# friendlymatthew/heif

Measured on AMD Instinct MI355X. Metric: Mpixels/s decoded (bit-exact) on 4032x3024 HEIC batch, higher is better.
Workload: dtype u8

## Files before the change

### heif_amd/csrc/api.cpp

```cpp
#include <hip/hip_runtime.h>

#include <algorithm>
#include <cmath>
#include <cstdlib>
#include <cstring>
#include <atomic>
#include <memory>
#include <mutex>
#include <string>
#include <thread>
#include <vector>

#include "../../include/heifgpu.h"
#include "common/desc.hpp"
#include "host/batch.hpp"
#include "host/heic_image.hpp"
#include "kernels/cabac.hpp"
#include "kernels/kernels.hpp"

using namespace hg;

struct heifgpu_image {
    ParsedImage img;
};

static_assert(sizeof(heifgpu_image_info) == 80, "heifgpu_image_info: 20 x uint32");
static_assert(sizeof(heifgpu_planes) == 40, "heifgpu_planes: 3 pointers + 3 int32 (+ padding)");
static_assert(sizeof(heifgpu_batch_opts) == 20, "heifgpu_batch_opts: 5 x uint32");
static_assert(sizeof(heifgpu_display_info) == 44, "heifgpu_display_info: 11 x 32 bits");
static_assert(sizeof(heifgpu_surface) == 16, "heifgpu_surface: pointer + int32 (+ padding)");
static_assert(sizeof(heifgpu_rect) == 16, "heifgpu_rect: 4 x uint32");
static_assert(HEIFGPU_PIX_RGB8 == RENDER_RGB8 && HEIFGPU_PIX_RGBA8 == RENDER_RGBA8 && HEIFGPU_PIX_RGB16 == RENDER_RGB16 &&
                  HEIFGPU_PIX_RGBA16 == RENDER_RGBA16,
              "pixel formats");
static_assert(sizeof(heifgpu_ipc_handle) == 72, "heifgpu_ipc_handle: 64-byte HIP handle + uint64 offset");
static_assert(HEIFGPU_PARSE_AUTO == PARSE_AUTO && HEIFGPU_PARSE_LANES == PARSE_LANES && HEIFGPU_PARSE_SOLO == PARSE_SOLO &&
                  HEIFGPU_PARSE_SPREAD == PARSE_SPREAD,
              "parse modes");
static_assert(sizeof(heifgpu_tile_params) == 55 * 4 + 64 * 4, "heifgpu_tile_params: 55 int32 + 64 uint32");

constexpr int kTimingSlots = 32;
struct RenderRing;
struct heifgpu_ctx {
    int device = 0;
    bool timing = false;
    hipStream_t parse = nullptr, xform = nullptr, recon = nullptr, upload = nullptr;
    hipStream_t prep = nullptr;
    hipEvent_t fork = nullptr, join = nullptr;
    StreamKnobs stream;
    hipEvent_t tev[kTimingSlots][10] = {};
    int timed_calls = 0, folded = 0;
    double acc[6] = {};
    RenderRing *render = nullptr;
};

namespace {
size_t xprog_words(const HostBatch &hb) { return size_t(hb.rows) + 1; }
size_t xntu_words(const HostBatch &hb) { return size_t(hb.rows) + hb.pics.size() + 1; }

bool prep_stream_default() {
    const char *e = std::getenv("HEIFGPU_PREP_STREAM");
    return e && std::atoi(e) != 0;
}

hipError_t fold_timing(heifgpu_ctx *ctx, int slot) {
    hipEvent_t *e = ctx->tev[slot];
    hipError_t r = hipEventSynchronize(e[8]);
    if (r != hipSuccess) return r;
    float t = 0.f;
    if ((r = hipEventElapsedTime(&t, e[0], e[1])) != hipSuccess) return r;
    ctx->acc[5] += t;
    if ((r = hipEventElapsedTime(&t, e[9], e[2])) != hipSuccess) return r;
    ctx->acc[0] += t;
    if ((r = hipEventElapsedTime(&t, e[3], e[4])) != hipSuccess) return r;
    ctx->acc[1] += t;
    for (int i = 2; i < 5; ++i) {
        if ((r = hipEventElapsedTime(&t, e[i + 3], e[i + 4])) != hipSuccess) return r;
        ctx->acc[i] += t;
    }
    return hipSuccess;
}
}

namespace {

thread_local std::string g_err;

int fail(int code, const std::string &msg) {
    g_err = msg;
    return code;
}

bool fault_injected(const char *what) {
    const char *e = std::getenv("HEIFGPU_FAULT_INJECT");
    return e && std::strcmp(e, what) == 0;
}

#define HIP_TRY(expr)                                                                             \
    do {                                                                                          \
        hipError_t e_ = (expr);                                                                   \
        if (e_ != hipSuccess) return fail(HEIFGPU_E_DEVICE, std::string(#expr) + ": " + hipGetErrorString(e_)); \
    } while (0)

template <class T>
struct DevBuf {
    T *p = nullptr;
    size_t n = 0;
    DevBuf() = default;
    DevBuf(const DevBuf &) = delete;
    DevBuf &operator=(const DevBuf &) = delete;
    ~DevBuf() {
        if (p) (void)hipFree(p);
    }
    size_t cap = 0;
    hipError_t alloc(size_t count) {
        n = count;
        if (p && count <= cap) return hipSuccess;
        if (p) {
            hipError_t e = hipFree(p);
            p = nullptr;
            cap = 0;
            if (e != hipSuccess) return e;
        }
        cap = std::max<size_t>(count, 1);
        return hipMalloc(reinterpret_cast<void **>(&p), cap * sizeof(T));
    }
};

struct PinnedBuf {
    uint8_t *p = nullptr;
    size_t cap = 0;
    PinnedBuf() = default;
    PinnedBuf(const PinnedBuf &) = delete;
    PinnedBuf &operator=(const PinnedBuf &) = delete;
    ~PinnedBuf() {
        if (p) (void)hipHostFree(p);
    }
    hipError_t reserve(size_t bytes) {
        if (p && bytes <= cap) return hipSuccess;
        if (p) {
            hipError_t e = hipHostFree(p);
            p = nullptr;
            cap = 0;
            if (e != hipSuccess) return e;
        }
        cap = std::max<size_t>(bytes, 4096);
        return hipHostMalloc(reinterpret_cast<void **>(&p), cap, hipHostMallocDefault);
    }
};

}

constexpr int kRenderSlots = 4;
struct RenderRing {
    struct Slot {
        PinnedBuf host;
        DevBuf<RenderDesc> dev;
        DevBuf<ScaleDesc> sdev;
        DevBuf<TensorDesc> tdev;
        hipEvent_t done = nullptr;
        bool pending = false;
    } slot[kRenderSlots];
    int next = 0;
    ~RenderRing() {
        for (Slot &s : slot)
            if (s.done) (void)hipEventDestroy(s.done);
    }
};

struct ParseSet {
    DevBuf<TuRec> tus;
    DevBuf<Coef> coefs;
    DevBuf<uint32_t> row_counts, status;
    DevBuf<uint8_t> maps;
    DevBuf<SaoParams> sao;
    DevBuf<int16_t> resid;
    DevBuf<uint32_t> xprog, xntu;
    DevBuf<uint8_t> rbsp;
    DevBuf<uint32_t> rsubs;
    hipEvent_t parsed = nullptr, transformed = nullptr, recon_done = nullptr, progreset = nullptr, prepped = nullptr;
    bool pending = false;
    ~ParseSet() {
        if (parsed) (void)hipEventDestroy(parsed);
        if (transformed) (void)hipEventDestroy(transformed);
        if (recon_done) (void)hipEventDestroy(recon_done);
        if (progreset) (void)hipEventDestroy(progreset);
        if (prepped) (void)hipEventDestroy(prepped);
    }
};

struct DescGen {
    DevBuf<PicDesc> pics;
    DevBuf<SeqParams> seqs;
    DevBuf<uint8_t> sf;
    DevBuf<OutImage> outs;
    DevBuf<uint32_t> sticky;
    std::vector<OutImage> out_host;
    hipEvent_t done = nullptr;
    bool pending = false;
    std::vector<uint32_t> pic_image;
    size_t n_images = 0;
    bool loaded = false;
    ~DescGen() {
        if (done) (void)hipEventDestroy(done);
    }
};

struct heifgpu_batch {
    int device = 0;
    size_t n_images = 0;
    int n_pics = 0;
    uint32_t tile_stride = 1, tile_offset = 0;
    PinnedBuf stage;
    hipEvent_t uploaded = nullptr;
    bool loaded = false;
    BatchArgs args{};
    DevBuf<uint8_t> bits;
    DevBuf<uint32_t> subs, porder;
    DevBuf<uint8_t> xctx;
    DevBuf<uint8_t> recon;
    DescGen gen[2];
    int cur = 0;
    ParseSet set[3];
    int n_sets = 1, next_set = 0, last_set = 0;
    std::vector<uint32_t> pic_image;
    std::vector<heifgpu_image_info> infos;
    ~heifgpu_batch() {
        if (uploaded) (void)hipEventDestroy(uploaded);
    }
};

extern "C" {

const char *heifgpu_last_error(void) { return g_err.c_str(); }

int heifgpu_image_parse(const uint8_t *data, size_t len, heifgpu_image **out) {
    return heifgpu_image_parse_item(data, len, 0, out);
}

int heifgpu_image_parse_item(const uint8_t *data, size_t len, uint32_t item_id, heifgpu_image **out) {
    if (!data || !out) return fail(HEIFGPU_E_INVALID, "null argument");
    *out = nullptr;
    try {
        auto im = std::make_unique<heifgpu_image>();
        im->img = parse_heic(data, len, item_id);
        *out = im.release();
        return HEIFGPU_OK;
    } catch (const UnsupportedError &e) {
        return fail(HEIFGPU_E_UNSUPPORTED, e.what());
    } catch (const std::exception &e) {
        return fail(HEIFGPU_E_PARSE, e.what());
    }
}

int heifgpu_image_parse_many(const uint8_t *const *data, const size_t *len, size_t n, int threads,
                             heifgpu_image **out, int *rc) {
    if (!data || !len || !out) return fail(HEIFGPU_E_INVALID, "null argument");
    for (size_t i = 0; i < n; ++i) out[i] = nullptr;
    std::vector<int> codes(n, HEIFGPU_OK);
    std::vector<std::string> msgs(n);
    std::atomic<size_t> next{0};
    auto worker = [&] {
        for (size_t i; (i = next.fetch_add(1)) < n;) {
            if (!data[i]) {
                codes[i] = HEIFGPU_E_INVALID;
                msgs[i] = "null data";
                continue;
            }
            try {
                auto im = std::make_unique<heifgpu_image>();
                im->img = parse_heic(data[i], len[i], 0);
                out[i] = im.release();
            } catch (const UnsupportedError &e) {
                codes[i] = HEIFGPU_E_UNSUPPORTED;
                msgs[i] = e.what();
            } catch (const std::exception &e) {
                codes[i] = HEIFGPU_E_PARSE;
                msgs[i] = e.what();
            }
        }
    };
    size_t nt = threads > 0 ? size_t(threads) : size_t(std::max(1u, std::thread::hardware_concurrency()));
    nt = std::min(nt, n);
    std::vector<std::thread> pool;
    for (size_t t = 1; t < nt; ++t) pool.emplace_back(worker);
    worker();
    for (auto &th : pool) th.join();
    int first = HEIFGPU_OK;
    for (size_t i = 0; i < n; ++i) {
        if (rc) rc[i] = codes[i];
        if (codes[i] != HEIFGPU_OK && first == HEIFGPU_OK) {
            first = codes[i];
            g_err = "image " + std::to_string(i) + ": " + msgs[i];
        }
    }
    return first;
}

int heifgpu_gather_tiles(const heifgpu_image_info *info, const heifgpu_planes *dst, const heifgpu_planes *src,
                         uint32_t tile_stride, uint32_t tile_offset, void *stream) {
    if (!info || !dst || !src) return fail(HEIFGPU_E_INVALID, "null argument");
    if (tile_stride == 0) tile_stride = 1;
    if (tile_offset >= tile_stride) return fail(HEIFGPU_E_INVALID, "tile_offset must be below tile_stride");
    if (info->chroma_format_idc > 3) return fail(HEIFGPU_E_INVALID, "chroma_format_idc");
    const int planes = info->chroma_format_idc ? 3 : 1;
    for (int c = 0; c < planes; ++c)
        if (!dst->plane[c] || !src->plane[c]) return fail(HEIFGPU_E_INVALID, "missing plane");
    hipPointerAttribute_t ad{}, as{};
    HIP_TRY(hipPointerGetAttributes(&ad, dst->plane[0]));
    HIP_TRY(hipPointerGetAttributes(&as, src->plane[0]));
    int cur = 0;
    HIP_TRY(hipGetDevice(&cur));
    HIP_TRY(hipSetDevice(ad.device));
    if (ad.device != as.device) {
        const hipError_t e = hipDeviceEnablePeerAccess(as.device, 0);
        (void)hipGetLastError();
        if (e != hipSuccess && e != hipErrorPeerAccessAlreadyEnabled) {
            (void)hipSetDevice(cur);
            HIP_TRY(e);
        }
    }
    GatherArgs g{};
    for (int c = 0; c < 3; ++c) {
        g.dst[c] = reinterpret_cast<uint64_t>(dst->plane[c]);
        g.src[c] = reinterpret_cast<uint64_t>(src->plane[c]);
        g.dpitch[c] = dst->pitch[c];
        g.spitch[c] = src->pitch[c];
    }
    g.planes = planes;
    g.sx = chroma_sx(int(info->chroma_format_idc));
    g.sy = chroma_sy(int(info->chroma_format_idc));
    g.bps = int32_t(info->bytes_per_sample);
    g.W = int32_t(info->width);
    g.H = int32_t(info->height);
    g.cols = int32_t(std::max(1u, info->grid_cols));
    g.tw = int32_t(info->tile_width ? info->tile_width : info->width);
    g.th = int32_t(info->tile_height ? info->tile_height : info->height);
    g.n_tiles = int32_t(std::max(1u, info->num_tiles));
    g.stride = int32_t(tile_stride);
    g.offset = int32_t(tile_offset);
    const hipError_t e = launch_gather_tiles(g, static_cast<hipStream_t>(stream));
    (void)hipSetDevice(cur);
    HIP_TRY(e);
    return HEIFGPU_OK;
}

namespace {
std::mutex g_ipc_mu;
std::vector<std::pair<void *, void *>> g_ipc_open;
}

int heifgpu_ipc_export(const void *dev_ptr, heifgpu_ipc_handle *out) {
    static_assert(sizeof(hipIpcMemHandle_t) == sizeof(out->handle), "hipIpcMemHandle_t is 64 bytes");
    if (!dev_ptr || !out) return fail(HEIFGPU_E_INVALID, "null argument");
    hipDeviceptr_t base = nullptr;
    size_t size = 0;
    HIP_TRY(hipMemGetAddressRange(&base, &size, const_cast<void *>(dev_ptr)));
    hipIpcMemHandle_t h;
    HIP_TRY(hipIpcGetMemHandle(&h, base));
    std::memcpy(out->handle, &h, sizeof(h));
    out->offset = uint64_t(static_cast<const uint8_t *>(dev_ptr) - static_cast<const uint8_t *>(base));
    return HEIFGPU_OK;
}

int heifgpu_ipc_open(int device, const heifgpu_ipc_handle *h, void **dev_ptr) {
    if (!h || !dev_ptr) return fail(HEIFGPU_E_INVALID, "null argument");
    *dev_ptr = nullptr;
    int cur = 0;
    HIP_TRY(hipGetDevice(&cur));
    HIP_TRY(hipSetDevice(device));
    hipIpcMemHandle_t mh;
    std::memcpy(&mh, h->handle, sizeof(mh));
    void *base = nullptr;
    const hipError_t e = hipIpcOpenMemHandle(&base, mh, hipIpcMemLazyEnablePeerAccess);
    (void)hipSetDevice(cur);
    HIP_TRY(e);
    *dev_ptr = static_cast<uint8_t *>(base) + h->offset;
    std::lock_guard<std::mutex> lk(g_ipc_mu);
    g_ipc_open.emplace_back(*dev_ptr, base);
    return HEIFGPU_OK;
}

int heifgpu_ipc_close(void *dev_ptr) {
    void *base = nullptr;
    {
        std::lock_guard<std::mutex> lk(g_ipc_mu);
        for (size_t i = 0; i < g_ipc_open.size(); ++i)
            if (g_ipc_open[i].first == dev_ptr) {
                base = g_ipc_open[i].second;
                g_ipc_open.erase(g_ipc_open.begin() + long(i));
                break;
            }
    }
    if (!base) return fail(HEIFGPU_E_INVALID, "not a pointer returned by heifgpu_ipc_open");
    HIP_TRY(hipIpcCloseMemHandle(base));
    return HEIFGPU_OK;
}

int heifgpu_image_get_info(const heifgpu_image *img, heifgpu_image_info *info) {
    if (!img || !info) return fail(HEIFGPU_E_INVALID, "null argument");
    const ParsedImage &p = img->img;
    const SequenceParameterSet &s = p.params[0].sps;
    std::memset(info, 0, sizeof(*info));
    info->width = p.out_width;
    info->height = p.out_height;
    info->chroma_format_idc = uint32_t(s.chroma_array_type());
    info->bit_depth = uint32_t(8 + s.bit_depth_luma_minus8);
    info->bytes_per_sample = info->bit_depth > 8 ? 2 : 1;
    info->grid_rows = p.rows;
    info->grid_cols = p.cols;
    info->tile_width = p.tile_width;
    info->tile_height = p.tile_height;
    info->num_tiles = uint32_t(p.tiles.size());
    info->rotation = p.rotation;
    info->ispe_width = p.ispe_width;
    info->ispe_height = p.ispe_height;
    info->coded_bytes = p.coded_bytes;
    info->primary_item_id = p.primary_item_id;
    info->num_thumbnails = p.num_thumbnails;
    info->matrix_coeffs = p.nclx ? p.nclx_matrix : uint32_t(s.matrix_coeffs);
    info->full_range = p.nclx ? p.nclx_full_range : (s.video_full_range_flag ? 1u : 0u);
    info->item_id = p.item_id;
    info->aux_item_id = p.aux_item_id;
    return HEIFGPU_OK;
}

int heifgpu_ycbcr_to_rgb(heifgpu_ctx *ctx, const heifgpu_image_info *info, const heifgpu_planes *in, void *rgb,
                         int32_t rgb_pitch, void *stream) {
    if (!ctx || !info || !in || !rgb || !in->plane[0]) return fail(HEIFGPU_E_INVALID, "invalid argument");
    if (info->chroma_format_idc > 3) return fail(HEIFGPU_E_INVALID, "chroma_format_idc");
    if (info->chroma_format_idc && (!in->plane[1] || !in->plane[2])) return fail(HEIFGPU_E_INVALID, "missing chroma plane");
    if (info->bit_depth < 8 || info->bit_depth > 16) return fail(HEIFGPU_E_INVALID, "bit depth");
    HIP_TRY(hipSetDevice(ctx->device));
    ColorArgs c{};
    for (int k = 0; k < 3; ++k) {
        c.plane[k] = reinterpret_cast<uint64_t>(in->plane[k]);
        c.pitch[k] = in->pitch[k];
    }
    c.rgb = reinterpret_cast<uint64_t>(rgb);
    c.rgb_pitch = rgb_pitch;
    c.w = int32_t(info->width);
    c.h = int32_t(info->height);
    c.rotation = int32_t(info->rotation & 3);
    c.out_w = (c.rotation & 1) ? c.h : c.w;
    c.out_h = (c.rotation & 1) ? c.w : c.h;
    if (rgb_pitch < 3 * c.out_w) return fail(HEIFGPU_E_INVALID, "rgb_pitch smaller than 3 * output width");
    c.chroma = int32_t(info->chroma_format_idc);
    c.shift = int32_t(info->bit_depth) - 8;
    color_coefs(info->matrix_coeffs, info->full_range != 0, c);
    HIP_TRY(launch_ycbcr_rgb(c, int(info->bytes_per_sample), static_cast<hipStream_t>(stream)));
    return HEIFGPU_OK;
}

int heifgpu_image_get_display(const heifgpu_image *img, heifgpu_display_info *out) {
    if (!img || !out) return fail(HEIFGPU_E_INVALID, "null argument");
    const ParsedImage &p = img->img;
    std::memset(out, 0, sizeof(*out));
    out->out_width = p.display.out_width;
    out->out_height = p.display.out_height;
    for (int k = 0; k < 4; ++k) out->m[k] = p.display.m[k];
    out->t[0] = p.display.t[0];
    out->t[1] = p.display.t[1];
    out->n_transforms = p.display.n_transforms;
    out->alpha_item_id = p.alpha_item_id;
    out->alpha_premultiplied = p.alpha_premultiplied;
    return HEIFGPU_OK;
}

static int render_desc_fill(size_t i, const heifgpu_image *const *imgs, const heifgpu_planes *in,
                            const heifgpu_image *const *alpha_imgs, const heifgpu_planes *alpha_in, uint32_t format,
                            const heifgpu_surface *out, const DisplayMap &dm, uint32_t ow, uint32_t oh, int &bps,
                            RenderDesc &d) {
    const bool wide = format >= HEIFGPU_PIX_RGB16, with_alpha = (format & 1) != 0;
    const int bpp = (with_alpha ? 4 : 3) * (wide ? 2 : 1);
    heifgpu_image_info info;
    heifgpu_image_get_info(imgs[i], &info);
// ... 187 lines not shown
    }
    if (!ctx) return fail(HEIFGPU_E_INVALID, "null context");
    hipStream_t s = static_cast<hipStream_t>(stream);
    RenderRing::Slot *slot = nullptr;
    if (int rc = render_ring_slot(ctx, &slot)) return rc;
    RenderRing::Slot &sl = *slot;
    const size_t bytes = n * sizeof(ScaleDesc);
    HIP_TRY(sl.host.reserve(bytes));
    HIP_TRY(sl.sdev.alloc(n));
    std::memcpy(sl.host.p, descs.data(), bytes);
    HIP_TRY(hipMemcpyAsync(sl.sdev.p, sl.host.p, bytes, hipMemcpyHostToDevice, s));
    HIP_TRY(launch_render_scaled(sl.sdev.p, int(n), max_tiles, int(format), bps, s));
    HIP_TRY(hipEventRecord(sl.done, s));
    sl.pending = true;
    return HEIFGPU_OK;
}

int heifgpu_render_batch_tensor(heifgpu_ctx *ctx, const heifgpu_image *const *imgs, size_t n, const heifgpu_planes *in,
                                const heifgpu_image *const *alpha_imgs, const heifgpu_planes *alpha_in,
                                const heifgpu_tensor_format *fmt, const heifgpu_scale *scale, const uint32_t *flip,
                                const heifgpu_tensor_surface *out, void *stream) {
    if (!imgs || !in || !fmt || !scale || !out || n == 0) return fail(HEIFGPU_E_INVALID, "invalid argument");
    if (fmt->src > HEIFGPU_PIX_RGBA16) return fail(HEIFGPU_E_INVALID, "source format");
    if (fmt->elem > HEIFGPU_ELEM_BF16) return fail(HEIFGPU_E_INVALID, "element type");
    if (fmt->layout > HEIFGPU_LAYOUT_HWC) return fail(HEIFGPU_E_INVALID, "layout");
    const int nch = (fmt->src & 1) ? 4 : 3;
    for (int c = 0; c < nch; ++c)
        if (!std::isfinite(fmt->a[c]) || !std::isfinite(fmt->b[c]))
            return fail(HEIFGPU_E_INVALID, "scale or bias not finite");
    if (n > 65535) return fail(HEIFGPU_E_INVALID, "more than 65535 images in one render call");
    const int64_t esz = fmt->elem == HEIFGPU_ELEM_F32 ? 4 : 2;
    std::vector<TensorDesc> descs(n);
    int bps = 0, max_tiles = 0;
    for (size_t i = 0; i < n; ++i) {
        const uint32_t fl = flip ? flip[i] : 0;
        if (fl > 3) return fail(HEIFGPU_E_INVALID, "flip above 3");
        TensorDesc &td = descs[i];
        if (int rc = scale_desc_fill(i, imgs, in, alpha_imgs, alpha_in, fmt->src, scale[i], fl, nullptr, bps, td.s))
            return rc;
        const heifgpu_tensor_surface &o = out[i];
        if (!o.data || (reinterpret_cast<uintptr_t>(o.data) & uintptr_t(esz - 1)))
            return fail(HEIFGPU_E_INVALID, "tensor data null or not aligned to its element");
        const int64_t row = int64_t(td.s.r.out_w) * esz * (fmt->layout == HEIFGPU_LAYOUT_HWC ? nch : 1);
        if (o.stride_y < row || (o.stride_y & (esz - 1)))
            return fail(HEIFGPU_E_INVALID, "stride_y below the row or not a multiple of the element size");
        if (fmt->layout == HEIFGPU_LAYOUT_CHW && (o.stride_c & (esz - 1)))
            return fail(HEIFGPU_E_INVALID, "stride_c not a multiple of the element size");
        td.s.r.out = reinterpret_cast<uint64_t>(o.data);
        td.stride_c = fmt->layout == HEIFGPU_LAYOUT_CHW ? o.stride_c : 0;
        td.stride_y = o.stride_y;
        td.elem = int32_t(fmt->elem);
        td.layout = int32_t(fmt->layout);
        for (int c = 0; c < 4; ++c) {
            td.a[c] = c < nch ? fmt->a[c] : 0.f;
            td.b[c] = c < nch ? fmt->b[c] : 0.f;
        }
        max_tiles = std::max(max_tiles, td.s.r.tiles);
    }
    if (!ctx) return fail(HEIFGPU_E_INVALID, "null context");
    hipStream_t s = static_cast<hipStream_t>(stream);
    RenderRing::Slot *slot = nullptr;
    if (int rc = render_ring_slot(ctx, &slot)) return rc;
    RenderRing::Slot &sl = *slot;
    const size_t bytes = n * sizeof(TensorDesc);
    HIP_TRY(sl.host.reserve(bytes));
    HIP_TRY(sl.tdev.alloc(n));
    std::memcpy(sl.host.p, descs.data(), bytes);
    HIP_TRY(hipMemcpyAsync(sl.tdev.p, sl.host.p, bytes, hipMemcpyHostToDevice, s));
    HIP_TRY(launch_render_tensor(sl.tdev.p, int(n), max_tiles, int(fmt->src), bps, s));
    HIP_TRY(hipEventRecord(sl.done, s));
    sl.pending = true;
    return HEIFGPU_OK;
}

void heifgpu_image_free(heifgpu_image *img) { delete img; }

int heifgpu_create(int device, heifgpu_ctx **out) {
    if (!out) return fail(HEIFGPU_E_INVALID, "null argument");
    *out = nullptr;
    int n = 0;
    HIP_TRY(hipGetDeviceCount(&n));
    if (device < 0 || device >= n) return fail(HEIFGPU_E_DEVICE, "no such HIP device");
    HIP_TRY(hipSetDevice(device));
    auto c = std::make_unique<heifgpu_ctx>();
    c->device = device;
    c->stream = stream_knobs_from_env();
    static const bool prio = [] {
        const char *e = std::getenv("HEIFGPU_PARSE_PRIORITY");
        return e && std::atoi(e) != 0;
    }();
    int least = 0, greatest = 0;
    HIP_TRY(hipDeviceGetStreamPriorityRange(&least, &greatest));
    HIP_TRY(hipStreamCreateWithPriority(&c->parse, hipStreamNonBlocking, prio ? greatest : least));
    static const bool rprio = [] {
        const char *e = std::getenv("HEIFGPU_RECON_PRIORITY");
        return e && std::atoi(e) != 0;
    }();
    HIP_TRY(hipStreamCreateWithPriority(&c->xform, hipStreamNonBlocking, rprio ? greatest : least));
    HIP_TRY(hipStreamCreateWithPriority(&c->recon, hipStreamNonBlocking, rprio ? greatest : least));
    HIP_TRY(hipStreamCreateWithFlags(&c->upload, hipStreamNonBlocking));
    if (prep_stream_default()) HIP_TRY(hipStreamCreateWithFlags(&c->prep, hipStreamNonBlocking));
    HIP_TRY(hipEventCreateWithFlags(&c->fork, hipEventDisableTiming));
    HIP_TRY(hipEventCreateWithFlags(&c->join, hipEventDisableTiming));
    for (auto &row : c->tev)
        for (auto &e : row) HIP_TRY(hipEventCreate(&e));
    *out = c.release();
    return HEIFGPU_OK;
}

void heifgpu_destroy(heifgpu_ctx *ctx) {
    if (!ctx) return;
    (void)hipSetDevice(ctx->device);
    (void)hipDeviceSynchronize();
    for (auto &row : ctx->tev)
        for (auto &e : row)
            if (e) (void)hipEventDestroy(e);
    if (ctx->fork) (void)hipEventDestroy(ctx->fork);
    if (ctx->join) (void)hipEventDestroy(ctx->join);
    if (ctx->parse) (void)hipStreamDestroy(ctx->parse);
    if (ctx->xform) (void)hipStreamDestroy(ctx->xform);
    if (ctx->recon) (void)hipStreamDestroy(ctx->recon);
    if (ctx->upload) (void)hipStreamDestroy(ctx->upload);
    if (ctx->prep) (void)hipStreamDestroy(ctx->prep);
    delete ctx->render;
    delete ctx;
}

int heifgpu_set_timing(heifgpu_ctx *ctx, int enable) {
    if (!ctx) return fail(HEIFGPU_E_INVALID, "null ctx");
    if (enable && !ctx->timing) {
        for (double &v : ctx->acc) v = 0.0;
        ctx->timed_calls = ctx->folded = 0;
    }
    ctx->timing = enable != 0;
    return HEIFGPU_OK;
}

int heifgpu_stage_times(heifgpu_ctx *ctx, float ms[6]) {
    if (!ctx || !ms) return fail(HEIFGPU_E_INVALID, "null argument");
    if (!ctx->timing) return fail(HEIFGPU_E_INVALID, "timing disabled");
    for (int i = 0; i < 6; ++i) ms[i] = 0.f;
    for (int c = ctx->folded; c < ctx->timed_calls; ++c) HIP_TRY(fold_timing(ctx, c % kTimingSlots));
    if (ctx->timed_calls)
        for (int i = 0; i < 6; ++i) ms[i] = float(ctx->acc[i] / ctx->timed_calls);
    for (double &v : ctx->acc) v = 0.0;
    ctx->timed_calls = ctx->folded = 0;
    return HEIFGPU_OK;
}

static Rect rect_of(const heifgpu_rect &r) { return Rect{r.x, r.y, r.width, r.height}; }

int heifgpu_window_source_rect(const heifgpu_image *img, const heifgpu_rect *window, heifgpu_rect *src) {
    if (!img || !src) return fail(HEIFGPU_E_INVALID, "null argument");
    Rect out;
    if (!window_source_rect(img->img, window ? rect_of(*window) : Rect{}, out))
        return fail(HEIFGPU_E_INVALID, "window empty or outside the displayed picture");
    *src = heifgpu_rect{out.x, out.y, out.w, out.h};
    return HEIFGPU_OK;
}

int heifgpu_image_tiles_for_rect(const heifgpu_image *img, const heifgpu_rect *src, uint32_t *col0, uint32_t *row0,
                                 uint32_t *cols, uint32_t *rows) {
    if (!img) return fail(HEIFGPU_E_INVALID, "null argument");
    const Rect r = src ? rect_of(*src) : Rect{};
    if (!rect_inside(r, img->img.out_width, img->img.out_height))
        return fail(HEIFGPU_E_INVALID, "source rectangle empty or outside the image");
    uint32_t v[4];
    tiles_for_rect(img->img, r, v[0], v[1], v[2], v[3]);
    if (col0) *col0 = v[0];
    if (row0) *row0 = v[1];
    if (cols) *cols = v[2];
    if (rows) *rows = v[3];
    return HEIFGPU_OK;
}

static int prepare_args(const heifgpu_image *const *imgs, size_t n, const heifgpu_batch_opts *opts,
                        const heifgpu_rect *src, uint32_t &stride, uint32_t &offset,
                        std::vector<const ParsedImage *> &parsed, std::vector<Rect> &rects) {
    stride = opts && opts->tile_stride ? opts->tile_stride : 1u;
    offset = opts ? opts->tile_offset : 0u;
    if (offset >= stride) return fail(HEIFGPU_E_INVALID, "tile_offset must be below tile_stride");
    for (size_t i = 0; i < n; ++i) {
        if (!imgs[i]) return fail(HEIFGPU_E_INVALID, "null image");
        parsed.push_back(&imgs[i]->img);
        if (!src) continue;
        rects.push_back(rect_of(src[i]));
        if (!rect_inside(rects.back(), imgs[i]->img.out_width, imgs[i]->img.out_height))
            return fail(HEIFGPU_E_INVALID, "source rectangle of image " + std::to_string(i) + " empty or outside the image");
    }
    return HEIFGPU_OK;
}

int heifgpu_batch_count_pictures(const heifgpu_image *const *imgs, size_t n, const heifgpu_batch_opts *opts,
                                 const heifgpu_rect *src, uint32_t *pictures) {
    if (!imgs || !pictures || n == 0) return fail(HEIFGPU_E_INVALID, "invalid argument");
    uint32_t stride, offset;
    std::vector<const ParsedImage *> parsed;
    std::vector<Rect> rects;
    if (int rc = prepare_args(imgs, n, opts, src, stride, offset, parsed, rects)) return rc;
    try {
        *pictures = uint32_t(build_batch(parsed.data(), n, stride, offset, true,
                                         src ? rects.data() : nullptr).pics.size());
    } catch (const UnsupportedError &e) {
        return fail(HEIFGPU_E_UNSUPPORTED, e.what());
    } catch (const std::exception &e) {
        return fail(HEIFGPU_E_PARSE, e.what());
    }
    return HEIFGPU_OK;
}

int heifgpu_batch_picture_count(const heifgpu_batch *b, uint32_t *pictures) {
    if (!b || !pictures) return fail(HEIFGPU_E_INVALID, "null argument");
    if (!b->loaded) return fail(HEIFGPU_E_INVALID, "batch not loaded (its last prepare failed)");
    *pictures = uint32_t(b->n_pics);
    return HEIFGPU_OK;
}

int heifgpu_batch_prepare_ex(heifgpu_ctx *ctx, const heifgpu_image *const *imgs, size_t n,
                             const heifgpu_batch_opts *opts, heifgpu_batch **inout) {
    return heifgpu_batch_prepare_rects(ctx, imgs, n, opts, nullptr, inout);
}

int heifgpu_batch_prepare_rects(heifgpu_ctx *ctx, const heifgpu_image *const *imgs, size_t n,
                                const heifgpu_batch_opts *opts, const heifgpu_rect *src, heifgpu_batch **inout) {
    if (!ctx || !imgs || !inout || n == 0) return fail(HEIFGPU_E_INVALID, "invalid argument");
    const uint32_t stride = opts && opts->tile_stride ? opts->tile_stride : 1u;
    const uint32_t offset = opts ? opts->tile_offset : 0u;
    if (offset >= stride) return fail(HEIFGPU_E_INVALID, "tile_offset must be below tile_stride");
    const uint32_t mode_req = opts ? opts->parse_mode : 0u;
    if (mode_req > HEIFGPU_PARSE_ROWS) return fail(HEIFGPU_E_INVALID, "parse_mode");
    if (mode_req == HEIFGPU_PARSE_ROWS)
        return fail(HEIFGPU_E_UNSUPPORTED, "HEIFGPU_PARSE_ROWS was removed in ABI 6 (DESIGN.md 5.9)");
    const int ppw_req = opts ? int(std::min<uint32_t>(opts->pics_per_wave, 64u)) : 0;
    if (*inout && (*inout)->device != ctx->device) return fail(HEIFGPU_E_INVALID, "batch belongs to another device");
    std::vector<const ParsedImage *> parsed;
    std::vector<Rect> rects;
    {
        uint32_t s_, o_;
        if (int rc = prepare_args(imgs, n, opts, src, s_, o_, parsed, rects)) return rc;
    }
    HIP_TRY(hipSetDevice(ctx->device));
    std::vector<heifgpu_image_info> infos;
    for (size_t i = 0; i < n; ++i) {
        heifgpu_image_info info;
        heifgpu_image_get_info(imgs[i], &info);
        infos.push_back(info);
    }
    HostBatch hb;
    try {
        hb = build_batch(parsed.data(), n, stride, offset, true, src ? rects.data() : nullptr);
    } catch (const UnsupportedError &e) {
        return fail(HEIFGPU_E_UNSUPPORTED, e.what());
    } catch (const std::exception &e) {
        return fail(HEIFGPU_E_PARSE, e.what());
    }
    std::unique_ptr<heifgpu_batch> fresh;
    heifgpu_batch *b = *inout;
    if (!b) {
        fresh = std::make_unique<heifgpu_batch>();
        b = fresh.get();
        b->device = ctx->device;
        HIP_TRY(hipEventCreateWithFlags(&b->uploaded, hipEventDisableTiming));
        static const int pipeline = [] {
            const char *e = std::getenv("HEIFGPU_PIPELINE");
            return e ? std::atoi(e) : 3;
        }();
        const int sets = opts && opts->pipeline_sets ? int(opts->pipeline_sets) : pipeline;
        b->n_sets = sets <= 1 ? 1 : (sets >= 3 ? 3 : 2);
        for (int k = 0; k < b->n_sets; ++k) {
            HIP_TRY(hipEventCreateWithFlags(&b->set[k].parsed, hipEventDisableTiming));
            HIP_TRY(hipEventCreateWithFlags(&b->set[k].transformed, hipEventDisableTiming));
            HIP_TRY(hipEventCreateWithFlags(&b->set[k].recon_done, hipEventDisableTiming));
            HIP_TRY(hipEventCreateWithFlags(&b->set[k].progreset, hipEventDisableTiming));
            HIP_TRY(hipEventCreateWithFlags(&b->set[k].prepped, hipEventDisableTiming));
        }
        for (DescGen &g : b->gen) HIP_TRY(hipEventCreateWithFlags(&g.done, hipEventDisableTiming));
    }
    HIP_TRY(hipEventSynchronize(b->uploaded));
    const int gi = b->gen[b->cur].loaded ? b->cur ^ 1 : b->cur;
    DescGen &G = b->gen[gi];
    for (int k = 0; k < b->n_sets; ++k)
        if (b->set[k].pending) HIP_TRY(hipStreamWaitEvent(ctx->upload, b->set[k].parsed, 0));
    if (G.pending) HIP_TRY(hipStreamWaitEvent(ctx->upload, G.done, 0));
    std::vector<uint32_t> order;
    const int mode = parse_mode_for(int(mode_req), int(hb.pics.size()), hb.pics.data());
    const int solo_waves = solo_waves_for(hb.lane_rows);
    int parse_group = 1;
    if (mode == PARSE_SPREAD) {
        if (spread_parse_order(hb.pics.data(), int(hb.pics.size()), order) < 0)
            return fail(HEIFGPU_E_UNSUPPORTED, "spread parse: over 2^20 pictures or 4096 substreams per picture");
    } else {
        parse_group = lanes_parse_order(hb.pics.data(), int(hb.pics.size()), hb.lane_rows,
                                        mode == PARSE_SOLO ? 1 : ppw_req, order);
    }
    const bool cross_rows = mode == PARSE_SPREAD;
    const bool grows = (order.size() > b->porder.cap || hb.bits_size > b->bits.cap || hb.bits_size > b->set[0].rbsp.cap || hb.pics.size() > G.pics.cap ||
                                     hb.subs.size() > b->subs.cap || hb.seqs.size() > G.seqs.cap ||
                                     hb.sf.size() > G.sf.cap || n > G.outs.cap || hb.recon_bytes > b->recon.cap ||
                                     hb.resid_elems > b->set[0].resid.cap || hb.tu_n > b->set[0].tus.cap ||
                                     hb.coef_n > b->set[0].coefs.cap || hb.map_bytes > b->set[0].maps.cap ||
                                     hb.sao_n > b->set[0].sao.cap || 2 * size_t(hb.rows) > b->set[0].row_counts.cap ||
                                     hb.pics.size() > b->set[0].status.cap || hb.pics.size() > G.sticky.cap ||
                                     (cross_rows && (xprog_words(hb) > b->set[0].xprog.cap || hb.rows * CTX_PAD > b->xctx.cap)) ||
                                     (mode == PARSE_SPREAD && xntu_words(hb) > b->set[0].xntu.cap));
    if (grows) {
        for (int k = 0; k < b->n_sets; ++k)
            if (b->set[k].pending) HIP_TRY(hipEventSynchronize(b->set[k].recon_done));
        HIP_TRY(hipStreamSynchronize(ctx->upload));
    }
    b->loaded = false;
    G.loaded = false;
    G.pic_image.clear();
    G.n_images = 0;
    if (fault_injected("prepare"))
        return fail(HEIFGPU_E_INVALID, "injected prepare failure (HEIFGPU_FAULT_INJECT=prepare)");
    HIP_TRY(b->bits.alloc(hb.bits_size));
    HIP_TRY(G.pics.alloc(hb.pics.size()));
    HIP_TRY(b->subs.alloc(hb.subs.size()));
    HIP_TRY(G.seqs.alloc(hb.seqs.size()));
    HIP_TRY(G.sf.alloc(hb.sf.size()));
    HIP_TRY(G.outs.alloc(n));
    HIP_TRY(G.sticky.alloc(hb.pics.size()));
    HIP_TRY(hipMemsetAsync(G.sticky.p, 0, hb.pics.size() * sizeof(uint32_t), ctx->upload));
    for (int k = 0; k < b->n_sets; ++k) {
        ParseSet &ps = b->set[k];
        HIP_TRY(ps.tus.alloc(hb.tu_n));
        HIP_TRY(ps.coefs.alloc(hb.coef_n));
        HIP_TRY(ps.row_counts.alloc(size_t(2) * hb.rows));
        HIP_TRY(ps.maps.alloc(hb.map_bytes));
        HIP_TRY(ps.sao.alloc(hb.sao_n));
        HIP_TRY(ps.status.alloc(hb.pics.size()));
        HIP_TRY(ps.resid.alloc(hb.resid_elems));
        HIP_TRY(ps.rbsp.alloc(hb.bits_size));
        HIP_TRY(ps.rsubs.alloc(hb.subs.size()));
    }
    HIP_TRY(b->recon.alloc(hb.recon_bytes));
    HIP_TRY(b->porder.alloc(order.size()));
    if (cross_rows) {
        for (int k = 0; k < b->n_sets; ++k) {
            HIP_TRY(b->set[k].xprog.alloc(xprog_words(hb)));
            if (mode == PARSE_SPREAD) HIP_TRY(b->set[k].xntu.alloc(xntu_words(hb)));
        }
        HIP_TRY(b->xctx.alloc(std::max<size_t>(hb.rows, 1) * CTX_PAD));
    }
    struct Seg {
        const void *src;
        size_t bytes;
        void *dst;
    };
    const Seg segs[] = {
        {nullptr, hb.bits_size, b->bits.p},
        {hb.pics.data(), hb.pics.size() * sizeof(PicDesc), G.pics.p},
        {hb.subs.data(), hb.subs.size() * sizeof(uint32_t), b->subs.p},
        {hb.seqs.data(), hb.seqs.size() * sizeof(SeqParams), G.seqs.p},
        {hb.sf.data(), hb.sf.size(), G.sf.p},
        {order.data(), order.size() * sizeof(uint32_t), b->porder.p},
    };
    size_t total = 0;
    for (const Seg &g : segs) total += (g.bytes + 255) & ~size_t(255);
    HIP_TRY(b->stage.reserve(total));
    {
        uint8_t *dst = b->stage.p;
        const size_t np = hb.pieces.size();
        const size_t nt = std::min<size_t>(std::max(1u, std::min(16u, std::thread::hardware_concurrency())),
                                           (hb.bits_size >> 22) + 1);
        std::atomic<size_t> next{0};
        auto copy = [&] {
            for (size_t i; (i = next.fetch_add(64)) < np;)
                for (size_t j = i; j < std::min(np, i + 64); ++j) {
                    const HostBatch::Piece &pc = hb.pieces[j];
                    std::memcpy(dst + pc.dst, pc.src, pc.len);
                    const size_t end = j + 1 < np ? hb.pieces[j + 1].dst : hb.bits_size;
                    std::memset(dst + pc.dst + pc.len, 0, end - pc.dst - pc.len);
                }
        };
        std::vector<std::thread> pool;
        for (size_t t = 1; t < nt; ++t) pool.emplace_back(copy);
        copy();
        for (auto &th : pool) th.join();
        if (np == 0) std::memset(dst, 0, hb.bits_size);
    }
    size_t off = 0;
    for (const Seg &g : segs) {
        if (g.bytes) {
            if (g.src) std::memcpy(b->stage.p + off, g.src, g.bytes);
            HIP_TRY(hipMemcpyAsync(g.dst, b->stage.p + off, g.bytes, hipMemcpyHostToDevice, ctx->upload));
        }
        off += (g.bytes + 255) & ~size_t(255);
    }
    for (int k = 0; k < b->n_sets; ++k) HIP_TRY(hipMemsetAsync(b->set[k].rbsp.p, 0, hb.bits_size, ctx->upload));
    HIP_TRY(hipEventRecord(b->uploaded, ctx->upload));
    b->n_images = n;
    b->tile_stride = stride;
    b->tile_offset = offset;
    b->infos = std::move(infos);
    b->pic_image = hb.pic_image;
    G.pic_image = hb.pic_image;
    G.n_images = n;
    G.loaded = true;
    b->n_pics = int(hb.pics.size());
    b->cur = gi;
    b->loaded = true;
    BatchArgs &a = b->args;
    a = BatchArgs{};
    a.bits = b->bits.p;
    a.pics = G.pics.p;
    a.subs = b->subs.p;
    a.rbsp = nullptr;
    a.rsubs = nullptr;
    a.parse_order = b->porder.p;
    a.n_slots = int(order.size());
    a.parse_group = parse_group;
    a.seqs = G.seqs.p;
    a.sf = G.sf.p;
    a.outs = G.outs.p;
    a.recon = b->recon.p;
    a.n_pics = b->n_pics;
    a.max_width = hb.max_w;
    a.max_wctb = hb.max_wctb;
    a.max_rows = hb.max_rows;
    a.max_log2ctb = hb.max_log2ctb;
    a.lane_rows = hb.lane_rows;
    a.parse_mode = mode;
    a.solo_waves = solo_waves;
    a.xprog = nullptr;
    a.xctx = cross_rows ? b->xctx.p : nullptr;
    a.intra_stream = intra_stream_for(mode, int(hb.pics.size()), hb.has_assembly, ctx->stream) ? 1 : 0;
    a.xntu = nullptr;
    a.stream_patience_us = ctx->stream.patience_us;
    a.wpp_ring = mode == PARSE_SOLO ? (hb.max_wpp_rows > solo_waves ? 1 : 0) : hb.wpp_ring;
    a.lanes_lean = mode == PARSE_LANES
                       ? lanes_variant_for(hb.seqs.data(), hb.pics.data(), int(hb.pics.size()), a.wpp_ring)
                       : LANES_GENERAL;
    a.flags_from_recs = mode == PARSE_LANES ? 1 : 0;
    a.has_assembly = hb.has_assembly ? 1 : 0;
    a.total_rows = int(hb.rows);
    a.bytes_per_sample = hb.bps;
    a.chroma_format = hb.chroma;
    G.out_host.assign(n, OutImage{});
    if (fresh) *inout = fresh.release();
    return HEIFGPU_OK;
}

int heifgpu_batch_prepare(heifgpu_ctx *ctx, const heifgpu_image *const *imgs, size_t n, heifgpu_batch **out) {
    if (!out) return fail(HEIFGPU_E_INVALID, "invalid argument");
    *out = nullptr;
    const int rc = heifgpu_batch_prepare_ex(ctx, imgs, n, nullptr, out);
    if (rc) return rc;
    HIP_TRY(hipStreamSynchronize(ctx->upload));
    return HEIFGPU_OK;
}

int heifgpu_batch_decode(heifgpu_ctx *ctx, heifgpu_batch *b, const heifgpu_planes *out, void *stream) {
    if (!ctx || !b || !out) return fail(HEIFGPU_E_INVALID, "invalid argument");
    if (b->device != ctx->device) return fail(HEIFGPU_E_INVALID, "batch belongs to another device");
    if (!b->loaded) return fail(HEIFGPU_E_INVALID, "batch not loaded (its last prepare failed)");
    hipStream_t s = static_cast<hipStream_t>(stream);
    HIP_TRY(hipSetDevice(ctx->device));
    DescGen &G = b->gen[b->cur];
    bool changed = false;
    for (size_t i = 0; i < b->n_images; ++i) {
        OutImage o{};
        for (int c = 0; c < 3; ++c) {
            o.plane[c] = reinterpret_cast<uint64_t>(out[i].plane[c]);
            o.pitch[c] = out[i].pitch[c];
        }
        if (!out[i].plane[0] || (b->infos[i].chroma_format_idc && (!out[i].plane[1] || !out[i].plane[2])))
            return fail(HEIFGPU_E_INVALID, "missing output plane");
        o.width = int32_t(b->infos[i].width);
        o.height = int32_t(b->infos[i].height);
        if (std::memcmp(&o, &G.out_host[i], sizeof(o)) != 0) {
            G.out_host[i] = o;
            changed = true;
        }
    }
    if (changed)
        HIP_TRY(hipMemcpyAsync(G.outs.p, G.out_host.data(), b->n_images * sizeof(OutImage), hipMemcpyHostToDevice, s));
    const int k = b->next_set;
    b->next_set = (k + 1) % b->n_sets;
    b->last_set = k;
    ParseSet &ps = b->set[k];
    BatchArgs a = b->args;
    a.tus = ps.tus.p;
    a.coefs = ps.coefs.p;
    a.row_counts = ps.row_counts.p;
    a.maps = ps.maps.p;
    a.sao = ps.sao.p;
    a.status = ps.status.p;
    a.resid = ps.resid.p;
    a.rbsp = ps.rbsp.p;
    a.rsubs = ps.rsubs.p;
    if (a.parse_mode == PARSE_SPREAD) {
        a.xprog = ps.xprog.p;
        a.xjob = ps.xprog.p + a.total_rows;
        a.xntu = a.intra_stream ? ps.xntu.p : nullptr;
    }
    static const int max_stages = [] {
        const char *e = std::getenv("HEIFGPU_STAGES");
        return e ? std::atoi(e) : 5;
    }();
    if (max_stages < 5) {
        a.intra_stream = 0;
        a.xntu = nullptr;
        HIP_TRY(hipStreamSynchronize(ctx->upload));
        HIP_TRY(hipStreamSynchronize(ctx->parse));
        HIP_TRY(hipStreamSynchronize(ctx->xform));
        HIP_TRY(hipStreamSynchronize(ctx->recon));
        HIP_TRY(hipMemsetAsync(ps.status.p, 0, size_t(b->n_pics) * sizeof(uint32_t), s));
        HIP_TRY(hipMemsetAsync(ps.row_counts.p, 0, size_t(2) * uint32_t(b->args.total_rows) * sizeof(uint32_t), s));
        HIP_TRY(launch_rbsp(a, s));
        hipError_t (*fns[5])(const BatchArgs &, hipStream_t) = {launch_parse, launch_transform, launch_intra,
                                                                launch_deblock, launch_sao_out};
        for (int i = 0; i < max_stages; ++i) HIP_TRY(fns[i](a, s));
        HIP_TRY(launch_status_fold(ps.status.p, G.sticky.p, b->n_pics, s));
        return HEIFGPU_OK;
    }
#if defined(HG_ABLATE)
    static const int ablate = [] {
        const char *e = std::getenv("HEIFGPU_ABLATE");
        return e ? std::atoi(e) : 0;
    }();
#else
    constexpr int ablate = 0;
#endif
    hipStream_t p = ctx->parse, r = ctx->recon;
    if (b->n_pics == 0) {
        return HEIFGPU_OK;
    }
    const bool t = ctx->timing;
    hipEvent_t *ev = nullptr;
    if (t) {
        const int slot = ctx->timed_calls % kTimingSlots;
        if (ctx->timed_calls - ctx->folded >= kTimingSlots) {
            HIP_TRY(fold_timing(ctx, slot));
            ++ctx->folded;
        }
        ev = ctx->tev[slot];
        ++ctx->timed_calls;
    }
    hipStream_t q = ctx->prep ? ctx->prep : p;
    HIP_TRY(hipStreamWaitEvent(q, b->uploaded, 0));
    if (ps.pending) HIP_TRY(hipStreamWaitEvent(q, ps.recon_done, 0));
    if (t) HIP_TRY(hipEventRecord(ev[0], q));
    HIP_TRY(launch_rbsp(a, q));
    if (a.intra_stream) HIP_TRY(hipEventRecord(ps.progreset, q));
    if (t) HIP_TRY(hipEventRecord(ev[1], q));
    if (q != p) {
        HIP_TRY(hipEventRecord(ps.prepped, q));
        HIP_TRY(hipStreamWaitEvent(p, ps.prepped, 0));
    }
    if (t) HIP_TRY(hipEventRecord(ev[9], p));
    HIP_TRY(launch_parse(a, p));
    if (t) HIP_TRY(hipEventRecord(ev[2], p));
    HIP_TRY(hipEventRecord(ps.parsed, p));
    HIP_TRY(hipEventRecord(ctx->fork, s));
    if (a.intra_stream) {
        HIP_TRY(hipStreamWaitEvent(r, ps.progreset, 0));
        if (t) {
            HIP_TRY(hipEventRecord(ev[3], r));
            HIP_TRY(hipEventRecord(ev[4], r));
        }
    } else {
        hipStream_t x = b->n_sets >= 3 ? ctx->xform : r;
        HIP_TRY(hipStreamWaitEvent(x, ps.parsed, 0));
        if (t) HIP_TRY(hipEventRecord(ev[3], x));
        if (!(ablate & 1)) HIP_TRY(launch_transform(a, x));
        if (t) HIP_TRY(hipEventRecord(ev[4], x));
        HIP_TRY(hipEventRecord(ps.transformed, x));
        HIP_TRY(hipStreamWaitEvent(r, ps.transformed, 0));
    }
    if (t) HIP_TRY(hipEventRecord(ev[5], r));
    if (!(ablate & 2)) HIP_TRY(launch_intra(a, r));
    if (a.intra_stream) {
        HIP_TRY(hipStreamWaitEvent(r, ps.parsed, 0));
        BatchArgs a2 = a;
        a2.stream_redo = 1;
        HIP_TRY(launch_intra(a2, r));
    }
    if (t) HIP_TRY(hipEventRecord(ev[6], r));
    if (!(ablate & 4)) HIP_TRY(launch_deblock(a, r));
    if (t) HIP_TRY(hipEventRecord(ev[7], r));
    HIP_TRY(hipStreamWaitEvent(r, ctx->fork, 0));
    if (!(ablate & 8)) HIP_TRY(launch_sao_out(a, r));
    if (t) HIP_TRY(hipEventRecord(ev[8], r));
    HIP_TRY(launch_status_fold(ps.status.p, G.sticky.p, b->n_pics, r));
    HIP_TRY(hipEventRecord(ps.recon_done, r));
    ps.pending = true;
    HIP_TRY(hipEventRecord(G.done, r));
    G.pending = true;
    HIP_TRY(hipEventRecord(ctx->join, r));
    HIP_TRY(hipStreamWaitEvent(s, ctx->join, 0));
    return HEIFGPU_OK;
}

int heifgpu_batch_parse_geometry(const heifgpu_batch *b, uint32_t *mode, uint32_t *workgroups,
                                 uint32_t *pics_per_wave, uint32_t *waves_per_workgroup) {
    if (!b || !b->loaded) return fail(HEIFGPU_E_INVALID, "invalid batch");
    const BatchArgs &a = b->args;
    const bool solo = a.parse_mode == PARSE_SOLO, lanes = a.parse_mode == PARSE_LANES;
    const uint32_t ppw = lanes ? uint32_t(std::max(1, a.parse_group)) : 1u;
    if (mode) *mode = uint32_t(a.parse_mode);
    if (workgroups) *workgroups = (uint32_t(a.n_slots) + ppw - 1) / ppw;
    if (pics_per_wave) *pics_per_wave = ppw;
    if (waves_per_workgroup) *waves_per_workgroup = solo ? uint32_t(a.solo_waves) : 1u;
    return HEIFGPU_OK;
}

int heifgpu_batch_lanes_variant(const heifgpu_batch *b, uint32_t *variant) {
    if (!b || !b->loaded || !variant) return fail(HEIFGPU_E_INVALID, "invalid argument");
    *variant = b->args.parse_mode == PARSE_LANES ? uint32_t(b->args.lanes_lean) : uint32_t(LANES_GENERAL);
    return HEIFGPU_OK;
}

int heifgpu_batch_status(heifgpu_ctx *ctx, heifgpu_batch *b, uint32_t *status, void *stream) {
    if (!ctx || !b) return fail(HEIFGPU_E_INVALID, "invalid argument");
    if (b->device != ctx->device) return fail(HEIFGPU_E_INVALID, "batch belongs to another device");
    if (!b->loaded) return fail(HEIFGPU_E_INVALID, "batch not loaded (its last prepare failed)");
    hipStream_t s = static_cast<hipStream_t>(stream);
    HIP_TRY(hipSetDevice(ctx->device));
    DescGen &G = b->gen[b->cur];
    std::vector<uint32_t> st(size_t(b->n_pics));
    if (!st.empty()) {
        HIP_TRY(hipMemcpyAsync(st.data(), G.sticky.p, st.size() * sizeof(uint32_t), hipMemcpyDeviceToHost, s));
        HIP_TRY(hipMemsetAsync(G.sticky.p, 0, st.size() * sizeof(uint32_t), s));
    }
    HIP_TRY(hipStreamSynchronize(s));
    std::vector<uint32_t> per(b->n_images, 0);
    for (size_t p = 0; p < st.size(); ++p) per[b->pic_image[p]] |= st[p];
    bool bad = false;
    for (size_t i = 0; i < b->n_images; ++i) {
        if (status) status[i] = per[i];
        bad |= per[i] != 0;
    }
    return bad ? fail(HEIFGPU_E_DECODE, "one or more pictures failed the kernel bitstream checks") : HEIFGPU_OK;
}

int heifgpu_batch_status_previous(heifgpu_ctx *ctx, heifgpu_batch *b, uint32_t *status, size_t cap, size_t *n_prev,
                                  void *stream) {
    if (!ctx || !b || !n_prev) return fail(HEIFGPU_E_INVALID, "invalid argument");
    if (b->device != ctx->device) return fail(HEIFGPU_E_INVALID, "batch belongs to another device");
    *n_prev = 0;
    if (!b->loaded) return fail(HEIFGPU_E_INVALID, "batch not loaded (its last prepare failed)");
    DescGen &P = b->gen[b->cur ^ 1];
    if (!P.loaded || P.pic_image.empty()) return HEIFGPU_OK;
    *n_prev = P.n_images;
    if (!status) return HEIFGPU_OK;
    if (cap < P.n_images) return fail(HEIFGPU_E_INVALID, "status array smaller than the previous load");
    hipStream_t s = static_cast<hipStream_t>(stream);
    HIP_TRY(hipSetDevice(ctx->device));
    if (P.pending) HIP_TRY(hipStreamWaitEvent(s, P.done, 0));
    std::vector<uint32_t> st(P.pic_image.size());
    HIP_TRY(hipMemcpyAsync(st.data(), P.sticky.p, st.size() * sizeof(uint32_t), hipMemcpyDeviceToHost, s));
    HIP_TRY(hipMemsetAsync(P.sticky.p, 0, st.size() * sizeof(uint32_t), s));
    HIP_TRY(hipStreamSynchronize(s));
    std::vector<uint32_t> per(P.n_images, 0);
    for (size_t p = 0; p < st.size(); ++p) per[P.pic_image[p]] |= st[p];
    bool bad = false;
    for (size_t i = 0; i < P.n_images; ++i) {
        status[i] = per[i];
        bad |= per[i] != 0;
    }
    return bad ? fail(HEIFGPU_E_DECODE, "one or more pictures of the previous load failed the kernel bitstream checks")
               : HEIFGPU_OK;
}

int heifgpu_abi_version(void) { return HEIFGPU_ABI_VERSION; }

void heifgpu_batch_free(heifgpu_batch *b) {
    if (!b) return;
    (void)hipSetDevice(b->device);
    (void)hipDeviceSynchronize();
    delete b;
}

int heifgpu_decode_batch(heifgpu_ctx *ctx, const heifgpu_image *const *imgs, size_t n, const heifgpu_planes *out,
                         void *stream, uint32_t *status) {
    heifgpu_batch *b = nullptr;
    int rc = heifgpu_batch_prepare(ctx, imgs, n, &b);
    if (rc) return rc;
    rc = heifgpu_batch_decode(ctx, b, out, stream);
    if (!rc) rc = heifgpu_batch_status(ctx, b, status, stream);
    heifgpu_batch_free(b);
    return rc;
}

size_t heifgpu_remove_emulation_prevention(const uint8_t *in, size_t n, uint8_t *out) {
    std::vector<uint8_t> v = RbspReader::remove_emulation_prevention(in, n);
    if (!v.empty()) std::memcpy(out, v.data(), v.size());
    return v.size();
}

int heifgpu_read_ue(const uint8_t *buf, size_t n, uint32_t *val) {
    try {
        RbspReader r(buf, n);
        *val = r.read_ue();
        return HEIFGPU_OK;
    } catch (const std::exception &e) {
        return fail(HEIFGPU_E_PARSE, e.what());
    }
}

int heifgpu_read_se(const uint8_t *buf, size_t n, int32_t *val) {
    try {
        RbspReader r(buf, n);
        *val = r.read_se();
        return HEIFGPU_OK;
    } catch (const std::exception &e) {
        return fail(HEIFGPU_E_PARSE, e.what());
    }
}

namespace {
struct VecBins {
    const uint8_t *b;
    int n, i = 0;
    bool under = false;
    int operator()() {
        if (i >= n) {
            under = true;
            return 0;
        }
        return b[i++] ? 1 : 0;
    }
};
}

int heifgpu_bins_truncated_rice(const uint8_t *bins, int n, int c_max, int c_rice, int *used) {
    VecBins v{bins, n};
    uint32_t r = bin_truncated_rice(v, uint32_t(c_max), c_rice);
    if (used) *used = v.i;
    return v.under ? -1 : int(r);
}

int heifgpu_bins_chroma_pred_mode(const uint8_t *bins, int n, int *used) {
    VecBins v{bins, n};
    uint32_t r = bin_intra_chroma_pred_mode(v, v);
    if (used) *used = v.i;
    return v.under ? -1 : int(r);
}

int heifgpu_bins_coeff_abs_level_remaining(const uint8_t *bins, int n, int c_rice, int *used) {
    VecBins v{bins, n};
    uint32_t r = bin_coeff_abs_level_remaining(v, c_rice);
    if (used) *used = v.i;
    return (v.under || r == 0xffffffffu) ? -1 : int(r);
}

int heifgpu_bins_exp_golomb(const uint8_t *bins, int n, int k, int *used) {
    VecBins v{bins, n};
    uint32_t r = bin_exp_golomb(v, k);
    if (used) *used = v.i;
    return (v.under || r == 0xffffffffu) ? -1 : int(r);
}

int heifgpu_image_tile_params(const heifgpu_image *img, uint32_t tile, heifgpu_tile_params *o) {
    if (!img || !o) return fail(HEIFGPU_E_INVALID, "invalid argument");
    const ParsedImage &pi = img->img;
    if (tile >= pi.tiles.size()) return fail(HEIFGPU_E_INVALID, "tile index out of range");
    const TileJob &t = pi.tiles[tile];
    const SequenceParameterSet &sps = pi.params[t.param].sps;
    const PictureParameterSet &pps = pi.params[t.param].pps;
    const SliceSegmentHeader &sh = t.segs[0].sh;
    std::memset(o, 0, sizeof(*o));
    o->nal_unit_type = t.segs[0].nal.nal_unit_type();
    o->slice_type = sh.slice_type;
    o->first_slice_segment_in_pic = sh.first_slice_segment_in_pic_flag;
    o->general_profile_idc = sps.general_profile_idc;
    o->general_level_idc = sps.general_level_idc;
    o->pic_width = sps.pic_width_in_luma_samples;
    o->pic_height = sps.pic_height_in_luma_samples;
    o->chroma_format_idc = sps.chroma_format_idc;
    o->bit_depth_luma = 8 + sps.bit_depth_luma_minus8;
    o->bit_depth_chroma = 8 + sps.bit_depth_chroma_minus8;
    o->log2_max_poc_lsb = sps.log2_max_pic_order_cnt_lsb;
    o->log2_min_cb = sps.log2_min_luma_coding_block_size;
    o->log2_ctb = sps.log2_ctb_size;
    o->log2_min_tb = sps.log2_min_tb_size;
    o->log2_max_tb = sps.log2_max_tb_size;
    o->max_th_depth_inter = sps.max_transform_hierarchy_depth_inter;
    o->max_th_depth_intra = sps.max_transform_hierarchy_depth_intra;
    o->scaling_list_enabled = sps.scaling_list_enabled_flag;
    o->amp = sps.amp_enabled_flag;
    o->sao = sps.sample_adaptive_offset_enabled_flag;
    o->pcm = sps.pcm_enabled_flag;
    o->num_short_term_ref_pic_sets = sps.num_short_term_ref_pic_sets;
    o->long_term_refs = sps.long_term_ref_pics_present_flag;
    o->temporal_mvp = sps.sps_temporal_mvp_enabled_flag;
    o->strong_intra_smoothing = sps.strong_intra_smoothing_enabled_flag;
    o->video_full_range = sps.video_full_range_flag;
    o->colour_primaries = sps.colour_primaries;
    o->transfer_characteristics = sps.transfer_characteristics;
    o->matrix_coeffs = sps.matrix_coeffs;
    o->init_qp = 26 + pps.init_qp_minus26;
    o->sign_data_hiding = pps.sign_data_hiding_enabled_flag;
    o->cabac_init_present = pps.cabac_init_present_flag;
    o->constrained_intra_pred = pps.constrained_intra_pred_flag;
    o->transform_skip = pps.transform_skip_enabled_flag;
    o->cu_qp_delta_enabled = pps.cu_qp_delta_enabled_flag;
    o->diff_cu_qp_delta_depth = pps.diff_cu_qp_delta_depth;
    o->cb_qp_offset = pps.pps_cb_qp_offset;
    o->cr_qp_offset = pps.pps_cr_qp_offset;
    o->slice_chroma_qp_offsets_present = pps.pps_slice_chroma_qp_offsets_present_flag;
    o->transquant_bypass = pps.transquant_bypass_enabled_flag;
    o->tiles_enabled = pps.tiles_enabled_flag;
    o->entropy_coding_sync = pps.entropy_coding_sync_enabled_flag;
    o->loop_filter_across_slices = pps.pps_loop_filter_across_slices_enabled_flag;
    o->deblocking_control_present = pps.deblocking_filter_control_present_flag;
    o->deblocking_override_enabled = pps.deblocking_filter_override_enabled_flag;
    o->deblocking_disabled = sh.slice_deblocking_filter_disabled_flag;
    o->beta_offset_div2 = sh.slice_beta_offset_div2;
    o->tc_offset_div2 = sh.slice_tc_offset_div2;
    o->log2_parallel_merge_level = pps.log2_parallel_merge_level;
// ... 12 lines not shown
```

### heif_amd/csrc/emu/emu_check.cpp

```cpp
#include <cstdio>
#include <cstdlib>
#include <cstring>
#include <vector>

#include "../../../oracle/oracle.h"
#include "../host/batch.hpp"
#include "../kernels/cabac.hpp"
#include "../kernels/kernels.hpp"

namespace hg {
thread_local EmuCtx g_emu;
}
using namespace hg;

int main(int argc, char **argv) {
    if (argc < 2) return 2;
    setvbuf(stdout, nullptr, _IONBF, 0);
    Rect want;
    bool have_rect = false;
    {
        int k = 1;
        for (int j = 1; j < argc; ++j) {
            if (j > 1 && !strncmp(argv[j], "rect=", 5)) {
                if (sscanf(argv[j] + 5, "%u,%u,%u,%u", &want.x, &want.y, &want.w, &want.h) != 4) return 2;
                have_rect = true;
            } else {
                argv[k++] = argv[j];
            }
        }
        argc = k;
    }
    int stages = argc > 2 ? atoi(argv[2]) : 5;
    const bool host_only = stages <= 0;
    const uint32_t tstride = !host_only && argc > 4 ? uint32_t(atoi(argv[3])) : 1u,
                   toff = !host_only && argc > 4 ? uint32_t(atoi(argv[4])) : 0u;
    auto read_file = [](const char *path, std::vector<uint8_t> &out) {
        FILE *f = fopen(path, "rb");
        if (!f) return false;
        fseek(f, 0, SEEK_END);
        long n = ftell(f);
        fseek(f, 0, SEEK_SET);
        out.assign(static_cast<size_t>(n), 0);
        const bool ok = fread(out.data(), 1, size_t(n), f) == size_t(n);
        fclose(f);
        return ok;
    };
    std::vector<uint8_t> data;
    if (!read_file(argv[1], data)) return 2;
    std::vector<std::vector<uint8_t>> more_data;
    for (int k = 3; host_only && k < argc; ++k) {
        more_data.emplace_back();
        if (!read_file(argv[k], more_data.back())) return 2;
    }
    ParsedImage im;
    std::vector<ParsedImage> more(more_data.size());
    HostBatch hb;
    try {
        im = parse_heic(data.data(), data.size());
        std::vector<const ParsedImage *> ims{&im};
        for (size_t k = 0; k < more.size(); ++k) {
            more[k] = parse_heic(more_data[k].data(), more_data[k].size());
            ims.push_back(&more[k]);
        }
        std::vector<Rect> rects(ims.size());
        rects[0] = want;
        hb = build_batch(ims.data(), ims.size(), tstride, toff, false, have_rect ? rects.data() : nullptr);
    } catch (const std::exception &e) {
        printf("host rejected: %s\n", e.what());
        return 3;
    }
    std::vector<TuRec> tus(hb.tu_n);
    std::vector<Coef> coefs(hb.coef_n);
    std::vector<uint32_t> rc(2 * hb.rows), status(hb.pics.size());
    std::vector<uint8_t> recon(hb.recon_bytes), maps(hb.map_bytes);
    if (getenv("HEIFGPU_EMU_DUMP_MAPS")) std::fill(maps.begin(), maps.end(), uint8_t(0xa5));
    std::vector<int16_t> resid(hb.resid_elems);
    std::vector<SaoParams> sao(hb.sao_n);
    const int W = int(im.out_width), H = int(im.out_height), bps = hb.bps;
    const int SX = chroma_sx(hb.chroma), SY = chroma_sy(hb.chroma);
    const int CW = (W + (1 << SX) - 1) >> SX, CH = (H + (1 << SY) - 1) >> SY;
    constexpr uint8_t kSentinel = 0xa5;
    std::vector<uint8_t> oy(size_t(W) * H * bps, kSentinel), ocb(size_t(CW) * CH * bps, kSentinel),
        ocr(size_t(CW) * CH * bps, kSentinel);
    OutImage out{};
    out.plane[0] = uint64_t(oy.data());
    out.plane[1] = uint64_t(ocb.data());
    out.plane[2] = uint64_t(ocr.data());
    out.pitch[0] = W * bps;
    out.pitch[1] = out.pitch[2] = CW * bps;
    out.width = W;
    out.height = H;
    BatchArgs a{};
    a.bits = hb.bits.data();
    a.pics = hb.pics.data();
    a.subs = hb.subs.data();
    std::vector<uint8_t> rbsp(hb.bits.size(), 0);
    std::vector<uint32_t> rsubs(hb.subs.size(), 0);
    a.rbsp = rbsp.data();
    a.rsubs = rsubs.data();
    std::vector<uint32_t> order;
    const int mode = parse_mode_for(PARSE_AUTO, int(hb.pics.size()), hb.pics.data());
    const int solo_waves = solo_waves_for(hb.lane_rows);
    int parse_group = 1;
    if (mode == PARSE_SPREAD) spread_parse_order(hb.pics.data(), int(hb.pics.size()), order);
    else
        parse_group = lanes_parse_order(hb.pics.data(), int(hb.pics.size()), hb.lane_rows, mode == PARSE_SOLO ? 1 : 0,
                                        order);
    std::vector<uint32_t> xprog(hb.rows + 1), xntu(hb.rows + hb.pics.size() + 1, 0);
    std::vector<uint8_t> xctx((hb.rows + 1) * size_t(CTX_PAD));
    a.parse_order = order.data();
    a.n_slots = int(order.size());
    a.parse_group = parse_group;
    a.seqs = hb.seqs.data();
    a.sf = hb.sf.data();
    a.outs = &out;
    a.tus = tus.data();
    a.coefs = coefs.data();
    a.row_counts = rc.data();
    a.recon = recon.data();
    a.resid = resid.data();
    a.maps = maps.data();
    a.sao = sao.data();
    a.status = status.data();
    a.n_pics = int(hb.pics.size());
    a.max_width = hb.max_w;
    a.max_wctb = hb.max_wctb;
    a.max_rows = hb.max_rows;
    a.max_log2ctb = hb.max_log2ctb;
    a.lane_rows = hb.lane_rows;
    a.parse_mode = mode;
    a.solo_waves = solo_waves;
    a.xprog = xprog.data();
    a.xctx = xctx.data();
    a.xjob = xprog.data() + hb.rows;
    const StreamKnobs knobs = stream_knobs_from_env();
    a.intra_stream = intra_stream_for(mode, int(hb.pics.size()), hb.has_assembly, knobs) ? 1 : 0;
    a.xntu = a.intra_stream ? xntu.data() : nullptr;
    a.stream_patience_us = knobs.patience_us;
    a.wpp_ring = mode == PARSE_SOLO ? (hb.max_wpp_rows > solo_waves ? 1 : 0) : hb.wpp_ring;
    a.lanes_lean = mode == PARSE_LANES
                       ? lanes_variant_for(hb.seqs.data(), hb.pics.data(), int(hb.pics.size()), a.wpp_ring)
                       : LANES_GENERAL;
    a.flags_from_recs = mode == PARSE_LANES ? 1 : 0;
    a.has_assembly = hb.has_assembly ? 1 : 0;
    a.total_rows = int(hb.rows);
    a.bytes_per_sample = bps;
    a.chroma_format = hb.chroma;
    if (stages <= 0) {
        printf("host ok: %zu pictures\n", hb.pics.size());
        printf("parse mode: %s\n", mode == PARSE_SOLO ? "solo" : mode == PARSE_SPREAD ? "spread" : "lanes");
        if (mode == PARSE_LANES) printf("lanes variant: %s\n", a.lanes_lean ? "lean" : "general");
        return 0;
    }
    std::fill(rc.begin(), rc.end(), 0xa5a5a5a5u);
    std::fill(status.begin(), status.end(), 0x5au);
    std::fill(xprog.begin(), xprog.end(), 0x7777u);
    std::fill(xntu.begin(), xntu.end(), 0x3333u);
    printf("pictures: %zu\n", hb.pics.size());
    emu_rbsp(a);
    emu_parse(a);
    uint32_t st = 0;
    for (uint32_t s : status) st |= s;
    uint64_t ntu = 0, ncoef = 0;
    for (uint32_t r = 0; r < hb.rows; ++r) {
        ntu += rc[2 * r];
        ncoef += rc[2 * r + 1];
    }
    if (getenv("HG_EMU_DEBUG_MODES")) {
        int shown = 0;
        for (const PicDesc &pd : hb.pics)
            for (uint32_t r = 0; r < (uint32_t)((hb.seqs[pd.seq].height + (1 << hb.seqs[pd.seq].log2_ctb) - 1) >> hb.seqs[pd.seq].log2_ctb); ++r) {
                const uint32_t nt = rc[2 * (pd.row_off + r)];
                for (uint32_t t = 0; t < nt && shown < 10; ++t) {
                    const TuRec &tu = tus[pd.tu_off + (uint64_t)r * pd.tu_cap_row + t];
                    if (tu.mode > 34) {
                        printf("bad mode %d pic %u row %u t %u x %d y %d log2 %d flags 0x%x ctu %d\n", tu.mode, (unsigned)(&pd - hb.pics.data()), r, t, tu.x, tu.y, tu.log2, tu.flags, tu.ctu);
                        ++shown;
                    }
                }
            }
    }
    printf("parse mode: %s\n", mode == PARSE_SOLO     ? "solo"
                               : mode == PARSE_SPREAD ? "spread"
                                                      : "lanes");
    if (mode == PARSE_LANES) printf("lanes variant: %s\n", a.lanes_lean ? "lean" : "general");
    printf("parse: status 0x%x, %llu TBs, %llu coefficients\n", st, (unsigned long long)ntu, (unsigned long long)ncoef);
    if (stages >= 2 && !a.intra_stream) emu_transform(a);
    if (stages >= 3) {
        emu_intra(a);
        if (a.intra_stream) {
            BatchArgs a2 = a;
            a2.stream_redo = 1;
            emu_intra(a2);
        }
    }
    if (stages >= 4) emu_deblock(a);
    if (const char *path = getenv("HEIFGPU_EMU_DUMP_MAPS")) {
        FILE *f = fopen(path, "wb");
        if (!f) return 2;
        for (const PicDesc &pd : hb.pics) {
            const SeqParams &sp = hb.seqs[pd.seq];
            const size_t n = size_t((sp.width + 3) >> 2) * size_t((sp.height + 3) >> 2);
            fwrite(maps.data() + pd.map_off, 1, 2 * n, f);
        }
        fclose(f);
    }
    if (stages >= 5) {
        emu_sao_out(a);
    } else {
        int dbk = stages >= 4 ? 0 : 1;
        oracle_set_debug_flags(dbk | 2);
        for (const PicDesc &pd : hb.pics) {
            const SeqParams &sp = hb.seqs[pd.seq];
            for (int c = 0; c < 3; ++c) {
                if (c && !sp.chroma_format) break;
                const int sx = c ? SX : 0, sy = c ? SY : 0, PW = sp.width >> sx, PH = sp.height >> sy;
                size_t off = c == 0 ? 0 : size_t(sp.width) * sp.height + size_t(c - 1) * PW * PH;
                int vw = std::min(sp.out_w, W - pd.out_x) >> sx, vh = std::min(sp.out_h, H - pd.out_y) >> sy;
                for (int y = 0; y < vh; ++y)
                    for (int x = 0; x < vw; ++x) {
                        size_t src = (off + size_t(y + (sp.conf_t >> sy)) * PW + x + (sp.conf_l >> sx)) * bps;
                        uint8_t *dst = reinterpret_cast<uint8_t *>(out.plane[c]) +
                                       size_t((pd.out_y >> sy) + y) * out.pitch[c] + size_t((pd.out_x >> sx) + x) * bps;
                        memcpy(dst, recon.data() + pd.recon_off + src, size_t(bps));
                    }
            }
        }
    }
    if (stages < 3) return st ? 1 : 0;
    oracle_image ref;
    if (oracle_decode_heic(data.data(), data.size(), &ref, nullptr, 0, nullptr)) {
        printf("oracle failed: %s\n", oracle_last_error());
        return 1;
    }
    long bad_total = 0;
    std::vector<uint8_t> shown;
    if (have_rect) {
        shown.assign(size_t(W) * H, 0);
        for (const PicDesc &pd : hb.pics) {
            if (pd.flags & PD_CHILD) continue;
            const SeqParams &sp = hb.seqs[pd.seq];
            for (int y = std::max(pd.out_y, 0); y < std::min(pd.out_y + sp.out_h, H); ++y)
                for (int x = std::max(pd.out_x, 0); x < std::min(pd.out_x + sp.out_w, W); ++x) shown[size_t(y) * W + x] = 1;
        }
        long uncovered = 0;
        for (uint32_t y = want.y; y < want.y + want.h; ++y)
            for (uint32_t x = want.x; x < want.x + want.w; ++x) uncovered += !shown[size_t(y) * W + x];
        printf("rect %u,%u %ux%u: %ld samples not covered by the selected pictures\n", want.x, want.y, want.w, want.h,
               uncovered);
        bad_total += uncovered;
    }
    const char *names[3] = {"Y", "Cb", "Cr"};
    for (int c = 0; c < 3; ++c) {
        const uint8_t *g = c == 0 ? oy.data() : (c == 1 ? ocb.data() : ocr.data());
        int pw = int(ref.pw[c]), ph = int(ref.ph[c]);
        long bad = 0;
        int fx = -1, fy = -1;
        const int sx = c ? SX : 0, sy = c ? SY : 0;
        for (int y = 0; y < ph; ++y)
            for (int x = 0; x < pw; ++x) {
                int gv = bps == 1 ? g[size_t(y) * pw + x] : reinterpret_cast<const uint16_t *>(g)[size_t(y) * pw + x];
                const uint32_t tile = uint32_t((y << sy) / int(im.tile_height)) * im.cols + uint32_t((x << sx) / int(im.tile_width));
                const bool sel = have_rect ? shown[size_t(y << sy) * W + (x << sx)] != 0 : tile % tstride == toff;
                const int exp = sel ? int(ref.plane[c][size_t(y) * pw + x]) : (bps == 1 ? kSentinel : kSentinel * 0x101);
                if (gv != exp) {
                    if (!bad) fx = x, fy = y;
                    ++bad;
                }
            }
        printf("%s: %ld mismatches", names[c], bad);
        if (bad) {
            printf(" first at (%d,%d) tile (%d,%d) emu %d ref %d", fx, fy, (fy << sy) / int(im.tile_height),
                   (fx << sx) / int(im.tile_width),
                   bps == 1 ? g[size_t(fy) * pw + fx] : 0, ref.plane[c][size_t(fy) * pw + fx]);
        }
        printf("\n");
        bad_total += bad;
    }
    oracle_image_free(&ref);
    printf("%s\n", bad_total || st ? "EMU PARITY FAIL" : "EMU PARITY OK");
    return bad_total || st ? 1 : 0;
}
```

### heif_amd/csrc/emu/emu_parse.cpp

```cpp
#include "../kernels/parse_units.hpp"

#include <cstdio>
#include <string>
#include <vector>

namespace hg {

template <class EG>
void emu_parse_lanes(const BatchArgs &a) {
    const int ppw = a.parse_order && a.parse_group > 0 ? a.parse_group : lanes_pics_per_wave(a.lane_rows, a.n_pics);
    const int n_slots = a.parse_order ? a.n_slots : a.n_pics;
    const int waves = (n_slots + ppw - 1) / ppw;
    uint64_t tab[kTabRows], seq[15];
    uint8_t scan8[128];
    for (int i = 0; i < 64; ++i) scan8_tables(scan8, i);
    for (int i = 0; i < kTabRows; ++i) tab[i] = state_row_ctx(i);
    for (int i = 0; i < 15; ++i) seq[i] = sig_seq(i);
    std::vector<LaneLds> lds(64);
    std::vector<LanePic> pics(64);
    std::vector<Lane> lanes(64);
    std::vector<uint8_t> wctx(a.wpp_ring ? 64 * CTX_PAD : 0);
    uint32_t prog[64];
    static const bool stats = std::getenv("HEIFGPU_LANES_STATS") != nullptr;
    static const std::string order = [] {
        const char *e = std::getenv("HEIFGPU_EMU_PASS_ORDER");
        std::string o;
        if (e && *e) {
            for (const char *c = e; *c; ++c)
                if (*c >= '0' + U_CTU && *c <= '0' + U_TBD) o += *c;
        } else {
            for (int i = 0; i < kPassKinds; ++i) o += (char)('0' + pass_kind(i));
        }
        return o;
    }();
    for (int w = 0; w < waves; ++w) {
        for (int l = 0; l < 64; ++l) {
            prog[l] = 0;
            const int pl = l / a.lane_rows, row = l % a.lane_rows;
            const int slot = w * ppw + pl;
            const bool in = pl < ppw && slot < n_slots && (!a.parse_order || a.parse_order[slot] != ~0u);
            const int pic = a.pic0 + (in && a.parse_order ? (int)a.parse_order[slot] : slot);
            const bool live = in && lane_init(lanes[l], pics[pl], lds[l], a, pic, row, pl * a.lane_rows, a.lane_rows);
            if (!live) lanes[l].st = U_DONE;
        }
        Env E{&a, lds.data(), prog, a.wpp_ring ? wctx.data() : nullptr, 0};
        long passes = 0, units = 0, kruns = 0, kr[U_TBD + 1] = {}, ku[U_TBD + 1] = {};
        for (;; ++passes) {
            bool any = false, progressed = false;
            for (int l = 0; l < 64; ++l) any |= lanes[l].st != U_DONE;
            if (!any) break;
            for (int l = 0; l < 64; ++l)
                if (lanes[l].st != U_DONE) {
                    const LanePic &P = pics[l / a.lane_rows];
                    const EG G{lds[l].ctx, tab, seq, a.rbsp, (P.bits_end + 64u) & ~3u, scan8, scan8 + 64};
                    q_refill(lanes[l], G);
                }
            for (const char ch : order) {
                const int kind = ch - '0';
                bool mine[64], anym = false;
                int cnt = 0;
                for (int l = 0; l < 64; ++l) {
                    E.lane = l;
                    mine[l] = lanes[l].st == kind && (kind != U_CTU || ctu_ready<EG>(lanes[l], pics[l / a.lane_rows], E));
                    anym |= mine[l];
                    cnt += mine[l] ? 1 : 0;
                }
                if (!anym) continue;
                ++kruns;
                ++kr[kind];
                ku[kind] += cnt;
                if (kind == U_SB) {
                    bool any4 = false;
                    for (int l = 0; l < 64; ++l) any4 |= mine[l] && lanes[l].tb_log2 == 2;
                    HG_COV(any4 ? COV_SB_RUN_ANY4 : COV_SB_RUN_NO4);
                }
                for (int l = 0; l < 64; ++l) {
                    Lane &L = lanes[l];
                    E.lane = l;
                    LanePic &P = pics[l / a.lane_rows];
                    if (!mine[l]) continue;
                    progressed = true;
                    ++units;
                    const EG G{lds[l].ctx, tab, seq, a.rbsp, (P.bits_end + 64u) & ~3u, scan8, scan8 + 64};
                    run_unit(kind, L, lds[l], P, E, G);
                }
            }
            if (!progressed) {
                for (int l = 0; l < 64; ++l)
                    if (lanes[l].st != U_DONE) {
                        lanes[l].status |= ST_SUBSTREAM_END;
                        atomicOr(&a.status[pics[l / a.lane_rows].pic], lanes[l].status & ~ST_SEGSW);
                        lanes[l].st = U_DONE;
                    }
                break;
            }
        }
        if (stats) {
            printf("wave %d: %ld passes, %.1f units per pass, %ld kind runs, %.2f units per kind run\n", w, passes,
                   (double)units / passes, kruns, (double)units / kruns);
            printf("  runs");
            for (int k = U_CTU; k <= U_TBD; ++k) printf(" %ld", kr[k]);
            printf("\n  units");
            for (int k = U_CTU; k <= U_TBD; ++k) printf(" %ld", ku[k]);
            printf("\n  paths");
            for (int k = 0; k < COV_N; ++k) printf(" %ld", g_cov[k]), g_cov[k] = 0;
            printf("\n  sb_paths");
            for (int k = COV_N; k < COV_SB_END; ++k) printf(" %ld", g_cov[k]), g_cov[k] = 0;
            printf("\n  tb_paths");
            for (int k = COV_SB_END; k < COV_ALL; ++k) printf(" %ld", g_cov[k]), g_cov[k] = 0;
            printf("\n");
        }
    }
}

template <bool Spread>
void emu_parse_solo(const BatchArgs &a) {
    using EG = EngSoloT<Spread>;
    const int NW = Spread ? a.max_rows : a.solo_waves;
    const int n_slots = a.parse_order ? a.n_slots : a.n_pics;
    uint64_t seq[15];
    for (int i = 0; i < 15; ++i) seq[i] = sig_seq(i);
    std::vector<LaneLds> lds((size_t)NW);
    std::vector<Lane> lanes((size_t)NW);
    std::vector<uint8_t> wctx((size_t)NW * CTX_PAD);
    std::vector<uint32_t> wbuf((size_t)NW * 192);
    std::vector<SoloWin> wins((size_t)NW);
    LanePic P;
    uint32_t prog[64];
    for (int slot = 0; slot < n_slots; ++slot) {
        const bool in = !a.parse_order || a.parse_order[slot] != ~0u;
        if (!in) continue;
        const uint32_t ent = a.parse_order ? a.parse_order[slot] : (uint32_t)slot;
        if (Spread && (ent >> 20) != 0) continue;
        const int pic = a.pic0 + (int)(Spread ? (ent & 0xfffffu) : ent);
        for (int w = 0; w < NW; ++w) {
            prog[w] = 0;
            if (!lane_init<false>(lanes[(size_t)w], P, lds[(size_t)w], a, pic, w, 0, Spread ? (1 << 20) : NW))
                lanes[(size_t)w].st = U_DONE;
            wins[(size_t)w].w = &wbuf[(size_t)w * 192];
            wins[(size_t)w].f = &wbuf[(size_t)w * 192 + 128];
        }
        const uint32_t lim = (P.bits_end + 64u) & ~3u;
        if (Spread)
            for (int w = 0; w < P.R; ++w) a.xprog[P.row_off + (uint32_t)w] = 0;
        Env E = Spread ? Env{&a, lds.data(), a.xprog + P.row_off, a.xctx + (size_t)P.row_off * CTX_PAD, 0}
                       : Env{&a, lds.data(), prog, wctx.data(), 0};
        for (;;) {
            bool any = false, progressed = false;
            for (int w = 0; w < NW; ++w) {
                Lane &L = lanes[(size_t)w];
                if (L.st == U_DONE) continue;
                any = true;
                E.lane = w;
                if (L.st == U_CTU && !ctu_ready<EG>(L, P, E)) continue;
                progressed = true;
                SoloWin &sw = wins[(size_t)w];
                const uint32_t start = L.st == U_CTU ? substream_start<EG>(L, P, a) : ~0u;
                if (start != ~0u) sw.restart(a.rbsp, start, lim, 0);
                else sw.advance(a.rbsp, L.lb, lim, 0);
                const EG G{lds[(size_t)w].ctx, 0u, 0u, seq, a.rbsp, lim, sw.view(), 0u, 0u, 0u};
                run_unit(L.st, L, lds[(size_t)w], P, E, G);
            }
            if (!any) break;
            if (!progressed) {
                for (int w = 0; w < NW; ++w)
                    if (lanes[(size_t)w].st != U_DONE) {
                        lanes[(size_t)w].status |= ST_SUBSTREAM_END;
                        atomicOr(&a.status[P.pic], lanes[(size_t)w].status);
                        lanes[(size_t)w].st = U_DONE;
                    }
                break;
            }
        }
    }
}

void emu_parse(const BatchArgs &a) {
    if (a.parse_mode == PARSE_SOLO) emu_parse_solo<false>(a);
    else if (a.parse_mode == PARSE_SPREAD) emu_parse_solo<true>(a);
    else if (a.lanes_lean) emu_parse_lanes<EngLean>(a);
    else emu_parse_lanes<Eng>(a);
}

}
```

### heif_amd/csrc/kernels/kernels.hpp

```cpp
#pragma once
#include "../common/desc.hpp"
#include "wave.hpp"
#include <cstdlib>
#include <vector>

#if defined(HG_HOST_EMU)
#include <atomic>
#include <thread>
#endif

namespace hg {

struct BatchArgs {
    const uint8_t *bits;
    const PicDesc *pics;
    const uint32_t *subs;
    uint8_t *rbsp;
    uint32_t *rsubs;
    const uint32_t *parse_order;
    int n_slots;
    const SeqParams *seqs;
    const uint8_t *sf;
    const OutImage *outs;
    TuRec *tus;
    Coef *coefs;
    uint32_t *row_counts;
    uint8_t *recon;
    int16_t *resid;
    uint8_t *maps;
    SaoParams *sao;
    uint32_t *status;
    int n_pics;
    int pic0;
    int max_width;
    int max_wctb;
    int max_rows;
    int total_rows;
    int bytes_per_sample;
    int chroma_format;
    int parse_group;
    int max_log2ctb;
    int lane_rows;
    int wpp_ring;
    int parse_mode;
    int solo_waves;
    uint32_t *xprog;
    uint8_t *xctx;
    uint32_t *xntu;
    uint32_t *xjob;
    int intra_stream;
    int stream_redo;
    uint32_t stream_patience_us;
    int has_assembly;
    int intra_split;
    int lanes_lean;
    int flags_from_recs;
};

struct ColorArgs {
    uint64_t plane[3];
    int32_t pitch[3];
    uint64_t rgb;
    int32_t rgb_pitch;
    int32_t w, h;
    int32_t out_w, out_h;
    int32_t rotation;
    int32_t chroma, shift;
    int32_t yoff, ys;
    int32_t cr_r, cb_g, cr_g, cb_b;
};
struct GatherArgs {
    uint64_t dst[3], src[3];
    int32_t dpitch[3], spitch[3];
    int32_t planes, bps;
    int32_t sx, sy;
    int32_t W, H;
    int32_t tw, th, cols, n_tiles, stride, offset;
};
inline void color_coefs(uint32_t matrix, bool full, ColorArgs &c) {
    double kr = 0.299, kb = 0.114;
    if (matrix == 1) kr = 0.2126, kb = 0.0722;
    else if (matrix == 9) kr = 0.2627, kb = 0.0593;
    const double kg = 1.0 - kr - kb;
    const double ys = full ? 1.0 : 255.0 / 219.0, cs = full ? 1.0 : 255.0 / 224.0;
    auto fx = [](double v) { return (int32_t)(v * 65536.0 + 0.5); };
    c.yoff = full ? 0 : 16;
    c.ys = fx(ys);
    c.cr_r = fx(2.0 * (1.0 - kr) * cs);
    c.cb_b = fx(2.0 * (1.0 - kb) * cs);
    c.cb_g = fx(2.0 * kb * (1.0 - kb) / kg * cs);
    c.cr_g = fx(2.0 * kr * (1.0 - kr) / kg * cs);
}

enum : int { RENDER_RGB8 = 0, RENDER_RGBA8 = 1, RENDER_RGB16 = 2, RENDER_RGBA16 = 3 };
constexpr int kRenderTile = 64;
constexpr int kRenderRowW = 256, kRenderRowH = 16;
struct RenderDesc {
    uint64_t plane[3];
    uint64_t alpha;
    uint64_t out;
    int32_t pitch[3], alpha_pitch, out_pitch;
    int32_t out_w, out_h;
    int32_t m[4], t[2];
    int32_t tiles_x, tiles;
    int32_t swap;
    int32_t chroma, shift;
    int32_t alpha_bps, alpha_shift;
    int32_t yoff, cmid, maxv;
    int32_t ys, cr_r, cb_g, cr_g, cb_b;
};
inline void render_coefs(uint32_t matrix, bool full, int depth, RenderDesc &d) {
    ColorArgs c{};
    color_coefs(matrix, full, c);
    if (depth > 8) {
        double kr = 0.299, kb = 0.114;
        if (matrix == 1) kr = 0.2126, kb = 0.0722;
        else if (matrix == 9) kr = 0.2627, kb = 0.0593;
        const double kg = 1.0 - kr - kb, top = double((1 << depth) - 1);
        const double ys = full ? 1.0 : top / double(219 << (depth - 8)), cs = full ? 1.0 : top / double(224 << (depth - 8));
        auto fx = [](double v) { return (int32_t)(v * 65536.0 + 0.5); };
        c.yoff = full ? 0 : 16 << (depth - 8);
        c.ys = fx(ys);
        c.cr_r = fx(2.0 * (1.0 - kr) * cs);
        c.cb_b = fx(2.0 * (1.0 - kb) * cs);
        c.cb_g = fx(2.0 * kb * (1.0 - kb) / kg * cs);
        c.cr_g = fx(2.0 * kr * (1.0 - kr) / kg * cs);
    }
    d.yoff = c.yoff;
    d.ys = c.ys;
    d.cr_r = c.cr_r;
    d.cb_g = c.cb_g;
    d.cr_g = c.cr_g;
    d.cb_b = c.cb_b;
    d.cmid = 1 << (depth - 1);
    d.maxv = (1 << depth) - 1;
}

constexpr int kScaleCols = 512;
constexpr int kScaleRowsA = 8, kScaleTile = 64;
struct ScaleDesc {
    RenderDesc r;
    int32_t ca, cb;
    int32_t oa, ob;
    int32_t ma, ta, mb, tb;
    int32_t na, nb, nb_log2;
    int32_t pad;
    uint64_t den;
    double inv_den;
};

enum : int { TENSOR_F32 = 0, TENSOR_F16 = 1, TENSOR_BF16 = 2 };
enum : int { TENSOR_CHW = 0, TENSOR_HWC = 1 };
struct TensorDesc {
    ScaleDesc s;
    int64_t stride_c, stride_y;
    int32_t elem, layout;
    float a[4], b[4];
};

enum : int { PARSE_AUTO = 0, PARSE_LANES = 1, PARSE_SOLO = 2, PARSE_SPREAD = 3 };
constexpr int kSoloMaxWaves = 16;
int lanes_parse_order(const PicDesc *pics, int n, int lane_rows, int ppw_force, std::vector<uint32_t> &order);
int lanes_pics_per_wave(int lane_rows, int n_pics);
constexpr int kStreamMaxPics = 192;
struct StreamKnobs {
    bool enabled = true;
    int max_pics = kStreamMaxPics;
    uint32_t patience_us = 200000;
};
StreamKnobs stream_knobs_from_env();
bool intra_stream_for(int parse_mode, int n_pics, bool has_assembly, const StreamKnobs &k);
int parse_mode_for(int requested, int n_pics, const PicDesc *pics = nullptr);
enum : int { LANES_GENERAL = 0, LANES_LEAN = 1 };
bool lanes_lean_eligible(const SeqParams *seqs, const PicDesc *pics, int n_pics, int wpp_ring);
int lanes_variant_for(const SeqParams *seqs, const PicDesc *pics, int n_pics, int wpp_ring);
int spread_parse_order(const PicDesc *pics, int n, std::vector<uint32_t> &order);
int solo_waves_for(int lane_rows);

#if defined(HG_HOST_EMU)
template <class K>
void emu_launch(K kernel, int gx, int gy, int waves, const BatchArgs &a, bool grid_stride = false,
                size_t dyn_lds = 0) {
    for (int by = 0; by < gy; ++by)
        for (int bx = 0; bx < (grid_stride ? 1 : gx); ++bx) {
            std::atomic<int> cnt{0}, gen{0};
            std::vector<std::thread> th;
            unsigned char *lds = dyn_lds ? static_cast<unsigned char *>(std::malloc(dyn_lds)) : nullptr;
            for (int w = 0; w < waves; ++w)
                th.emplace_back([&, w] {
                    g_emu.bidx = {unsigned(bx), unsigned(by), 0};
                    g_emu.tidx = {unsigned(grid_stride ? 0 : 64 * w), 0, 0};
                    g_emu.bdim = {unsigned(grid_stride ? 1 : 64 * waves), 1, 1};
                    g_emu.gdim = {unsigned(grid_stride ? 1 : gx), unsigned(gy), 1};
                    g_emu.bar_count = &cnt;
                    g_emu.bar_gen = &gen;
                    g_emu.bar_n = waves;
                    g_emu.smem = lds;
                    kernel(a);
                });
            for (auto &t : th) t.join();
            std::free(lds);
        }
}
void emu_rbsp(const BatchArgs &a);
void emu_parse(const BatchArgs &a);
void emu_transform(const BatchArgs &a);
void emu_intra(const BatchArgs &a);
void emu_deblock(const BatchArgs &a);
void emu_sao_out(const BatchArgs &a);
#else
hipError_t launch_rbsp(const BatchArgs &a, hipStream_t s);
hipError_t launch_ycbcr_rgb(const ColorArgs &c, int bytes_per_sample, hipStream_t s);
hipError_t launch_gather_tiles(const GatherArgs &g, hipStream_t s);
hipError_t launch_render(const RenderDesc *descs, int n_images, int max_tiles, int format, int bytes_per_sample,
                         hipStream_t s);
hipError_t launch_render_scaled(const ScaleDesc *descs, int n_images, int max_tiles, int format, int bytes_per_sample,
                                hipStream_t s);
hipError_t launch_render_tensor(const TensorDesc *descs, int n_images, int max_tiles, int format, int bytes_per_sample,
                                hipStream_t s);
hipError_t launch_parse(const BatchArgs &a, hipStream_t s);
hipError_t launch_parse_solo(const BatchArgs &a, hipStream_t s);
hipError_t launch_parse_lean(const BatchArgs &a, int waves, size_t lds_bytes, hipStream_t s);
hipError_t launch_transform(const BatchArgs &a, hipStream_t s);
hipError_t launch_intra(const BatchArgs &a, hipStream_t s);
hipError_t launch_deblock(const BatchArgs &a, hipStream_t s);
hipError_t launch_sao_out(const BatchArgs &a, hipStream_t s);
hipError_t launch_status_fold(const uint32_t *status, uint32_t *sticky, int n, hipStream_t s);
#endif

}
```

### heif_amd/csrc/kernels/parse_state.hpp

```cpp
#pragma once
#include "cabac.hpp"
#include "kernels.hpp"
#include "tables.hpp"

#include <algorithm>
#include <cstdint>
#include <vector>

#if defined(HG_HOST_EMU)
#include <cstdio>
#endif

#if !defined(HG_HOST_EMU)
extern "C" __device__ int hg_writelane(int src, int lane, int old) __asm("llvm.amdgcn.writelane.i32");
#endif
#if !defined(HG_NO_COLD_HINTS)
#define HG_UNLIKELY(x) __builtin_expect(!!(x), 0)
#define HG_LIKELY(x) __builtin_expect(!!(x), 1)
#else
#define HG_UNLIKELY(x) (x)
#define HG_LIKELY(x) (x)
#endif

namespace hg {

namespace {
__constant__ uint8_t c_lps_l[256] = {HG_LPS_TABLE};
__constant__ uint8_t c_trans_l[64] = {HG_TRANS_LPS};
__constant__ uint8_t c_ctx_init_l[CTX_NUM] = {HG_CTX_INIT_VALUES};
}
#if defined(HG_PARSE_PROF) && !defined(HG_HOST_EMU)
__device__ uint64_t g_prof_lanes[16];
constexpr int kCtuTimeCap = 1 << 17;
__device__ uint64_t g_ctu_t[kCtuTimeCap][3];
constexpr int kWaveRec = 4096, kWaveRecCap = 4096;
#endif

namespace {

HG_HD inline uint64_t state_row(int st) {
    uint64_t r = 0;
    for (int q = 0; q < 4; ++q) r |= (uint64_t)c_lps_l[(st << 2) | q] << (8 * q);
    const uint64_t lps_next = ((uint64_t)c_trans_l[st] << 1) | (st == 0 ? 1u : 0u);
    const uint64_t mps_next = (uint64_t)(st < 62 ? st + 1 : st) << 1;
    return r | (lps_next << 32) | (mps_next << 40);
}

constexpr int kTabRows = 128;
HG_HD inline uint64_t state_row_ctx(int s) {
    const uint64_t r = state_row(s >> 1);
    const uint64_t mps = (uint64_t)(s & 1);
    return (r & 0xffffffffull) | (((((r >> 32) & 0xffu) ^ mps) | ((mps ^ 1u) << 7)) << 32) |
           (((((r >> 40) & 0xffu) ^ mps) | (mps << 7)) << 40);
}

constexpr uint32_t kProgDone = 0x7fffffffu;
constexpr uint32_t PF_COHERENT = 1u << 31;

struct alignas(16) LaneLds {
    uint8_t ctx[CTX_PAD];
    uint8_t ipmL[16], ipmA[16];
    uint8_t dL[8], dA[8];
    int8_t qL[8], qA[8];
};

struct LanePic {
    int W, H, log2ctb, wctb, hctb, minCb, minTb, maxTb, maxDepthIntra, chroma;
    int log2qg, bdY, bdC, qpbdY, qpbdC, pcmMin, pcmMax, pcmBdY, pcmBdC, cbOff, crOff, sliceQp;
    int subx, suby;
    int w4, h4, w8, saoL, saoC;
    int R, lane0, ring;
    uint32_t flags, bits_off, bits_end, sub_first, row_off, tu_cap, coef_cap, pic;
    int8_t HG_GAS *gqpy;
    uint8_t HG_GAS *gflags;
    uint8_t HG_GAS *gdepth;
    SaoParams HG_GAS *gsao;
    TuRec HG_GAS *tu_base;
    Coef HG_GAS *coef_base;
};

enum Unit : int {
    U_DONE = 0,
    U_CTU,
    U_CQT,
    U_CU,
    U_TT,
    U_TB,
    U_SB,
    U_CTU_END,
    U_TBD,
};
constexpr int kPassKinds = 8;
HG_HD constexpr int pass_kind(int i) { return i < U_SB ? i + 1 : (i == U_SB ? (int)U_TBD : (int)U_CTU_END); }

enum : uint32_t {
    F_WPP = 1u << 0,
    F_FIRST_QG = 1u << 1,
    F_QG_NEW = 1u << 2,
    F_DQP_CODED = 1u << 3,
    F_BYPASS = 1u << 4,
    F_NXN = 1u << 5,
    F_CBF_L = 1u << 6,
    F_CBF_CB = 1u << 7,
    F_CBF_CR = 1u << 8,
    F_TS = 1u << 9,
    F_TB_CBF = 1u << 10,
    F_ANY_SB = 1u << 11,
    F_STOP = 1u << 12,
    F_PCM = 1u << 13,
    F_REINIT = 1u << 14,
};
constexpr uint32_t kMsegShift = 16, kMsegOne = 1u << kMsegShift;
constexpr uint32_t ST_SEGSW = 1u << 30;

struct Lane {
    uint32_t range, value;
    int k;
    uint64_t cur;
    int cn;
    uint32_t a0, a1, a2, a3, b0, b1, b2, b3, f0, f1, f2, f3;
    int ai, bv, fp;
    uint32_t lb;
    int32_t budget;
    uint32_t status;
    int st;
    uint32_t fl;
    int row, c, ctbx, ctby;
    int qx, qy, ql, qd;
    int tx, ty, tl, td;
    uint32_t tcbf;
    int qp_prev_last, qp_pred, cu_qp_delta_val, qpy_cur, qg_x, qg_y;
    int cu_modes, cu_chroma;
    int tb_t, tb_n, tb_cidx, tb_x, tb_y, tb_log2, tb_mode;
    uint32_t tb_coef0;
    int rc_scan, rc_last_sub, rc_last_pos, rc_i, rc_prev_c1;
    uint64_t rc_csbf;
    uint32_t ntu, ncoef;
    uint32_t nesc;
    uint32_t tu_row, coef_row;
    uint32_t cx;
    uint32_t reinit;
#if defined(HG_PARSE_PROF_SB)
    uint64_t psb[6];
#endif
};
#if defined(HG_PARSE_PROF_SB) && !defined(HG_HOST_EMU)
#define HG_PHASE_T(L, i, t0)                                                         \
    do {                                                                             \
        const uint64_t t_ = __builtin_amdgcn_s_memtime();                            \
        if ((int)__lane_id() == __builtin_ctzll(__ballot(1))) (L).psb[i] += t_ - (t0); \
        (t0) = t_;                                                                   \
    } while (0)
#endif
#if defined(HG_PARSE_PROF_SB) && !defined(HG_HOST_EMU) && !defined(HG_PARSE_PROF_TB)
#define HG_SB_T(L, i, t0) HG_PHASE_T(L, i, t0)
#elif defined(HG_PARSE_PROF_TB) && !defined(HG_HOST_EMU)
#define HG_SB_T(L, i, t0) ((void)(t0))
#else
#define HG_SB_T(L, i, t0) ((void)0)
#endif
#if defined(HG_PARSE_PROF_TB) && !defined(HG_HOST_EMU)
#define HG_TB_T0(t0) uint64_t t0 = __builtin_amdgcn_s_memtime()
#define HG_TB_T(L, i, t0) HG_PHASE_T(L, i, t0)
#else
#define HG_TB_T0(t0) ((void)0)
#define HG_TB_T(L, i, t0) ((void)0)
#endif

enum Cov : int {
    COV_TB_LUMA,
    COV_TB_CHROMA = COV_TB_LUMA + 4,
    COV_NXN = COV_TB_CHROMA + 4,
    COV_NXN_MPM,
    COV_NXN_REM = COV_NXN_MPM + 3,
    COV_DQP,
    COV_DQP_EG0,
    COV_LAST_SUFFIX,
    COV_CODED_AFTER_EMPTY,
    COV_CU_ENDS_IN_SB,
    COV_TSKIP,
    COV_LAST_CTX5,
    COV_N,
    COV_SB_SIG4 = COV_N,
    COV_SB_SIG,
    COV_SB_BEYOND8,
    COV_SB_RICE4,
    COV_SB_ESCAPE,
    COV_SB_EGK,
    COV_SB_HIDE,
    COV_SB_NO_HIDE,
    COV_SB_CTXSET_INC,
    COV_SB_INFER_DC,
    COV_SB_LAST_POS0,
    COV_SB_GT2,
    COV_SB_RUN_ANY4,
    COV_SB_RUN_NO4,
    COV_SB_END,
    COV_LAST_00 = COV_SB_END,
    COV_LAST_0M,
    COV_LAST_M0,
    COV_LAST_MM,
    COV_LAST_SUFFIX_X_ONLY,
    COV_LAST_SUFFIX_Y_ONLY,
    COV_LAST_SWAP,
    COV_ALL
};
#if defined(HG_HOST_EMU)
long g_cov[COV_ALL];
#define HG_COV(i) (++g_cov[i])
#else
#define HG_COV(i) ((void)0)
#endif

HG_HD inline size_t lane_blocks_bytes(int n) { return (sizeof(LaneLds) * (size_t)n + 15) & ~(size_t)15; }

#if !defined(HG_HOST_EMU) && defined(HG_PARSE_PROF)
int prof_read(uint64_t *out, int n) {
    uint64_t tmp[16] = {};
    if (hipMemcpyFromSymbol(tmp, HIP_SYMBOL(hg::g_prof_lanes), sizeof(tmp)) != hipSuccess) return -1;
    const uint64_t zero[16] = {};
    if (hipMemcpyToSymbol(HIP_SYMBOL(hg::g_prof_lanes), zero, sizeof(zero)) != hipSuccess) return -1;
#if defined(HG_PARSE_PROF_SB)
    const int head = 16;
#else
    const int head = 8;
#endif
    for (int k = 0; k < n && k < head; ++k) out[k] = tmp[k];
    if (n <= head) return n < head ? n : head;
    const size_t m = std::min((size_t)(n - head), (size_t)hg::kCtuTimeCap * 3);
    if (hipMemcpyFromSymbol(out + head, HIP_SYMBOL(hg::g_ctu_t), m * sizeof(uint64_t)) != hipSuccess) return -1;
    std::vector<uint64_t> z((size_t)hg::kCtuTimeCap * 3, 0);
    if (hipMemcpyToSymbol(HIP_SYMBOL(hg::g_ctu_t), z.data(), z.size() * sizeof(uint64_t)) != hipSuccess) return -1;
    return (int)(head + m);
}
#endif

}
}
```

### heif_amd/csrc/kernels/parse_units.hpp

```cpp
#pragma once
#include "parse_engine.hpp"

namespace hg {
namespace {

HG_HD inline int mode422(int m) {
    constexpr uint32_t t[9] = {0x02020100u, 0x05030202u, 0x0b0a0807u, 0x12100f0du, 0x16151413u,
                               0x18181717u, 0x1b1a1919u, 0x1d1c1c1bu, 0x001f1e1du};
    return (int)((t[m >> 2] >> (8 * (m & 3))) & 0xffu);
}

HG_HD inline int chroma_qp_map(int qpi, int chroma) {
    if (chroma != 1) return qpi < 51 ? qpi : 51;
    if (qpi < 30) return qpi;
    if (qpi > 43) return qpi - 6;
    return qpi < 34 ? qpi - 1 : 33 + ((qpi - 34) >> 1);
}

HG_HD inline void update_qpy(Lane &L, const LanePic &P) {
    L.qpy_cur = ((L.qp_pred + L.cu_qp_delta_val + 52 + 2 * P.qpbdY) % (52 + P.qpbdY)) - P.qpbdY;
}

HG_HD inline void derive_qp_pred(Lane &L, const LaneLds &ld, const LanePic &P) {
    int prev;
    const bool first_in_ctb = L.qg_x == L.ctbx && L.qg_y == L.ctby;
    if (L.fl & F_FIRST_QG) {
        prev = P.sliceQp;
        L.fl &= ~F_FIRST_QG;
    } else if ((L.fl & F_WPP) && first_in_ctb && L.c == 0) {
        prev = P.sliceQp;
    } else {
        prev = L.qp_prev_last;
    }
    const int mask = (1 << P.log2ctb) - 1;
    const int qa = (L.qg_x & mask) ? ld.qL[(L.qg_y - L.ctby) >> 3] : prev;
    const int qb = (L.qg_y & mask) ? ld.qA[(L.qg_x - L.ctbx) >> 3] : prev;
    L.qp_pred = (qa + qb + 1) >> 1;
}

HG_HD inline int derive_luma_mode(const Lane &L, const LaneLds &ld, int xPb, int yPb, int prev, int mpm_idx,
                                  int rem) {
    const int ca = xPb <= 0 ? 1 : ld.ipmL[(yPb - L.ctby) >> 2];
    const int cb = (yPb - 1 < L.ctby) ? 1 : ld.ipmA[(xPb - L.ctbx) >> 2];
    int l0, l1, l2;
    if (ca == cb) {
        if (ca < 2) {
            l0 = 0;
            l1 = 1;
            l2 = 26;
        } else {
            l0 = ca;
            l1 = 2 + ((ca + 29) % 32);
            l2 = 2 + ((ca - 2 + 1) % 32);
        }
    } else {
        l0 = ca;
        l1 = cb;
        if (ca != 0 && cb != 0) l2 = 0;
        else if (ca != 1 && cb != 1) l2 = 1;
        else l2 = 26;
    }
    if (prev) return mpm_idx == 0 ? l0 : (mpm_idx == 1 ? l1 : l2);
    int t;
    if (l0 > l1) { t = l0; l0 = l1; l1 = t; }
    if (l0 > l2) { t = l0; l0 = l2; l2 = t; }
    if (l1 > l2) { t = l1; l1 = l2; l2 = t; }
    int m = rem;
    if (m >= l0) ++m;
    if (m >= l1) ++m;
    if (m >= l2) ++m;
    return m;
}

HG_HD inline uint64_t scan4_word(int scan) { return scan == 0 ? kScan4Pos[0] : (scan == 1 ? kScan4Pos[1] : kScan4Pos[2]); }
template <class EG>
HG_HD inline int scan_pos(const EG &G, int l, int scan, int i) {
    if (l == 3) return G.scan8(scan, i);
    if (l == 0) return 0;
    const uint64_t t = l == 2 ? scan4_word(scan) : (scan == 0 ? kScan2Pos[0] : (scan == 1 ? kScan2Pos[1] : kScan2Pos[2]));
    const uint32_t e = (uint32_t)(t >> (4 * i)) & 15u;
    return (int)((e & 3) | ((e >> 2) << 4));
}
template <class EG>
HG_HD inline int scan_inv(const EG &G, int l, int scan, int raster) {
    if (l == 3) return G.scan8_inv(scan, raster);
    if (l == 0) return 0;
    const uint64_t t = l == 2 ? (scan == 0 ? kScan4Inv[0] : (scan == 1 ? kScan4Inv[1] : kScan4Inv[2]))
                              : (scan == 0 ? kScan2Inv[0] : (scan == 1 ? kScan2Inv[1] : kScan2Inv[2]));
    return (int)((uint32_t)(t >> (4 * raster)) & 15u);
}

constexpr uint64_t sig_pat_nib(int pc) {
    uint64_t w = 0;
    for (int e = 0; e < 16; ++e) {
        const int x = e & 3, y = e >> 2;
        const int v = pc == 0 ? (x + y == 0 ? 2 : (x + y < 3 ? 1 : 0))
                    : pc == 1 ? (y == 0 ? 2 : (y == 1 ? 1 : 0))
                    : pc == 2 ? (x == 0 ? 2 : (x == 1 ? 1 : 0)) : 2;
        w |= (uint64_t)(v + 1) << (4 * e);
    }
    return w;
}
HG_HD inline uint64_t sig_slots(int pcs) {
    return pcs == 0 ? sig_pat_nib(0) : pcs == 1 ? sig_pat_nib(1) : pcs == 2 ? sig_pat_nib(2) : sig_pat_nib(3);
}
HG_HD inline int msb32(uint32_t m) { return 31 - __builtin_clz(m); }

HG_HD inline uint64_t sig_seq(int idx) {
    const int scan = idx / 5, pat = idx % 5;
    const uint64_t slots = pat == 4 ? kSigCtxMap4 : sig_slots(pat);
    const uint64_t sw = scan4_word(scan);
    uint64_t q = 0;
    for (int n = 0; n < 16; ++n) {
        const int e = (int)((sw >> (4 * n)) & 15u);
        q |= ((slots >> (4 * e)) & 15u) << (4 * n);
    }
    return q;
}

HG_HD inline void scan8_tables(uint8_t *t, int lane) {
    t[lane] = kScanPos[3][0][lane];
    t[64 + lane] = kScanInv[3][0][lane];
}

struct Env {
    const BatchArgs *a;
    LaneLds *lds;
    uint32_t *prog;
    uint8_t *wctx;
    int lane;
};

HG_HD inline uint8_t *wpp_stage(const Env &E, const LanePic &P, int row) {
    return E.wctx + (size_t)(P.lane0 + row % P.R) * CTX_PAD;
}
HG_HD inline uint32_t *prog_word(const Env &E, const LanePic &P, int row) { return &E.prog[P.lane0 + row % P.R]; }

template <class EG>
HG_HD inline bool wpp_ready(const Lane &L, const LanePic &P, const Env &E) {
    if (!(L.fl & F_WPP) || L.row == 0) return true;
    const int ahead = L.c == 0 ? 2 : L.c + 1;
    const uint32_t need = (uint32_t)(L.row - 1) * (uint32_t)P.wctb + (uint32_t)(ahead < P.wctb ? ahead : P.wctb);
    const uint32_t *pw = prog_word(E, P, L.row - 1);
    return (EG::kSpread ? load_agent(pw) : prog_load(pw)) >= need;
}

template <class EG>
HG_HD inline uint32_t lanes_nmid(const LanePic &P) { return (pic_flags<EG>(P) >> PD_NMID_SHIFT) & PD_NMID_MAX; }

template <class EG>
HG_HD inline uint32_t substream_start(const Lane &L, const LanePic &P, const BatchArgs &a) {
    if (L.c != 0) {
        if constexpr (!EG::kSolo && !EG::kLean) {
            if (L.status & ST_SEGSW) {
                const uint32_t m = L.fl >> kMsegShift;
                return P.bits_off +
                       (a.rsubs[P.sub_first + (uint32_t)P.hctb + (m < lanes_nmid<EG>(P) ? 1u + m : 0u)] & SUB_OFFSET);
            }
        }
        return ~0u;
    }
    if ((L.fl & F_WPP) || L.row == 0)
        return P.bits_off + (a.rsubs[P.sub_first + ((L.fl & F_WPP) ? L.row : 0)] & SUB_OFFSET);
    if (pic_flags<EG>(P) & SP_ROW_SEGMENTS) {
        const uint32_t e = a.rsubs[P.sub_first + L.row];
        if (!(e & SUB_CONTINUE)) return P.bits_off + (e & SUB_OFFSET);
    }
    return ~0u;
}

HG_HD inline void row_outputs(Lane &L, const LanePic &P) {
    L.tu_row = (uint32_t)L.row * P.tu_cap;
    L.coef_row = (uint32_t)L.row * P.coef_cap;
    L.ntu = L.ncoef = L.nesc = 0;
}

template <class EG>
HG_HD inline void coef_push(Lane &L, const LanePic &P, uint32_t w) {
    if (pic_flags<EG>(P) & PF_COHERENT) store_word_agent((uint32_t *)(P.coef_base + L.coef_row + L.ncoef++), w);
    else P.coef_base[L.coef_row + L.ncoef++] = w;
}

template <class EG>
HG_HD inline void unit_ctu(Lane &L, LaneLds &ld, LanePic &P, const Env &E, const EG &G) {
    if (!wpp_ready<EG>(L, P, E)) return;
    L.ctbx = L.c << P.log2ctb;
    L.ctby = L.row << P.log2ctb;
    const uint32_t start = substream_start<EG>(L, P, *E.a);
    if (HG_UNLIKELY(start != ~0u)) {
        const bool segsw = !EG::kSolo && !EG::kLean && (L.status & ST_SEGSW) != 0;
        const bool init = !segsw && (L.row == 0 || ((L.fl & F_WPP) && P.wctb < 2));
        const bool wpp_copy = !init && (L.fl & F_WPP);
        if constexpr (EG::kCtxReg) {
#if !defined(HG_HOST_EMU)
            const int ln = (int)__lane_id();
            uint32_t w = L.cx;
            if (init) {
                w = 0;
                for (int b = 0; b < 4; ++b) {
                    const int i = 4 * ln + b;
                    if (i < CTX_NUM) w |= (uint32_t)ctx_init_state(c_ctx_init_l[i], P.sliceQp) << (8 * b);
                }
            } else if (wpp_copy) {
                w = 0;
                if (ln < CTX_PAD / 4) {
                    const uint8_t *src = (EG::kSpread || pic_ring<EG>(P)) ? wpp_stage(E, P, L.row) : ld.ctx;
                    const uint32_t *sw = reinterpret_cast<const uint32_t *>(src) + ln;
                    w = EG::kSpread ? load_agent(sw) : *sw;
                }
            }
            L.cx = w;
#endif
        } else if (init) {
#pragma nounroll
            for (int i = 0; i < CTX_NUM; ++i) ld.ctx[i] = ctx_init_state(c_ctx_init_l[i], P.sliceQp);
        } else if (wpp_copy && (EG::kSpread || pic_ring<EG>(P))) {
            const uint32_t *src = reinterpret_cast<const uint32_t *>(wpp_stage(E, P, L.row));
            uint32_t *dst = reinterpret_cast<uint32_t *>(ld.ctx);
#pragma nounroll
            for (int k = 0; k < CTX_PAD / 4; ++k) dst[k] = EG::kSpread ? load_agent(src + k) : src[k];
        }
        engine_init(L, G, start, P.bits_end);
        if (segsw) {
            L.status &= ~ST_SEGSW;
            if ((L.fl >> kMsegShift) >= lanes_nmid<EG>(P)) L.status |= ST_SUBSTREAM_END;
            L.fl += kMsegOne;
        } else {
            if (L.row == 0) L.fl |= F_FIRST_QG;
            if constexpr (!EG::kSolo) {
                const uint32_t nm = lanes_nmid<EG>(P);
                if ((L.fl & F_WPP) && nm)
                    L.fl = (L.fl & (kMsegOne - 1)) |
                           (E.a->subs[P.sub_first + (uint32_t)P.hctb + 1u + nm + L.row] << kMsegShift);
            }
        }
    }
    if (P.saoL || P.saoC) {
        int ml = 0, mu = 0;
        if (L.c > 0) ml = dec(L, G, CTX_SAO_MERGE);
        if (L.row > 0 && !ml) mu = dec(L, G, CTX_SAO_MERGE);
        uint32_t *dst = reinterpret_cast<uint32_t *>(P.gsao + (size_t)L.row * P.wctb + L.c);
        uint32_t w0 = 0, w1 = 0, w2 = 0, w3 = 0, w4 = 0, w5 = 0, w6 = 0, w7 = 0;
        if (ml || mu) {
            const uint32_t *src = ml ? dst - 8 : reinterpret_cast<const uint32_t *>(P.gsao + (size_t)(L.row - 1) * P.wctb + L.c);
            w0 = load_word_coherent(src + 0);
            w1 = load_word_coherent(src + 1);
            w2 = load_word_coherent(src + 2);
            w3 = load_word_coherent(src + 3);
            w4 = load_word_coherent(src + 4);
            w5 = load_word_coherent(src + 5);
            w6 = load_word_coherent(src + 6);
            w7 = load_word_coherent(src + 7);
        } else {
            auto put8 = [&](int b, uint32_t v) {
                const uint32_t m = (v & 0xffu) << (8 * (b & 3));
                switch (b >> 2) {
                case 0: w0 |= m; break;
                case 1: w1 |= m; break;
                case 2: w2 |= m; break;
                case 3: w3 |= m; break;
                case 4: w4 |= m; break;
                case 5: w5 |= m; break;
                case 6: w6 |= m; break;
                default: w7 |= m; break;
                }
            };
            auto put16 = [&](int b, int v) {
                put8(b, (uint32_t)v);
                put8(b + 1, (uint32_t)v >> 8);
            };
            const int ncomp = HG_PIC_CHROMA(P) ? 3 : 1;
            int type1 = 0, eo1 = 0;
#pragma unroll
            for (int cc = 0; cc < 3; ++cc) {
                if (cc >= ncomp) break;
                if (!((P.saoL && cc == 0) || (P.saoC && cc > 0))) continue;
                const int type = cc < 2 ? (dec(L, G, CTX_SAO_TYPE) ? (byp(L, G) ? 2 : 1) : 0) : type1;
                if (cc == 1) type1 = type;
                put8(cc, (uint32_t)type);
                if (!type) continue;
                const int bd = cc ? P.bdC : P.bdY;
                const int cmax = (1 << ((bd < 10 ? bd : 10) - 5)) - 1;
                int o[4];
#pragma unroll
                for (int i = 0; i < 4; ++i) {
                    int v = 0;
                    while (v < cmax && byp(L, G)) ++v;
                    o[i] = v;
                }
                int band_eo;
                if (type == 1) {
#pragma unroll
                    for (int i = 0; i < 4; ++i)
                        if (o[i] && byp(L, G)) o[i] = -o[i];
                    band_eo = (int)byp_bits(L, G, 5);
                } else {
                    band_eo = cc < 2 ? (int)byp_bits(L, G, 2) : eo1;
                    if (cc == 1) eo1 = band_eo;
                    o[2] = -o[2];
                    o[3] = -o[3];
                }
                put8(3 + cc, (uint32_t)band_eo);
#pragma unroll
                for (int i = 0; i < 4; ++i) put16(6 + 8 * cc + 2 * i, o[i]);
            }
        }
        const uint32_t w[8] = {w0, w1, w2, w3, w4, w5, w6, w7};
#pragma unroll
        for (int k = 0; k < 8; ++k) {
            if constexpr (EG::kSpread) store_agent(dst + k, w[k]);
            else dst[k] = w[k];
        }
    }
    L.qx = L.ctbx, L.qy = L.ctby, L.ql = P.log2ctb, L.qd = 0;
    L.st = U_CQT;
}

template <class EG>
HG_HD inline void unit_cqt(Lane &L, LaneLds &ld, LanePic &P, const EG &G) {
    for (;;) {
        const int n = 1 << L.ql;
        bool split;
        if (L.qx + n <= P.W && L.qy + n <= P.H && L.ql > P.minCb) {
            int cond = 0;
            if (L.qx > 0 && ld.dL[(L.qy - L.ctby) >> 3] > L.qd) ++cond;
            if (L.qy > 0) {
                const int ad = (L.qy - 1 < L.ctby)
                                   ? load_byte_coherent(P.gdepth + (size_t)(L.row - 1) * P.w8 + (L.qx >> 3))
                                   : ld.dA[(L.qx - L.ctbx) >> 3];
                if (ad > L.qd) ++cond;
            }
            split = dec(L, G, CTX_SPLIT_CU + cond) != 0;
        } else {
            split = L.ql > P.minCb;
        }
        if (L.ql >= P.log2qg) {
            L.fl = (L.fl & ~F_DQP_CODED) | F_QG_NEW;
            L.cu_qp_delta_val = 0;
            L.qg_x = L.qx;
            L.qg_y = L.qy;
        }
        if (!split) break;
        --L.ql;
        ++L.qd;
    }
    L.st = U_CU;
}

HG_HD inline void cu_done(Lane &L, LaneLds &ld, LanePic &P);
template <class EG>
HG_HD inline void tu_emit(Lane &L, const LanePic &P);

template <class EG>
HG_HD inline void pcm_cu(Lane &L, LaneLds &ld, LanePic &P, const EG &G) {
    const int n = 1 << L.ql;
    {
        const int nb = n >> 2, by = (L.qy - L.ctby) >> 2, bx = (L.qx - L.ctbx) >> 2;
        for (int k = 0; k < nb; ++k) {
            ld.ipmL[by + k] = 1;
            ld.ipmA[bx + k] = 1;
        }
    }
    uint32_t bit = (uint32_t)(8 * (int32_t)P.bits_end - L.budget - L.k + 7) & ~7u;
    L.fl = (L.fl | F_PCM | F_TB_CBF) & ~F_TS;
    const int ntb = HG_PIC_CHROMA(P) == 0 ? 1 : (HG_PIC_CHROMA(P) == 2 ? 5 : 3), nh = HG_PIC_CHROMA(P) == 2 ? 2 : 1;
    for (int t = 0; t < ntb; ++t) {
        const int c = t == 0 ? 0 : 1 + (t - 1) / nh, h = t == 0 ? 0 : (t - 1) % nh;
        const int l2 = (c && HG_PIC_CHROMA(P) != 3) ? L.ql - 1 : L.ql, m = 1 << l2;
        const int pbd = c ? P.pcmBdC : P.pcmBdY, sh = (c ? P.bdC : P.bdY) - pbd;
        L.tb_cidx = c;
        L.tb_x = c ? L.qx >> HG_PIC_SUBX(P) : L.qx;
        L.tb_y = c ? (L.qy >> HG_PIC_SUBY(P)) + (h << l2) : L.qy;
        L.tb_log2 = l2;
        L.tb_mode = 1;
        L.tb_coef0 = L.ncoef;
#pragma nounroll
        for (int i = 0; i < m * m; ++i) {
            const uint32_t b = (bit >> 3) < G.lim ? bit >> 3 : G.lim;
            const uint32_t w = ((uint32_t)G.rbsp[b] << 16) | ((uint32_t)G.rbsp[b + 1] << 8) | (uint32_t)G.rbsp[b + 2];
            const uint32_t v = (w >> (24u - (bit & 7u) - (uint32_t)pbd)) & ((1u << pbd) - 1u);
            bit += (uint32_t)pbd;
            if (L.ncoef + L.nesc < P.coef_cap) coef_push<EG>(L, P, ((v << sh) << 16) | (uint32_t)i);
            else L.status |= ST_CAPACITY;
        }
        tu_emit<EG>(L, P);
    }
    L.fl &= ~(F_PCM | F_TB_CBF);
    {
        const int nb = n >> 2, gx0 = L.qx >> 2, gy0 = L.qy >> 2;
        const int wx = gx0 + nb <= P.w4 ? nb : P.w4 - gx0, hy = gy0 + nb <= P.h4 ? nb : P.h4 - gy0;
        const uint64_t nf = ((L.fl & F_BYPASS) || (pic_flags<EG>(P) & SP_PCM_LOOP_FILTER_DISABLED)) ? MF_NOFILT : 0;
        const uint64_t rep = 0x0101010101010101ull;
        for (int y = 0; y < hy; ++y) {
            uint8_t *row = P.gflags + (size_t)(gy0 + y) * P.w4 + gx0;
            const uint64_t h = (y == 0 ? (uint64_t)MF_EDGE_H : 0u) | nf;
            store_bytes(row, wx, (rep * h) | (uint64_t)MF_EDGE_V);
        }
    }
    const uint32_t next = bit >> 3;
    if (next > P.bits_end) L.status |= ST_OVERRUN;
    if constexpr (EG::kSolo) {
        L.reinit = next;
        L.lb = next >> 2;
        L.fl |= F_REINIT;
    } else {
        engine_init(L, G, next, P.bits_end);
    }
    cu_done(L, ld, P);
}

template <class EG>
HG_HD inline void unit_cu(Lane &L, LaneLds &ld, LanePic &P, const EG &G) {
    if (L.fl & F_QG_NEW) {
        derive_qp_pred(L, ld, P);
        L.fl &= ~F_QG_NEW;
    }
    update_qpy(L, P);
    L.fl &= ~(F_BYPASS | F_NXN);
    if ((pic_flags<EG>(P) & SP_TQ_BYPASS) && dec(L, G, CTX_TQ_BYPASS)) L.fl |= F_BYPASS;
    if (L.ql == P.minCb && !dec(L, G, CTX_PART_MODE)) L.fl |= F_NXN;
    const bool nxn = (L.fl & F_NXN) != 0;
    const bool pcm = !nxn && (pic_flags<EG>(P) & SP_PCM) && L.ql >= P.pcmMin && L.ql <= P.pcmMax && term(L, G);
    {
        const int nd = 1 << (L.ql - 3);
        const int dy = (L.qy - L.ctby) >> 3, dx = (L.qx - L.ctbx) >> 3;
        for (int k = 0; k < nd; ++k) {
            ld.dL[dy + k] = (uint8_t)L.qd;
            ld.dA[dx + k] = (uint8_t)L.qd;
        }
    }
    if constexpr (!EG::kLean) {
        if (pcm) {
            pcm_cu(L, ld, P, G);
            return;
        }
    }
    const int np = nxn ? 4 : 1;
    const int pb = nxn ? 1 << (L.ql - 1) : 1 << L.ql;
    if (nxn) HG_COV(COV_NXN);
    int prev = 0;
    if constexpr (!EG::kSolo) {
        uint32_t t = ctx_ld(L, G, CTX_PREV_INTRA);
        for (int i = 0; i < np; ++i) prev |= dec_t(L, G, t & 0x7fu, t) << i;
        ctx_st(L, G, CTX_PREV_INTRA, t & 0x7fu);
    } else {
        for (int i = 0; i < np; ++i) prev |= dec(L, G, CTX_PREV_INTRA) << i;
    }
    int modes = 0;
    for (int i = 0; i < np; ++i) {
        const int p = (prev >> i) & 1;
        int mpm = 0, rem = 0;
        if constexpr (EG::kSolo) {
            if (p) mpm = byp(L, G) ? (byp(L, G) ? 2 : 1) : 0;
            else rem = (int)byp_bits(L, G, 5);
        } else {
            mpm = rem = byp_luma_mode(L, G, p);
        }
        if (nxn) HG_COV(p ? COV_NXN_MPM + mpm : COV_NXN_REM);
        const int xPb = L.qx + (i & 1) * pb, yPb = L.qy + (i >> 1) * pb;
        const int m = derive_luma_mode(L, ld, xPb, yPb, p, mpm, rem);
        modes |= m << (8 * i);
        const int nb = pb >> 2, by = (yPb - L.ctby) >> 2, bx = (xPb - L.ctbx) >> 2;
        for (int k = 0; k < nb; ++k) {
            ld.ipmL[by + k] = (uint8_t)m;
            ld.ipmA[bx + k] = (uint8_t)m;
        }
    }
    L.cu_modes = modes;
    if (HG_PIC_CHROMA(P)) {
        const int nc = HG_PIC_CHROMA(P) == 3 ? np : 1;
        int cms = 0;
        for (int i = 0; i < nc; ++i) {
            const int icpm = dec(L, G, CTX_CHROMA_MODE) ? (int)byp_bits(L, G, 2) : 4;
            const int lm = (modes >> (8 * i)) & 0xff;
            int cm;
            if (icpm == 4) {
                cm = lm;
            } else {
                cm = icpm == 0 ? 0 : (icpm == 1 ? 26 : (icpm == 2 ? 10 : 1));
                if (cm == lm) cm = 34;
            }
            if (HG_PIC_CHROMA(P) == 2) cm = mode422(cm);
            cms |= cm << (8 * i);
        }
        L.cu_chroma = nc == 1 ? (int)((uint32_t)cms * 0x01010101u) : cms;
    }
    L.tx = L.qx, L.ty = L.qy, L.tl = L.ql, L.td = 0, L.tcbf = 0;
    L.st = U_TT;
}

#if defined(HG_FLAGS_IN_PARSE)
template <class EG>
constexpr bool kFlagsInParse = true;
#else
template <class EG>
constexpr bool kFlagsInParse = EG::kSolo;
#endif

template <class EG>
HG_HD inline void unit_tt(Lane &L, LaneLds &ld, LanePic &P, const EG &G) {
    HG_TB_T0(ttt);
    const bool nxn = (L.fl & F_NXN) != 0;
    const int max_depth = P.maxDepthIntra + (nxn ? 1 : 0);
    for (;;) {
        bool split;
        if (L.tl <= P.maxTb && L.tl > P.minTb && L.td < max_depth && !(nxn && L.td == 0))
            split = dec(L, G, CTX_SPLIT_TF + 5 - L.tl) != 0;
        else
            split = L.tl > P.maxTb || (nxn && L.td == 0);
        uint32_t cbf = 0;
        if ((L.tl > 2 && HG_PIC_CHROMA(P)) || HG_PIC_CHROMA(P) == 3) {
            const uint32_t pc = L.td == 0 ? 3u : (L.tcbf >> (4 * (L.td - 1))) & 3u;
            const bool two = HG_PIC_CHROMA(P) == 2 && (!split || L.tl == 3);
            if (pc & 1) {
                cbf |= (uint32_t)dec(L, G, CTX_CBF_CHROMA + L.td);
                if (two) cbf |= (uint32_t)dec(L, G, CTX_CBF_CHROMA + L.td) << 2;
            }
            if (pc & 2) {
                cbf |= (uint32_t)dec(L, G, CTX_CBF_CHROMA + L.td) << 1;
                if (two) cbf |= (uint32_t)dec(L, G, CTX_CBF_CHROMA + L.td) << 3;
            }
        }
        L.tcbf = (L.tcbf & ~(15u << (4 * L.td))) | (cbf << (4 * L.td));
        if (!split) break;
        --L.tl;
        ++L.td;
    }
    const uint32_t cbf = (L.tcbf >> (4 * L.td)) & 15u;
    L.fl &= ~F_CBF_L;
    if (dec(L, G, CTX_CBF_LUMA + (L.td == 0 ? 1 : 0))) L.fl |= F_CBF_L;
    const bool chroma4 = (HG_PIC_CHROMA(P) == 1 || HG_PIC_CHROMA(P) == 2) && L.tl == 2;
    const uint32_t pc = L.td > 0 ? (L.tcbf >> (4 * (L.td - 1))) & 15u : 0u;
    const bool cbf_c = HG_PIC_CHROMA(P) == 0 ? false : (chroma4 ? pc != 0 : cbf != 0);
    if (((L.fl & F_CBF_L) || cbf_c) && (pic_flags<EG>(P) & SP_CU_QP_DELTA) && !(L.fl & F_DQP_CODED)) {
        int v = 0;
        if constexpr (!EG::kSolo) {
            v = dec(L, G, CTX_CU_QP_DELTA);
            if (v) {
                uint32_t t = ctx_ld(L, G, CTX_CU_QP_DELTA + 1);
                while (v < 5 && dec_t(L, G, t & 0x7fu, t)) ++v;
                ctx_st(L, G, CTX_CU_QP_DELTA + 1, t & 0x7fu);
            }
        } else {
            while (v < 5 && dec(L, G, CTX_CU_QP_DELTA + (v == 0 ? 0 : 1))) ++v;
        }
        HG_COV(COV_DQP);
        if (v == 5) {
            HG_COV(COV_DQP_EG0);
            int ones = 0;
            bool bad = false;
            while (byp(L, G)) {
                if (++ones > 31) {
                    bad = true;
                    break;
                }
            }
            if (bad) L.status |= ST_SYNTAX;
            else v += (int)(((1u << ones) - 1u) + byp_bits(L, G, ones));
        }
        if (v && byp(L, G)) v = -v;
        const int vlo = -(26 + P.qpbdY / 2), vhi = 25 + P.qpbdY / 2;
        if (HG_UNLIKELY(v < vlo || v > vhi)) {
            L.status |= ST_SYNTAX;
            v = v < vlo ? vlo : vhi;
        }
        L.fl |= F_DQP_CODED;
        L.cu_qp_delta_val = v;
        update_qpy(L, P);
    }
    HG_TB_T(L, 3, ttt);
    if constexpr (kFlagsInParse<EG>) {
        const int nb = 1 << (L.tl - 2), gx0 = L.tx >> 2, gy0 = L.ty >> 2;
        const int wx = gx0 + nb <= P.w4 ? nb : P.w4 - gx0, hy = gy0 + nb <= P.h4 ? nb : P.h4 - gy0;
        const uint64_t nf = (lane_fl<EG>(L) & F_BYPASS) ? MF_NOFILT : 0;
        const uint64_t rep = 0x0101010101010101ull;
        for (int y = 0; y < hy; ++y) {
            uint8_t *row = P.gflags + (size_t)(gy0 + y) * P.w4 + gx0;
            const uint64_t h = (y == 0 ? (uint64_t)MF_EDGE_H : 0u) | nf;
            store_bytes(row, wx, (rep * h) | (uint64_t)MF_EDGE_V);
        }
    }
    HG_TB_T(L, 4, ttt);
    const int blk = L.td == 0 ? 0 : (((L.tx >> L.tl) & 1) | (((L.ty >> L.tl) & 1) << 1));
    L.tb_n = (HG_PIC_CHROMA(P) != 0 && (!chroma4 || blk == 3)) ? (HG_PIC_CHROMA(P) == 2 ? 5 : 3) : 1;
    L.tb_t = 0;
    L.st = U_TB;
}

template <class EG>
HG_HD inline void tu_emit(Lane &L, const LanePic &P) {
    const uint32_t fl = lane_fl<EG>(L);
    int qp;
    if (L.tb_cidx == 0) {
        qp = L.qpy_cur + P.qpbdY;
    } else {
        const int off = L.tb_cidx == 1 ? P.cbOff : P.crOff;
        int qpi = L.qpy_cur + off;
        qpi = qpi < -P.qpbdC ? -P.qpbdC : (qpi > 57 ? 57 : qpi);
        qp = chroma_qp_map(qpi, HG_PIC_CHROMA(P)) + P.qpbdC;
    }
    uint32_t f = (uint32_t)L.tb_cidx;
    if (fl & F_TB_CBF) f |= TU_CBF;
    if (fl & F_TS) f |= TU_TSKIP;
    if (fl & F_BYPASS) f |= TU_BYPASS;
    if (fl & F_PCM) f |= TU_PCM | TU_BYPASS;
    if (L.tb_cidx == 0 && L.tb_log2 == 2) f |= TU_DST;
    if (HG_LIKELY(L.ntu < P.tu_cap)) {
        const uint32_t w0 = (uint32_t)L.tb_x | ((uint32_t)L.tb_y << 16);
        const uint32_t w1 = (uint32_t)L.tb_log2 | (f << 8) | ((uint32_t)L.tb_mode << 16) | ((uint32_t)(uint8_t)qp << 24);
        const uint32_t w3 = (L.ncoef - L.tb_coef0) | ((uint32_t)L.c << 16);
        if (pic_flags<EG>(P) & PF_COHERENT) store_tu_agent(P.tu_base + L.tu_row + L.ntu, w0, w1, L.tb_coef0, w3);
        else store_tu(P.tu_base + L.tu_row + L.ntu, w0, w1, L.tb_coef0, w3);
        ++L.ntu;
    } else {
        L.status |= ST_CAPACITY;
    }
}

HG_HD inline void cu_done(Lane &L, LaneLds &ld, LanePic &P);

template <class EG>
HG_HD inline void tb_done(Lane &L, LaneLds &ld, LanePic &P) {
    tu_emit<EG>(L, P);
    if (++L.tb_t < L.tb_n) {
        L.st = U_TB;
        return;
    }
    while (L.td > 0) {
        const int s = 1 << L.tl;
        const int b = ((L.tx >> L.tl) & 1) | (((L.ty >> L.tl) & 1) << 1);
        if (b < 3) {
            const int px = L.tx & ~(2 * s - 1), py = L.ty & ~(2 * s - 1);
            L.tx = px + ((b + 1) & 1) * s;
            L.ty = py + ((b + 1) >> 1) * s;
            L.st = U_TT;
            return;
        }
        L.tx &= ~(2 * s - 1);
        L.ty &= ~(2 * s - 1);
        ++L.tl;
        --L.td;
    }
    cu_done(L, ld, P);
}

HG_HD inline void cu_done(Lane &L, LaneLds &ld, LanePic &P) {
    HG_TB_T0(tcu);
    {
        const int n = 1 << L.ql, nd = n >> 3;
        const int dy = (L.qy - L.ctby) >> 3, dx = (L.qx - L.ctbx) >> 3;
        for (int k = 0; k < nd; ++k) {
            ld.qL[dy + k] = (int8_t)L.qpy_cur;
            ld.qA[dx + k] = (int8_t)L.qpy_cur;
        }
        const int nb = n >> 2, gx0 = L.qx >> 2, gy0 = L.qy >> 2;
        const int wx = gx0 + nb <= P.w4 ? nb : P.w4 - gx0, hy = gy0 + nb <= P.h4 ? nb : P.h4 - gy0;
        for (int y = 0; y < hy; ++y) {
            int8_t *row = P.gqpy + (size_t)(gy0 + y) * P.w4 + gx0;
            store_bytes(reinterpret_cast<uint8_t *>(row), wx, 0x0101010101010101ull * (uint8_t)L.qpy_cur);
        }
        L.qp_prev_last = L.qpy_cur;
    }
    HG_TB_T(L, 5, tcu);
    while (L.qd > 0) {
        const int s = 1 << L.ql;
        const int px = L.qx & ~(2 * s - 1), py = L.qy & ~(2 * s - 1);
        for (int b = (((L.qx >> L.ql) & 1) | (((L.qy >> L.ql) & 1) << 1)) + 1; b < 4; ++b) {
            const int cx = px + (b & 1) * s, cy = py + (b >> 1) * s;
            if (cx < P.W && cy < P.H) {
                L.qx = cx;
                L.qy = cy;
                L.st = U_CQT;
                return;
            }
        }
        L.qx = px;
        L.qy = py;
        ++L.ql;
        --L.qd;
    }
    L.st = U_CTU_END;
}

template <class EG>
HG_HD inline void unit_tb(Lane &L, LaneLds &ld, LanePic &P, const EG &G) {
    HG_TB_T0(ttb);
    const int t = L.tb_t;
    const bool chroma4 = (HG_PIC_CHROMA(P) == 1 || HG_PIC_CHROMA(P) == 2) && L.tl == 2;
    const bool c422 = HG_PIC_CHROMA(P) == 2;
    const int comp = t == 0 ? 0 : (c422 ? 1 + ((t - 1) >> 1) : t), half = (c422 && t > 0) ? (t - 1) & 1 : 0;
    bool cbf;
    L.tb_cidx = comp;
    if (t == 0) {
        L.tb_x = L.tx;
        L.tb_y = L.ty;
        L.tb_log2 = L.tl;
        int k = 0;
        if (L.fl & F_NXN) {
            const int half = 1 << (L.ql - 1);
            k = ((L.ty - L.qy) >= half ? 2 : 0) + ((L.tx - L.qx) >= half ? 1 : 0);
        }
        L.tb_mode = (L.cu_modes >> (8 * k)) & 0xff;
        cbf = (L.fl & F_CBF_L) != 0;
    } else if (!chroma4) {
        L.tb_log2 = HG_PIC_CHROMA(P) == 3 ? L.tl : L.tl - 1;
        L.tb_x = L.tx >> HG_PIC_SUBX(P);
        L.tb_y = (L.ty >> HG_PIC_SUBY(P)) + (half << L.tb_log2);
        int k = 0;
        if (HG_PIC_CHROMA(P) == 3 && (L.fl & F_NXN)) {
            const int hp = 1 << (L.ql - 1);
            k = ((L.ty - L.qy) >= hp ? 2 : 0) + ((L.tx - L.qx) >= hp ? 1 : 0);
        }
        L.tb_mode = (L.cu_chroma >> (8 * k)) & 0xff;
        cbf = ((L.tcbf >> (4 * L.td + (comp - 1) + 2 * half)) & 1u) != 0;
    } else {
        const int s = 1 << (L.tl + 1);
        L.tb_x = (L.tx & ~(s - 1)) >> 1;
        L.tb_y = ((L.ty & ~(s - 1)) >> HG_PIC_SUBY(P)) + 4 * half;
        L.tb_log2 = 2;
        L.tb_mode = L.cu_chroma & 0xff;
        cbf = ((L.tcbf >> (4 * (L.td - 1) + (comp - 1) + 2 * half)) & 1u) != 0;
    }
    L.fl = (L.fl & ~(F_TS | F_TB_CBF)) | (cbf ? F_TB_CBF : 0u);
    L.tb_coef0 = L.ncoef;
    if (!cbf) {
        if constexpr (EG::kSolo) tb_done<EG>(L, ld, P);
        else L.st = U_TBD;
        return;
    }
    const int l2 = L.tb_log2, n = 1 << l2, cidx = comp;
    HG_COV((cidx ? COV_TB_CHROMA : COV_TB_LUMA) + l2 - 2);
    if (t == 1 && !(L.fl & F_CBF_L)) HG_COV(COV_CODED_AFTER_EMPTY);
    if ((pic_flags<EG>(P) & SP_TRANSFORM_SKIP) && !(L.fl & F_BYPASS) && l2 == 2 && dec(L, G, CTX_TS_FLAG + (cidx ? 1 : 0)))
        L.fl |= F_TS;
    if (L.fl & F_TS) HG_COV(COV_TSKIP);
    const int cmax = (l2 << 1) - 1;
    const int off = cidx == 0 ? 3 * (l2 - 2) + ((l2 - 1) >> 2) : 15;
    const int shift = cidx == 0 ? (l2 + 1) >> 2 : l2 - 2;
    int px = 0, py = 0;
    HG_TB_T(L, 0, ttb);
    while (px < cmax && dec(L, G, CTX_LAST_X + off + (px >> shift))) ++px;
    while (py < cmax && dec(L, G, CTX_LAST_Y + off + (py >> shift))) ++py;
    HG_TB_T(L, 1, ttb);
    int lx = px, ly = py;
    if (px > 3 || py > 3) HG_COV(COV_LAST_SUFFIX);
    if (px > 8 || py > 8) HG_COV(COV_LAST_CTX5);
    if ((px == 0 || px == cmax) && (py == 0 || py == cmax)) HG_COV(COV_LAST_00 + (px ? 2 : 0) + (py ? 1 : 0));
    if ((px > 3) != (py > 3)) HG_COV(px > 3 ? COV_LAST_SUFFIX_X_ONLY : COV_LAST_SUFFIX_Y_ONLY);
    if (px > 3) {
        const int k = (px >> 1) - 1;
        lx = (1 << k) * (2 + (px & 1)) + (int)byp_bits(L, G, k);
    }
    if (py > 3) {
        const int k = (py >> 1) - 1;
        ly = (1 << k) * (2 + (py & 1)) + (int)byp_bits(L, G, k);
    }
    int scan = 0;
    if (l2 == 2 || (l2 == 3 && (cidx == 0 || HG_PIC_CHROMA(P) == 3))) {
        if (L.tb_mode >= 6 && L.tb_mode <= 14) scan = 2;
        else if (L.tb_mode >= 22 && L.tb_mode <= 30) scan = 1;
    }
    if (scan == 2) {
        HG_COV(COV_LAST_SWAP);
        const int tt = lx;
        lx = ly;
        ly = tt;
    }
    if (HG_UNLIKELY(lx >= n || ly >= n)) {
        L.status |= ST_SYNTAX;
        lx &= n - 1;
        ly &= n - 1;
    }
    const int sbl = l2 - 2, sbw = 1 << sbl;
    L.rc_scan = scan;
    L.rc_last_sub = scan_inv(G, sbl, scan, (ly >> 2) * sbw + (lx >> 2));
    L.rc_last_pos = scan_inv(G, 2, scan, (ly & 3) * 4 + (lx & 3));
    L.rc_csbf = 0;
    L.rc_prev_c1 = 1;
    L.fl &= ~F_ANY_SB;
    L.rc_i = L.rc_last_sub;
    L.st = U_SB;
    HG_TB_T(L, 2, ttb);
}

template <bool Scalar = false>
HG_HD inline uint64_t spread16_nib(uint32_t m) {
#if !defined(HG_HOST_EMU) && defined(__HIP_DEVICE_COMPILE__)
    if constexpr (Scalar) {
        uint64_t x2, x4;
        asm("s_bitreplicate_b64_b32 %0, %1" : "=s"(x2) : "s"(uni32(m & 0xffffu)));
        asm("s_bitreplicate_b64_b32 %0, %1" : "=s"(x4) : "s"((uint32_t)x2));
        return x4 & 0x1111111111111111ull;
    }
#endif
    uint64_t x = m & 0xffffu;
    x = (x | (x << 24)) & 0x000000ff000000ffull;
    x = (x | (x << 12)) & 0x000f000f000f000full;
    x = (x | (x << 6)) & 0x0303030303030303ull;
    x = (x | (x << 3)) & 0x1111111111111111ull;
    return x;
}

template <class EG>
constexpr bool kSbVec = !EG::kSolo;

HG_HD inline uint64_t spread16_nib_halves(uint32_t m) {
    auto half = [](uint32_t x) {
        x = (x | (x << 12)) & 0x000f000fu;
        x = (x | (x << 6)) & 0x03030303u;
        x = (x | (x << 3)) & 0x11111111u;
        return x;
    };
    return (uint64_t)half(m & 0xffu) | ((uint64_t)half((m >> 8) & 0xffu) << 32);
}

template <class EG, class L_, class P_>
HG_HD inline void sb_store(L_ &L, const P_ &P, uint32_t sig, uint32_t signs, uint64_t nib, int xS, int yS, bool hide,
                           uint32_t nesc0) {
    uint32_t esc0;
    if constexpr (kSbVec<EG>) {
        esc0 = P.coef_cap - 1 - nesc0;
    } else {
        const uint32_t nesc_sb =
            (uint32_t)__builtin_popcountll(nib & (nib >> 1) & (nib >> 2) & (nib >> 3) & 0x1111111111111111ull);
        esc0 = P.coef_cap - 1 - (L.nesc - nesc_sb);
    }
    const uint32_t w0 = (sig & 0xffffu) | (signs & 0xffff0000u);
    const uint32_t w3 = (uint32_t)xS | ((uint32_t)yS << 3) | ((uint32_t)L.rc_scan << 6) | (hide ? 1u << 8 : 0u) |
                        (esc0 << 9);
    if (HG_LIKELY(L.ncoef + L.nesc + 4 <= P.coef_cap)) {
        TuRec *d = (TuRec *)(P.coef_base + L.coef_row + L.ncoef);
        if (pic_flags<EG>(P) & PF_COHERENT) store_tu_agent(d, w0, (uint32_t)nib, (uint32_t)(nib >> 32), w3);
        else store_tu(d, w0, (uint32_t)nib, (uint32_t)(nib >> 32), w3);
        L.ncoef += 4;
    } else {
        L.status |= ST_CAPACITY;
    }
}

template <class EG>
HG_HD inline void unit_sb(Lane &L, LaneLds &ld, LanePic &P, const EG &G) {
#if defined(HG_PARSE_PROF_SB) && !defined(HG_HOST_EMU)
    uint64_t tsb = __builtin_amdgcn_s_memtime();
#endif
    const int l2 = L.tb_log2, cidx = L.tb_cidx, i = L.rc_i;
    const int sbl = l2 - 2, sbw = 1 << sbl;
    const int sp = scan_pos(G, sbl, L.rc_scan, i);
    const int xS = sp & 15, yS = sp >> 4;
    int pcs = 0;
    if (xS < sbw - 1) pcs |= (int)((L.rc_csbf >> (yS * 8 + xS + 1)) & 1);
    if (yS < sbw - 1) pcs |= (int)((L.rc_csbf >> ((yS + 1) * 8 + xS)) & 1) << 1;
    bool coded = true, infer_dc = false;
    if (i < L.rc_last_sub && i > 0) {
        coded = dec(L, G, CTX_CSBF + ((pcs & 1) | (pcs >> 1)) + (cidx ? 2 : 0)) != 0;
        infer_dc = true;
    }
    uint32_t sig = 0;
    if (coded) {
        L.rc_csbf |= 1ull << (yS * 8 + xS);
        int nstart = 15;
        if (i == L.rc_last_sub) {
            sig = 1u << L.rc_last_pos;
            nstart = L.rc_last_pos - 1;
        }
        const int cbase = CTX_SIG + (cidx ? 27 : 0);
        auto cb = [&](int i) { return ctx_ld(L, G, cbase + i); };
        uint64_t seq = G.seqw(L.rc_scan * 5 + (l2 == 2 ? 4 : pcs));
        uint32_t c0 = 0, c1 = 0, c2 = 0;
        constexpr bool kCc7 = !EG::kSolo;
        uint64_t cc = 0;
        int off = 0;
        if (l2 == 2) {
            if constexpr (kCc7) {
                for (int k = 0; k < 9; ++k) cc |= (uint64_t)cb(k) << (7 * k);
            } else {
                c0 = cb(0) | (cb(1) << 8) | (cb(2) << 16) | (cb(3) << 24);
                c1 = cb(4) | (cb(5) << 8) | (cb(6) << 16) | (cb(7) << 24);
                c2 = cb(8);
            }
        } else {
            off = cidx == 0 ? ((xS | yS) ? 3 : 0) + (l2 == 3 ? (L.rc_scan == 0 ? 9 : 15) : 21) : (l2 == 3 ? 9 : 12);
            if ((xS | yS) == 0) seq &= ~0xfull;
            if constexpr (kCc7)
                cc = (uint64_t)cb(0) | ((uint64_t)cb(off) << 7) | ((uint64_t)cb(off + 1) << 14) |
                     ((uint64_t)cb(off + 2) << 21);
            else
                c0 = cb(0) | (cb(off) << 8) | (cb(off + 1) << 16) | (cb(off + 2) << 24);
        }
        HG_SB_T(L, 0, tsb);
        if constexpr (EG::kSolo) {
          if (l2 > 2) {
            auto dec_slot4 = [&](uint32_t slot) -> uint32_t {
                const uint32_t sh = slot * 8u;
                uint32_t cs = (c0 >> sh) & 0xffu;
                const uint32_t bin = (uint32_t)dec_s(L, G, cs);
                c0 = (c0 & ~(0xffu << sh)) | (cs << sh);
                return bin;
            };
            uint32_t sg = sig;
            for (int nn = nstart; nn > 0; --nn) sg |= dec_slot4((uint32_t)(seq >> (4 * nn)) & 3u) << nn;
            if (nstart >= 0) sg |= (infer_dc && sg == 0) ? 1u : dec_slot4((uint32_t)seq & 3u);
            sig = sg;
          } else {
            uint64_t cc = (uint64_t)c0 | ((uint64_t)c1 << 32);
            auto dec_slot = [&](uint32_t slot) -> uint32_t {
                const uint32_t sh = (slot & 7u) * 8u;
                const bool hi = slot >= 8u;
                uint32_t cs = hi ? c2 : (uint32_t)(cc >> sh) & 0xffu;
                const uint32_t bin = (uint32_t)dec_s(L, G, cs);
                const uint64_t ncc = (cc & ~(0xffull << sh)) | ((uint64_t)cs << sh);
                cc = hi ? cc : ncc;
                c2 = hi ? cs : c2;
                return bin;
            };
            uint32_t sg = sig;
            for (int nn = nstart; nn > 0; --nn) sg |= dec_slot((uint32_t)(seq >> (4 * nn)) & 15u) << nn;
            if (nstart >= 0) sg |= (infer_dc && sg == 0) ? 1u : dec_slot((uint32_t)seq & 15u);
            sig = sg;
            c0 = (uint32_t)cc;
            c1 = (uint32_t)(cc >> 32);
          }
        } else {
            auto dec_slot = [&](int slot) -> uint32_t {
                if constexpr (kCc7) {
                    const uint32_t sh = (uint32_t)slot * 7u;
                    const uint64_t m = 0x7full << sh;
                    uint32_t t;
                    const uint32_t bin = (uint32_t)dec_t(L, G, (uint32_t)(cc >> sh) & 0x7fu, t);
                    const uint64_t tv = (uint64_t)t << sh;
                    cc = (uint64_t)bfi32((uint32_t)m, (uint32_t)tv, (uint32_t)cc) |
                         ((uint64_t)bfi32((uint32_t)(m >> 32), (uint32_t)(tv >> 32), (uint32_t)(cc >> 32)) << 32);
                    return bin;
                } else {
                    uint32_t cs = cache_get(c0, c1, c2, slot);
                    const uint32_t bin = (uint32_t)dec_s(L, G, cs);
                    cache_put(c0, c1, c2, slot, cs);
                    return bin;
                }
            };
            if constexpr (kCc7) {
                uint64_t sq = nstart > 0 ? seq << (4 * (15 - nstart)) : 0ull;
                for (int nn = nstart; nn > 0; --nn) {
                    sig |= dec_slot((int)(uint32_t)(sq >> 60)) << nn;
                    sq <<= 4;
                }
            } else {
                for (int nn = nstart; nn > 0; --nn) sig |= dec_slot((int)((seq >> (4 * nn)) & 15u)) << nn;
            }
            if (nstart >= 0) {
                HG_COV(l2 == 2 ? COV_SB_SIG4 : COV_SB_SIG);
                if (infer_dc && sig == 0) {
                    HG_COV(COV_SB_INFER_DC);
                    sig |= 1u;
                } else {
                    sig |= dec_slot((int)(seq & 15u));
                }
            } else {
                HG_COV(COV_SB_LAST_POS0);
            }
        }
        auto cw = [&](int i, uint32_t v) { ctx_st(L, G, cbase + i, v & 0xffu); };
        if constexpr (kCc7) {
            if (l2 == 2) {
                for (int k = 0; k < 9; ++k) cw(k, (uint32_t)(cc >> (7 * k)) & 0x7fu);
            } else {
                cw(0, (uint32_t)cc & 0x7fu);
                cw(off, (uint32_t)(cc >> 7) & 0x7fu);
                cw(off + 1, (uint32_t)(cc >> 14) & 0x7fu);
                cw(off + 2, (uint32_t)(cc >> 21) & 0x7fu);
            }
        } else if (l2 == 2) {
            for (int k = 0; k < 4; ++k) cw(k, c0 >> (8 * k));
            for (int k = 0; k < 4; ++k) cw(4 + k, c1 >> (8 * k));
            cw(8, c2);
        } else {
            cw(0, c0);
            cw(off, c0 >> 8);
            cw(off + 1, c0 >> 16);
            cw(off + 2, c0 >> 24);
        }
#if defined(HG_PARSE_PROF_SB) && !defined(HG_PARSE_PROF_TB) && !defined(HG_HOST_EMU)
        L.psb[4] += (uint64_t)(nstart + 1);
#endif
        HG_SB_T(L, 1, tsb);
    }
    if (sig) {
        int ctx_set = (i == 0 || cidx > 0) ? 0 : 2;
        if ((L.fl & F_ANY_SB) && L.rc_prev_c1 == 0) {
            HG_COV(COV_SB_CTXSET_INC);
            ++ctx_set;
        }
        L.fl |= F_ANY_SB;
        int c1 = 1;
        uint32_t g1 = 0, g2 = 0;
        const int gbase = CTX_GT1 + ctx_set * 4 + (cidx ? 16 : 0);
        uint32_t gc = ctx_ld(L, G, gbase) | (ctx_ld(L, G, gbase + 1) << 8) | (ctx_ld(L, G, gbase + 2) << 16) |
                      (ctx_ld(L, G, gbase + 3) << 24);
        const int first_sig = 31 - __builtin_clz(sig & (0u - sig));
        const int last_sig = msb32(sig);
        int num_g1 = 0, last_g1 = -1;
        uint32_t beyond8 = sig;
        if constexpr (EG::kSolo) {
            uint32_t &m = beyond8;
            for (int j = 0; j < 8 && m; ++j) {
                const int nn = msb32(m);
                m ^= 1u << nn;
                const uint32_t gs = (uint32_t)(c1 < 3 ? c1 : 3) * 8u;
                uint32_t cs = (gc >> gs) & 0xffu;
                const uint32_t f = (uint32_t)dec_s(L, G, cs);
                gc = (gc & ~(0xffu << gs)) | (cs << gs);
                g1 |= f << nn;
                c1 = (c1 > 0 && !f) ? c1 + 1 : 0;
            }
            last_g1 = g1 ? msb32(g1) : -1;
        } else {
            for (uint32_t &m = beyond8; m && num_g1 < 8;) {
                const int nn = msb32(m);
                m &= ~(1u << nn);
                const int gs = g1 ? 0 : (num_g1 < 2 ? num_g1 + 1 : 3) * 8;
                const uint32_t gm = 0x7fu << gs;
                uint32_t t;
                const int f = dec_t(L, G, (gc >> gs) & 0xffu, t);
                gc = bfi32(gm, t << gs, gc);
                ++num_g1;
                g1 |= (uint32_t)f << nn;
            }
            c1 = g1 ? 0 : 1 + num_g1;
            last_g1 = g1 ? msb32(g1) : -1;
        }
        L.rc_prev_c1 = c1;
        for (int k = 0; k < 4; ++k) ctx_st(L, G, gbase + k, (gc >> (8 * k)) & 0xffu);
        if (last_g1 >= 0 && dec(L, G, CTX_GT2 + ctx_set + (cidx ? 4 : 0))) g2 = 1u << last_g1;
        if (g2) HG_COV(COV_SB_GT2);
        if (beyond8) HG_COV(COV_SB_BEYOND8);
        HG_SB_T(L, 2, tsb);
        const bool sign_hidden = !(lane_fl<EG>(L) & F_BYPASS) && (last_sig - first_sig > 3);
        const bool hide = (pic_flags<EG>(P) & SP_SIGN_HIDING) && sign_hidden;
        if (pic_flags<EG>(P) & SP_SIGN_HIDING) HG_COV(hide ? COV_SB_HIDE : COV_SB_NO_HIDE);
        const int nsign = __builtin_popcount(sig) - (hide ? 1 : 0);
        uint32_t signs = byp_bits(L, G, nsign);
        signs = nsign ? signs << (32 - nsign) : 0u;
        [[maybe_unused]] const uint32_t nesc0 = L.nesc;
        uint64_t nib;
        if constexpr (kSbVec<EG>) {
            nib = spread16_nib_halves(g1);
        } else {
            nib = spread16_nib<EG::kSolo>(g1) + (g2 ? 1ull << (4 * last_g1) : 0ull);
        }
        {
            const uint32_t lastb = last_g1 >= 0 ? 1u << last_g1 : 0u;
            uint32_t need = (g1 & ~lastb) | g2 | beyond8;
            int last_abs = 0, last_rice = 0;
            bool first_rem = true;
            [[maybe_unused]] int rice = 0;
            while (need) {
                const int nn = msb32(need);
                need ^= 1u << nn;
                const int g1b = (int)((g1 >> nn) & 1);
                const int base = 1 + g1b + (int)((g2 >> nn) & 1);
                int k;
                if constexpr (kSbVec<EG>) {
                    k = rice;
                } else if (first_rem) {
                    k = 0;
                    first_rem = false;
                } else {
                    k = last_rice + (last_abs > 3 * (1 << last_rice) ? 1 : 0);
                    k = k < 4 ? k : 4;
                }
                int rem = byp_rem(L, G, k);
                if (HG_UNLIKELY(rem < 0)) {
                    const int lim = 31 - (k + 1);
                    int ones = 0;
                    for (;;) {
                        const int mm = lim + 1 - ones < 8 ? lim + 1 - ones : 8;
                        const int pz = byp_unary(L, G, mm);
                        ones += pz;
                        if (pz < mm || ones > lim) break;
                    }
                    if (ones > lim) {
                        L.status |= ST_SYNTAX;
                        rem = 0;
                    } else {
                        rem = (int)((4u << k) + (((1u << ones) - 1u) << (k + 1)) + byp_bits(L, G, ones + k + 1));
                    }
                    HG_COV(COV_SB_EGK);
                }
                if (k == 4) HG_COV(COV_SB_RICE4);
                last_abs = base + rem;
                last_rice = k;
                const int am1 = base - 1 + rem;
                if constexpr (kSbVec<EG>) {
                    const int inc = last_abs > (3 << k) ? 1 : 0;
                    rice = k + inc < 4 ? k + inc : 4;
                    nib += (uint64_t)(uint32_t)((am1 < 15 ? am1 : 15) - g1b) << (4 * nn);
                } else {
                    nib = (nib & ~(0xfull << (4 * nn))) | ((uint64_t)(am1 < 15 ? am1 : 15) << (4 * nn));
                }
                if (HG_UNLIKELY(am1 >= 15)) {
                    HG_COV(COV_SB_ESCAPE);
                    if (L.ncoef + L.nesc + 4 < P.coef_cap) {
                        Coef HG_GAS *e = P.coef_base + L.coef_row + P.coef_cap - 1 - L.nesc;
                        if (pic_flags<EG>(P) & PF_COHERENT) store_word_agent((uint32_t *)e, (uint32_t)last_abs);
                        else *e = (uint32_t)last_abs;
                    } else {
                        L.status |= ST_CAPACITY;
                    }
                    ++L.nesc;
                }
            }
        }
        HG_SB_T(L, 3, tsb);
        sb_store<EG>(L, P, sig, signs, nib, xS, yS, hide, nesc0);
    }
    if (--L.rc_i < 0) {
        if (L.tb_t + 1 >= L.tb_n && L.tx + (1 << L.tl) == L.qx + (1 << L.ql) && L.ty + (1 << L.tl) == L.qy + (1 << L.ql))
            HG_COV(COV_CU_ENDS_IN_SB);
        if constexpr (EG::kSolo) tb_done<EG>(L, ld, P);
        else L.st = U_TBD;
    }
}

template <class EG>
HG_HD inline void unit_ctu_end(Lane &L, LaneLds &ld, LanePic &P, const Env &E, const EG &G) {
    if ((L.fl & F_WPP) && L.c == 1 && L.row + 1 < P.hctb) {
        uint32_t *dst = reinterpret_cast<uint32_t *>((EG::kSpread || pic_ring<EG>(P)) ? wpp_stage(E, P, L.row + 1)
                                                                              : E.lds[P.lane0 + (L.row + 1) % P.R].ctx);
        if constexpr (EG::kCtxReg) {
#if !defined(HG_HOST_EMU)
            const int ln = (int)__lane_id();
            if (ln < CTX_PAD / 4) {
                if constexpr (EG::kSpread) store_agent(dst + ln, L.cx);
                else dst[ln] = L.cx;
            }
#endif
        } else {
            const uint32_t *src = reinterpret_cast<const uint32_t *>(ld.ctx);
#pragma nounroll
            for (int k = 0; k < CTX_PAD / 4; ++k) {
                if constexpr (EG::kSpread) store_agent(dst + k, src[k]);
                else dst[k] = src[k];
            }
        }
    }
    {
        const int nb8 = 1 << (P.log2ctb - 3), col0 = L.ctbx >> 3;
        uint8_t *line = P.gdepth + (size_t)L.row * P.w8;
        for (int k = 0; k < nb8 && col0 + k < P.w8; ++k) {
            if constexpr (EG::kSpread) store_agent(line + col0 + k, ld.dA[k]);
            else line[col0 + k] = ld.dA[k];
        }
    }
    const bool last_in_pic = L.row == P.hctb - 1 && L.c == P.wctb - 1;
    const bool seg_end = !last_in_pic && L.c == P.wctb - 1 && (pic_flags<EG>(P) & SP_ROW_SEGMENTS) &&
                         (E.a->rsubs[P.sub_first + L.row] & SUB_SEG_END);
    const bool eos = (last_in_pic && !(pic_flags<EG>(P) & SP_SUBSET_END)) || seg_end;
    if (term(L, G) != (eos ? 1 : 0)) {
        if constexpr (EG::kSolo || EG::kLean) L.status |= ST_SUBSTREAM_END;
        else L.status |= (!eos && L.c < P.wctb - 1 && lanes_nmid<EG>(P)) ? ST_SEGSW : (uint32_t)ST_SUBSTREAM_END;
    }
    if (!eos && (last_in_pic || ((L.fl & F_WPP) && L.c == P.wctb - 1)) && !term(L, G)) L.status |= ST_SUBSTREAM_END;
    if (L.budget + L.k < 0) L.status |= ST_OVERRUN;
    ++L.c;
    const uint32_t pv = (L.fl & F_STOP) ? kProgDone : (uint32_t)L.row * (uint32_t)P.wctb + (uint32_t)L.c;
    if constexpr (EG::kSpread) {
        if (E.a->xntu) {
            HG_REL_AGENT();
            store_agent(E.a->xntu + P.row_off + L.row, L.ntu);
        }
        stores_done();
        store_agent(prog_word(E, P, L.row), pv);
    } else {
        release_fence();
        prog_store(prog_word(E, P, L.row), pv);
    }
    if (!(L.fl & F_STOP) && L.c < P.wctb) {
        L.st = U_CTU;
        return;
    }
    uint32_t *rc = E.a->row_counts + 2 * (size_t)(P.row_off + L.row);
    rc[0] = L.ntu;
    rc[1] = L.ncoef;
    const int step = (L.fl & F_WPP) ? P.R : 1;
    if (!(L.fl & F_STOP) && L.row + step < P.hctb) {
        L.row += step;
        L.c = 0;
        row_outputs(L, P);
        L.st = U_CTU;
        return;
    }
    const uint32_t st_rep = EG::kSolo ? L.status : (L.status & ~ST_SEGSW);
    if (st_rep) atomicOr(&E.a->status[P.pic], st_rep);
    L.st = U_DONE;
}

template <class EG>
HG_HD inline void run_unit(int kind, Lane &L, LaneLds &ld, LanePic &P, const Env &E, const EG &G) {
    if constexpr (EG::kSolo) {
        if (L.fl & F_REINIT) {
            engine_init(L, G, L.reinit, P.bits_end);
            L.fl &= ~F_REINIT;
        }
    }
    switch (kind) {
    case U_SB: unit_sb(L, ld, P, G); break;
    case U_TB: unit_tb(L, ld, P, G); break;
    case U_TT: unit_tt(L, ld, P, G); break;
    case U_CU: unit_cu(L, ld, P, G); break;
    case U_CQT: unit_cqt(L, ld, P, G); break;
    case U_CTU: unit_ctu(L, ld, P, E, G); break;
    case U_CTU_END: unit_ctu_end(L, ld, P, E, G); break;
    case U_TBD:
        if constexpr (!EG::kSolo) tb_done<EG>(L, ld, P);
        break;
    default: break;
    }
}

template <class EG = Eng>
HG_HD inline bool ctu_ready(const Lane &L, const LanePic &P, const Env &E) { return wpp_ready<EG>(L, P, E); }

template <bool Mid = true>
HG_HD inline bool pic_init(LanePic &P, const BatchArgs &a, int pic, int lane0, int cap) {
    const PicDesc &pd = a.pics[pic];
    if (pd.flags & PD_ASSEMBLY) return false;
    const SeqParams &sp = a.seqs[pd.seq];
    const int log2ctb = sp.log2_ctb, ctb = 1 << log2ctb;
    const int hctb = (sp.height + ctb - 1) >> log2ctb;
    const bool wpp = (sp.flags & SP_WPP) != 0;
    const int R = wpp ? (hctb < cap ? hctb : cap) : 1;
    P.R = R;
    P.lane0 = lane0;
    P.ring = wpp && hctb > R;
    P.W = sp.width;
    P.H = sp.height;
    P.log2ctb = log2ctb;
    P.wctb = (sp.width + ctb - 1) >> log2ctb;
    P.hctb = hctb;
    P.minCb = sp.log2_min_cb;
    P.minTb = sp.log2_min_tb;
    P.maxTb = sp.log2_max_tb;
    P.maxDepthIntra = sp.max_th_depth_intra;
    P.chroma = sp.chroma_format;
    P.subx = (sp.chroma_format == 1 || sp.chroma_format == 2) ? 1 : 0;
    P.suby = sp.chroma_format == 1 ? 1 : 0;
    P.log2qg = log2ctb - sp.diff_cu_qp_delta_depth;
    P.bdY = sp.bit_depth_y;
    P.bdC = sp.bit_depth_c;
    P.qpbdY = 6 * (sp.bit_depth_y - 8);
    P.qpbdC = 6 * (sp.bit_depth_c - 8);
    P.pcmMin = sp.log2_min_pcm;
    P.pcmMax = sp.log2_max_pcm;
    P.pcmBdY = sp.pcm_bd_y;
    P.pcmBdC = sp.pcm_bd_c;
    P.cbOff = sp.cb_qp_offset + pd.cb_qp_off;
    P.crOff = sp.cr_qp_offset + pd.cr_qp_off;
    P.sliceQp = pd.slice_qp;
    P.w4 = (sp.width + 3) >> 2;
    P.h4 = (sp.height + 3) >> 2;
    P.w8 = (sp.width + 7) >> 3;
    P.saoL = pd.sao_luma;
    P.saoC = pd.sao_chroma;
    P.flags = sp.flags | (a.xntu ? PF_COHERENT : 0u) | (Mid ? pd.flags & (PD_NMID_MAX << PD_NMID_SHIFT) : 0u);
    P.bits_off = (uint32_t)pd.bits_off;
    P.bits_end = (uint32_t)pd.bits_off + a.rsubs[pd.sub_first + pd.n_sub];
    P.sub_first = pd.sub_first;
    P.row_off = pd.row_off;
    P.tu_cap = pd.tu_cap_row;
    P.coef_cap = pd.coef_cap_row;
    P.pic = (uint32_t)pic;
    P.gqpy = (int8_t HG_GAS *)(a.maps + pd.map_off);
    P.gflags = (uint8_t HG_GAS *)(a.maps + pd.map_off + (size_t)P.w4 * P.h4);
    P.gdepth = (uint8_t HG_GAS *)(a.maps + pd.map_off + 2 * (size_t)P.w4 * P.h4);
    P.gsao = (SaoParams HG_GAS *)(a.sao + pd.sao_off);
    P.tu_base = (TuRec HG_GAS *)(a.tus + pd.tu_off);
    P.coef_base = (Coef HG_GAS *)(a.coefs + pd.coef_off);
    return true;
}

HG_HD inline void lane_start(Lane &L, const LanePic &P, LaneLds &ld, int row) {
    L.status = 0;
    L.cn = 0;
    L.k = 8;
    L.ai = L.bv = L.fp = 0;
    L.lb = 0;
    L.fl = (P.flags & SP_WPP) ? F_WPP : 0u;
    L.row = row;
    L.c = 0;
    L.qp_prev_last = P.sliceQp;
    row_outputs(L, P);
    L.st = U_CTU;
}

template <bool Mid = true>
HG_HD inline bool lane_init(Lane &L, LanePic &P, LaneLds &ld, const BatchArgs &a, int pic, int row, int lane0,
                            int cap) {
    if (!pic_init<Mid>(P, a, pic, lane0, cap) || row >= P.R) return false;
    lane_start(L, P, ld, row);
    return true;
}

}
}
```

### heif_amd/csrc/kernels/rbsp.hip

```cpp
#include "kernels.hpp"

namespace hg {

__device__ inline void zero_outputs(const BatchArgs &a, int pic, int lane, int nl) {
    const PicDesc &pd = a.pics[pic];
    if (lane == 0) a.status[pic] = 0;
    if (pic == a.pic0 && lane == 0 && a.xjob) *a.xjob = 0;
    if (pd.flags & PD_ASSEMBLY) return;
    const SeqParams &sp = a.seqs[pd.seq];
    const int hctb = (sp.height + (1 << sp.log2_ctb) - 1) >> sp.log2_ctb;
    for (int i = lane; i < 2 * hctb; i += nl) a.row_counts[2 * (size_t)pd.row_off + i] = 0;
    if (a.xprog)
        for (int i = lane; i < hctb; i += nl) a.xprog[pd.row_off + i] = 0;
    if (a.intra_stream && a.xntu) {
        for (int i = lane; i < hctb; i += nl) a.xntu[pd.row_off + i] = 0;
        if (lane == 0) a.xntu[a.total_rows + pic] = 0;
    }
}

#if defined(HG_HOST_EMU)
void emu_rbsp(const BatchArgs &a) {
    for (int p = a.pic0; p < a.pic0 + a.n_pics; ++p) {
        const PicDesc &pd = a.pics[p];
        const uint8_t *raw = a.bits + pd.bits_off;
        uint8_t *out = a.rbsp + pd.bits_off;
        const uint32_t len = pd.bits_len;
        std::vector<uint32_t> removed_before(len + 1, 0);
        uint32_t o = 0, r = 0;
        for (uint32_t i = 0; i < len; ++i) {
            removed_before[i] = r;
            const bool ep = raw[i] == 3 && i >= 2 && raw[i - 1] == 0 && raw[i - 2] == 0 && (i + 1 == len || raw[i + 1] <= 3);
            if (ep) ++r;
            else out[o++] = raw[i];
        }
        removed_before[len] = r;
        for (uint32_t s = 0; s <= pd.n_sub + (pd.flags >> PD_NMID_SHIFT); ++s) {
            const uint32_t e = a.subs[pd.sub_first + s] & SUB_OFFSET, fl = a.subs[pd.sub_first + s] & ~SUB_OFFSET;
            a.rsubs[pd.sub_first + s] = (e < len ? e - removed_before[e] : len - r) | fl;
        }
        zero_outputs(a, p, 0, 1);
    }
}
#else
namespace {

__device__ __forceinline__ uint32_t byte_of(const uint4 &q, int j) {
    const uint32_t w = j < 4 ? q.x : j < 8 ? q.y : j < 12 ? q.z : q.w;
    return (w >> ((j & 3) * 8)) & 0xffu;
}

__device__ __forceinline__ bool has3(uint32_t w) {
    const uint32_t x = w ^ 0x03030303u;
    return ((x - 0x01010101u) & ~x & 0x80808080u) != 0;
}

__device__ __forceinline__ int wave_excl_sum(int v, int lane, int &total) {
    int s = v;
#pragma unroll
    for (int d = 1; d < 64; d <<= 1) {
        const int t = __shfl_up(s, d, 64);
        if (lane >= d) s += t;
    }
    total = __shfl(s, 63, 64);
    return s - v;
}

}

__global__ void __launch_bounds__(64) k_rbsp(BatchArgs a) {
#if !defined(HG_HOST_EMU) && HG_PARSE_SETPRIO > 0
    __builtin_amdgcn_s_setprio(HG_PARSE_SETPRIO);
#endif
    const int pic = a.pic0 + (int)blockIdx.x;
    const int lane = (int)threadIdx.x;
    const PicDesc &pd = a.pics[pic];
    const uint8_t *raw = a.bits + pd.bits_off;
    uint8_t *out = a.rbsp + pd.bits_off;
    const uint32_t len = pd.bits_len;
    const uint32_t nent = pd.n_sub + 1 + (pd.flags >> PD_NMID_SHIFT);
    const uint32_t *subs = a.subs + pd.sub_first;
    uint32_t *rsubs = a.rsubs + pd.sub_first;
    uint32_t run = 0;
    for (uint32_t c0 = 0; c0 < len; c0 += 1024) {
        const uint32_t i0 = c0 + (uint32_t)lane * 16u;
        uint4 q = make_uint4(0, 0, 0, 0);
        uint32_t mask = 0;
        if (i0 < len) {
            q = *reinterpret_cast<const uint4 *>(raw + i0);
            if (has3(q.x) || has3(q.y) || has3(q.z) || has3(q.w)) {
                const uint32_t pw = i0 ? *reinterpret_cast<const uint32_t *>(raw + i0 - 4) : 0xffffffffu;
                const uint32_t nw = *reinterpret_cast<const uint32_t *>(raw + i0 + 16);
                uint32_t p2 = (pw >> 16) & 0xffu, p1 = pw >> 24;
                for (int j = 0; j < 16; ++j) {
                    const uint32_t b = byte_of(q, j);
                    const uint32_t nb = j < 15 ? byte_of(q, j + 1) : (nw & 0xffu);
                    const uint32_t pos = i0 + (uint32_t)j;
                    if (b == 3 && p1 == 0 && p2 == 0 && pos < len && (pos + 1 == len || nb <= 3)) mask |= 1u << j;
                    p2 = p1;
                    p1 = b;
                }
            }
        }
        int total;
        const uint32_t ex = (uint32_t)wave_excl_sum(__popc(mask), lane, total);
        if (i0 < len) {
            const uint32_t sh = run + ex;
            if (sh == 0 && mask == 0) {
                *reinterpret_cast<uint4 *>(out + i0) = q;
            } else {
                for (int j = 0; j < 16; ++j) {
                    const uint32_t pos = i0 + (uint32_t)j;
                    if (pos < len && !((mask >> j) & 1u))
                        out[pos - sh - (uint32_t)__popc(mask & ((1u << j) - 1u))] = (uint8_t)byte_of(q, j);
                }
            }
        }
        for (uint32_t g = 0; g < nent; g += 64) {
            const uint32_t idx = g + (uint32_t)lane;
            const uint32_t raw_e = idx < nent ? subs[idx] : 0xffffffffu;
            const uint32_t e = raw_e & SUB_OFFSET;
            const bool here = e >= c0 && e < c0 + 1024u && e < len;
            const int t = here ? (int)((e - c0) >> 4) : 0;
            const uint32_t ext = (uint32_t)__shfl((int)ex, t, 64);
            const uint32_t mt = (uint32_t)__shfl((int)mask, t, 64);
            if (here)
                rsubs[idx] = (e - (run + ext + (uint32_t)__popc(mt & ((1u << ((e - c0) & 15u)) - 1u)))) |
                             (raw_e & ~SUB_OFFSET);
        }
        run += (uint32_t)total;
    }
    for (uint32_t idx = (uint32_t)lane; idx < nent; idx += 64)
        if ((subs[idx] & SUB_OFFSET) >= len) rsubs[idx] = (len - run) | (subs[idx] & ~SUB_OFFSET);
    zero_outputs(a, pic, lane, 64);
}

hipError_t launch_rbsp(const BatchArgs &a, hipStream_t s) {
    if (a.n_pics <= 0) return hipSuccess;
    hipLaunchKernelGGL(k_rbsp, dim3(a.n_pics), dim3(64), 0, s, a);
    return hipGetLastError();
}
#endif

}
```

### heif_amd/csrc/kernels/transform.hip

```cpp
#include "xform.hpp"

namespace hg {

namespace {

#ifndef HG_XF_WAVES
#define HG_XF_WAVES 4
#endif
constexpr int kWaves = HG_XF_WAVES;

#define wave_sync() HG_WAVE_SYNC()

}

#if !defined(HG_XF_WPE)
#define HG_XF_WPE 7
#endif
__global__ void __launch_bounds__(kWaves * 64) __attribute__((amdgpu_waves_per_eu(HG_XF_WPE))) k_transform(BatchArgs a) {
    HG_BLOCK_SHARED __attribute__((aligned(16))) int16_t dtile[kWaves][32 * kXfDStride32];
    HG_BLOCK_SHARED __attribute__((aligned(16))) int16_t gtile[kWaves][32 * 32];
    HG_BLOCK_SHARED int32_t extent[kWaves][2];
    HG_BLOCK_SHARED XfTab s_tab;
#if defined(HG_HOST_EMU)
    xf_tables(&s_tab, 0, 1);
#else
    xf_tables(&s_tab, (int)threadIdx.x, (int)blockDim.x);
#endif
    const int16_t *s_mt = s_tab.mt;
    __syncthreads();
    const int pic = a.pic0 + blockIdx.y, row = blockIdx.x;
    const PicDesc pd = a.pics[pic];
    if (pd.flags & PD_ASSEMBLY) return;
    const SeqParams sp = a.seqs[pd.seq];
    const int hctb = (sp.height + (1 << sp.log2_ctb) - 1) >> sp.log2_ctb;
    if (row >= hctb) return;
    const int wave = (int)HG_UNI(threadIdx.x >> 6), lane = threadIdx.x & 63;
    const uint32_t ntu = a.row_counts[2 * (pd.row_off + row)];
    const TuRec *tus = a.tus + pd.tu_off + (uint64_t)row * pd.tu_cap_row;
    const CoefSrc<false> coefs{a.coefs + pd.coef_off + (uint64_t)row * pd.coef_cap_row};
    const int W = sp.width, H = sp.height;
    const int cw = HG_UNI(sp.chroma_format ? W >> chroma_sx(sp.chroma_format) : 0);
    const int ch = HG_UNI(sp.chroma_format ? H >> chroma_sy(sp.chroma_format) : 0);
    int16_t HG_GAS *const res0 = (int16_t HG_GAS *)(a.resid + pd.resid_off);
    int16_t HG_GAS *res_plane[3] = {res0, res0 + (size_t)W * H, res0 + (size_t)W * H + (size_t)cw * ch};
    const int pitch[3] = {W, cw, cw};
    const bool scaling = (sp.flags & SP_SCALING_LIST) != 0;
    int16_t *d = dtile[wave];
    int16_t *g = gtile[wave];

    {
        const uint32_t mine = ntu > (uint32_t)wave ? (ntu - (uint32_t)wave + kWaves - 1) / kWaves : 0;
        auto want4 = [&](const TuRec &tu) -> bool {
            const int cidx = tu.flags & TU_CIDX_MASK;
            return (tu.flags & TU_CBF) && tu.log2 == 2 && cidx <= 2 && tu.x + 4 <= pitch[cidx] &&
                   tu.y + 4 <= (cidx ? ch : H);
        };
        auto round4 = [&](auto &&grp) {
            for (int vl = lane; vl < 64; vl += kWave) d[vl] = 0;
            wave_sync();
            for (int vl = lane; vl < 64; vl += kWave) {
                TuRec tu;
                const int l16 = vl & 15;
                if (!grp(vl, tu)) continue;
                const int cidx = tu.flags & TU_CIDX_MASK;
                const int bd = cidx ? sp.bit_depth_c : sp.bit_depth_y;
                int pos, dv;
                if (tu.flags & TU_PCM) {
                    if (l16 >= (int)tu.ncoef) continue;
                    const Coef c = coefs.word(tu.coef + (uint32_t)l16);
                    pos = (int)(c & 15u);
                    dv = (int)(int16_t)(c >> 16);
                } else {
                    if (tu.ncoef < 4) continue;
                    const SbRec r = load_rec(coefs, tu.coef);
                    if (!((r.sig() >> l16) & 1u)) continue;
                    const int above = l16 < 15 ? __builtin_popcountll(r.esc() >> (4 * l16 + 4)) : 0;
                    dv = r.level(l16, above, coefs);
                    pos = r.pos(l16, 2);
                }
                if (!(tu.flags & TU_BYPASS)) {
                    const int qp = tu.qp, bd_shift = bd - 3;
                    const int ls = c_level_scale[qp % 6] << (qp / 6);
                    const int m =
                        scaling ? a.sf[sp.sf_off + sf_size_offset(0) + (uint32_t)cidx * 16u + (uint32_t)pos] : 16;
                    dv = clip16(((int64_t)dv * m * ls + ((int64_t)1 << (bd_shift - 1))) >> bd_shift);
                }
                d[(vl & 48) + ((pos & 3) << 2) + (pos >> 2)] = (int16_t)dv;
            }
            wave_sync();
            for (int vl = lane; vl < 64; vl += kWave) {
                TuRec tu;
                if (!grp(vl, tu) || (tu.flags & (TU_BYPASS | TU_TSKIP))) continue;
                const int y = (vl & 15) >> 2, x = vl & 3;
                const uint32_t *pa = reinterpret_cast<const uint32_t *>(mt_of(s_mt, 2, (tu.flags & TU_DST) != 0) + y * 4);
                const uint32_t *pb = reinterpret_cast<const uint32_t *>(d + (vl & 48) + x * 4);
                const int s = dot2_i16(pa[1], pb[1], dot2_i16(pa[0], pb[0], 0));
                g[vl] = (int16_t)min(max((s + 64) >> 7, -32768), 32767);
            }
            wave_sync();
            for (int vl = lane; vl < 64; vl += kWave) {
                TuRec tu;
                if (!grp(vl, tu)) continue;
                const int cidx = tu.flags & TU_CIDX_MASK;
                const int bd2 = 20 - (cidx ? sp.bit_depth_c : sp.bit_depth_y);
                const int y = (vl & 15) >> 2, x = vl & 3;
                const int16_t *dq = d + (vl & 48), *gq = g + (vl & 48);
                int r;
                if (tu.flags & TU_BYPASS) {
                    r = dq[x * 4 + y];
                } else if (tu.flags & TU_TSKIP) {
                    r = (dq[x * 4 + y] * (1 << 7) + (1 << (bd2 - 1))) >> bd2;
                } else {
                    const uint32_t *pa = reinterpret_cast<const uint32_t *>(mt_of(s_mt, 2, (tu.flags & TU_DST) != 0) + x * 4);
                    const uint32_t *pb = reinterpret_cast<const uint32_t *>(gq + y * 4);
                    const int s = dot2_i16(pa[1], pb[1], dot2_i16(pa[0], pb[0], 0));
                    r = (s + (1 << (bd2 - 1))) >> bd2;
                }
                res_plane[cidx][(size_t)(tu.y + y) * pitch[cidx] + tu.x + x] = (int16_t)clip16(r);
            }
            wave_sync();
        };
#if defined(HG_HOST_EMU)
        for (uint32_t j = 0; j < mine; j += 4) {
            round4([&](int vl, TuRec &tu) -> bool {
                const uint32_t jq = j + (uint32_t)(vl >> 4);
                if (jq >= mine) return false;
                tu = tus[(uint32_t)wave + kWaves * jq];
                return want4(tu);
            });
        }
#else
        static_assert(kWave == 64, "one record per lane");
        for (uint32_t c0 = 0; c0 < mine; c0 += 64) {
            const uint32_t jl = c0 + (uint32_t)lane;
            uint4 rec = make_uint4(0, 0, 0, 0);
            if (jl < mine) rec = *reinterpret_cast<const uint4 *>(tus + (uint32_t)wave + kWaves * jl);
            TuRec rl;
            __builtin_memcpy(&rl, &rec, sizeof(rl));
            uint64_t todo = __ballot(jl < mine && want4(rl));
            while (todo) {
                int src = -1;
                for (int q = 0; q < 4 && todo; ++q) {
                    const int jq = __builtin_ctzll(todo);
                    todo &= todo - 1;
                    if (q == (lane >> 4)) src = jq;
                }
                const int sl = src < 0 ? 0 : src;
                const uint4 r = make_uint4((uint32_t)__shfl((int)rec.x, sl, 64), (uint32_t)__shfl((int)rec.y, sl, 64),
                                           (uint32_t)__shfl((int)rec.z, sl, 64), (uint32_t)__shfl((int)rec.w, sl, 64));
                TuRec tu_c;
                __builtin_memcpy(&tu_c, &r, sizeof(tu_c));
                const bool ok_c = src >= 0;
                round4([&](int, TuRec &tu) -> bool {
                    tu = tu_c;
                    return ok_c;
                });
            }
        }
#endif
    }

    auto pass_b = [&](const TuRec &tu) {
        const int cidx = tu.flags & TU_CIDX_MASK;
        transform_tb(tu, coefs, sp, a.sf, XfScratch{d, g, extent[wave], &s_tab},
                     res_plane[cidx] + (size_t)tu.y * pitch[cidx] + tu.x, pitch[cidx], lane);
    };
    auto wanted = [&](const TuRec &tu) {
        const int cidx = tu.flags & TU_CIDX_MASK, n = 1 << tu.log2;
        return (tu.flags & TU_CBF) && tu.log2 != 2 && tu.log2 <= 5 && cidx <= 2 && tu.x + n <= pitch[cidx] &&
               tu.y + n <= (cidx ? ch : H);
    };
#if defined(HG_HOST_EMU)
    for (uint32_t t = wave; t < ntu; t += kWaves)
        if (wanted(tus[t])) pass_b(tus[t]);
#else
    for (uint32_t t0 = wave; t0 < ntu; t0 += 64u * kWaves) {
        const uint32_t t = t0 + (uint32_t)lane * kWaves;
        uint4 rec = make_uint4(0, 0, 0, 0);
        if (t < ntu) rec = *reinterpret_cast<const uint4 *>(tus + t);
        TuRec mine;
        __builtin_memcpy(&mine, &rec, sizeof(mine));
        uint64_t todo = __ballot(t < ntu && wanted(mine));
        while (todo) {
            const int j = __builtin_ctzll(todo);
            todo &= todo - 1;
            const uint4 r = make_uint4((uint32_t)__builtin_amdgcn_readlane((int)rec.x, j),
                                       (uint32_t)__builtin_amdgcn_readlane((int)rec.y, j),
                                       (uint32_t)__builtin_amdgcn_readlane((int)rec.z, j),
                                       (uint32_t)__builtin_amdgcn_readlane((int)rec.w, j));
            TuRec tu;
            __builtin_memcpy(&tu, &r, sizeof(tu));
            pass_b(tu);
        }
    }
#endif
}

__global__ void __launch_bounds__(kWaves * 64) k_paint_flags(BatchArgs a) {
    const int pic = a.pic0 + blockIdx.y, row = blockIdx.x;
    const PicDesc pd = a.pics[pic];
    if (pd.flags & PD_ASSEMBLY) return;
    const SeqParams sp = a.seqs[pd.seq];
    const int hctb = (sp.height + (1 << sp.log2_ctb) - 1) >> sp.log2_ctb;
    if (row >= hctb) return;
    const int w4 = (sp.width + 3) >> 2, h4 = (sp.height + 3) >> 2;
    uint8_t *flg = a.maps + pd.map_off + (size_t)w4 * h4;
    const uint32_t ntu = min(a.row_counts[2 * (pd.row_off + row)], pd.tu_cap_row);
    const TuRec *tus = a.tus + pd.tu_off + (uint64_t)row * pd.tu_cap_row;
    const int wave = (int)(threadIdx.x >> 6), lane = threadIdx.x & 63;
    for (uint32_t t0 = 64u * wave; t0 < ntu; t0 += 64u * kWaves) {
        for (int vl = lane; vl < 64; vl += kWave) {
            const uint32_t t = t0 + (uint32_t)vl;
            if (t >= ntu) continue;
            const TuRec tu = tus[t];
            if ((tu.flags & (TU_CIDX_MASK | TU_PCM)) || tu.log2 < 2 || tu.log2 > 5) continue;
            const int nb = 1 << (tu.log2 - 2), gx0 = tu.x >> 2, gy0 = tu.y >> 2;
            if (gx0 >= w4 || gy0 >= h4) continue;
            const int wx = gx0 + nb <= w4 ? nb : w4 - gx0, hy = gy0 + nb <= h4 ? nb : h4 - gy0;
            const uint8_t nf = (tu.flags & TU_BYPASS) ? MF_NOFILT : 0;
            for (int y = 0; y < hy; ++y) {
                uint8_t *r = flg + (size_t)(gy0 + y) * w4 + gx0;
                const uint8_t h = (uint8_t)((y == 0 ? MF_EDGE_H : 0) | nf);
                const uint64_t v = (0x0101010101010101ull * h) | (uint64_t)MF_EDGE_V;
                if (wx == 8) {
                    __builtin_memcpy(r, &v, 8);
                } else if (wx == 4) {
                    __builtin_memcpy(r, &v, 4);
                } else {
                    for (int x = 0; x < wx; ++x) r[x] = (uint8_t)(v >> (8 * x));
                }
            }
        }
    }
}

#if defined(HG_HOST_EMU)
void emu_transform(const BatchArgs &a) {
    emu_launch(k_transform, a.max_rows, a.n_pics, kWaves, a);
    if (a.flags_from_recs) emu_launch(k_paint_flags, a.max_rows, a.n_pics, kWaves, a);
}
#else
hipError_t launch_transform(const BatchArgs &a, hipStream_t s) {
    hipLaunchKernelGGL(k_transform, dim3(a.max_rows, a.n_pics), dim3(kWaves * 64), 0, s, a);
    if (a.flags_from_recs) hipLaunchKernelGGL(k_paint_flags, dim3(a.max_rows, a.n_pics), dim3(kWaves * 64), 0, s, a);
    return hipGetLastError();
}
#endif

}
```

Before: 27310.

## Defer QP map painting from lane parse to transform via compact CU lists

In lane parse mode, each CU now appends a packed word (position, size, QP) to a per-row CU list instead of painting the per-4x4 QP map. The transform stage's paint kernel expands these lists into the QP map in parallel. Per-CU line-buffer updates for intra modes and depths are also rewritten as 64-bit masked word writes, and luma mode derivation reads from registers. The aim is to take serial byte stores off the CABAC parse critical path, at the cost of extra buffers, a capacity check, and more work in the transform stage.

Result: faster. 27730 (median of 6 runs) (+1.5%).

```diff
diff --git a/heif_amd/csrc/api.cpp b/heif_amd/csrc/api.cpp
--- a/heif_amd/csrc/api.cpp
+++ b/heif_amd/csrc/api.cpp
@@ -172,6 +172,7 @@
     DevBuf<TuRec> tus;
     DevBuf<Coef> coefs;
     DevBuf<uint32_t> row_counts, status;
+    DevBuf<uint32_t> cus, cu_counts;
     DevBuf<uint8_t> maps;
     DevBuf<SaoParams> sao;
     DevBuf<int16_t> resid;
@@ -965,7 +966,9 @@
                                      hb.sao_n > b->set[0].sao.cap || 2 * size_t(hb.rows) > b->set[0].row_counts.cap ||
                                      hb.pics.size() > b->set[0].status.cap || hb.pics.size() > G.sticky.cap ||
                                      (cross_rows && (xprog_words(hb) > b->set[0].xprog.cap || hb.rows * CTX_PAD > b->xctx.cap)) ||
-                                     (mode == PARSE_SPREAD && xntu_words(hb) > b->set[0].xntu.cap));
+                                     (mode == PARSE_SPREAD && xntu_words(hb) > b->set[0].xntu.cap) ||
+                                     (mode == PARSE_LANES && (cu_list_off(hb.sao_n, hb.max_log2ctb) > b->set[0].cus.cap ||
+                                                              size_t(hb.rows) > b->set[0].cu_counts.cap)));
     if (grows) {
         for (int k = 0; k < b->n_sets; ++k)
             if (b->set[k].pending) HIP_TRY(hipEventSynchronize(b->set[k].recon_done));
@@ -990,6 +993,10 @@
         HIP_TRY(ps.tus.alloc(hb.tu_n));
         HIP_TRY(ps.coefs.alloc(hb.coef_n));
         HIP_TRY(ps.row_counts.alloc(size_t(2) * hb.rows));
+        if (mode == PARSE_LANES) {
+            HIP_TRY(ps.cus.alloc(cu_list_off(hb.sao_n, hb.max_log2ctb)));
+            HIP_TRY(ps.cu_counts.alloc(hb.rows));
+        }
         HIP_TRY(ps.maps.alloc(hb.map_bytes));
         HIP_TRY(ps.sao.alloc(hb.sao_n));
         HIP_TRY(ps.status.alloc(hb.pics.size()));
@@ -1147,6 +1154,8 @@
     a.tus = ps.tus.p;
     a.coefs = ps.coefs.p;
     a.row_counts = ps.row_counts.p;
+    a.cus = a.parse_mode == PARSE_LANES ? ps.cus.p : nullptr;
+    a.cu_counts = a.parse_mode == PARSE_LANES ? ps.cu_counts.p : nullptr;
     a.maps = ps.maps.p;
     a.sao = ps.sao.p;
     a.status = ps.status.p;
@@ -1171,6 +1180,7 @@
         HIP_TRY(hipStreamSynchronize(ctx->recon));
         HIP_TRY(hipMemsetAsync(ps.status.p, 0, size_t(b->n_pics) * sizeof(uint32_t), s));
         HIP_TRY(hipMemsetAsync(ps.row_counts.p, 0, size_t(2) * uint32_t(b->args.total_rows) * sizeof(uint32_t), s));
+        if (a.cu_counts) HIP_TRY(hipMemsetAsync(a.cu_counts, 0, uint32_t(b->args.total_rows) * sizeof(uint32_t), s));
         HIP_TRY(launch_rbsp(a, s));
         hipError_t (*fns[5])(const BatchArgs &, hipStream_t) = {launch_parse, launch_transform, launch_intra,
                                                                 launch_deblock, launch_sao_out};
diff --git a/heif_amd/csrc/emu/emu_check.cpp b/heif_amd/csrc/emu/emu_check.cpp
--- a/heif_amd/csrc/emu/emu_check.cpp
+++ b/heif_amd/csrc/emu/emu_check.cpp
@@ -72,6 +72,7 @@
     std::vector<TuRec> tus(hb.tu_n);
     std::vector<Coef> coefs(hb.coef_n);
     std::vector<uint32_t> rc(2 * hb.rows), status(hb.pics.size());
+    std::vector<uint32_t> cus(cu_list_off(hb.sao_n, hb.max_log2ctb), 0xa5a5a5a5u), cu_counts(hb.rows);
     std::vector<uint8_t> recon(hb.recon_bytes), maps(hb.map_bytes);
     if (getenv("HEIFGPU_EMU_DUMP_MAPS")) std::fill(maps.begin(), maps.end(), uint8_t(0xa5));
     std::vector<int16_t> resid(hb.resid_elems);
@@ -117,6 +118,8 @@
     a.tus = tus.data();
     a.coefs = coefs.data();
     a.row_counts = rc.data();
+    a.cus = cus.data();
+    a.cu_counts = cu_counts.data();
     a.recon = recon.data();
     a.resid = resid.data();
     a.maps = maps.data();
@@ -153,6 +156,7 @@
         return 0;
     }
     std::fill(rc.begin(), rc.end(), 0xa5a5a5a5u);
+    std::fill(cu_counts.begin(), cu_counts.end(), 0xa5a5a5a5u);
     std::fill(status.begin(), status.end(), 0x5au);
     std::fill(xprog.begin(), xprog.end(), 0x7777u);
     std::fill(xntu.begin(), xntu.end(), 0x3333u);
diff --git a/heif_amd/csrc/emu/emu_parse.cpp b/heif_amd/csrc/emu/emu_parse.cpp
--- a/heif_amd/csrc/emu/emu_parse.cpp
+++ b/heif_amd/csrc/emu/emu_parse.cpp
@@ -107,7 +107,9 @@
             printf("\n  sb_paths");
             for (int k = COV_N; k < COV_SB_END; ++k) printf(" %ld", g_cov[k]), g_cov[k] = 0;
             printf("\n  tb_paths");
-            for (int k = COV_SB_END; k < COV_ALL; ++k) printf(" %ld", g_cov[k]), g_cov[k] = 0;
+            for (int k = COV_SB_END; k < COV_TB_END; ++k) printf(" %ld", g_cov[k]), g_cov[k] = 0;
+            printf("\n  cu_paths");
+            for (int k = COV_TB_END; k < COV_ALL; ++k) printf(" %ld", g_cov[k]), g_cov[k] = 0;
             printf("\n");
         }
     }
diff --git a/heif_amd/csrc/kernels/kernels.hpp b/heif_amd/csrc/kernels/kernels.hpp
--- a/heif_amd/csrc/kernels/kernels.hpp
+++ b/heif_amd/csrc/kernels/kernels.hpp
@@ -54,8 +54,16 @@
     int has_assembly;
     int intra_split;
     int lanes_lean;
+    uint32_t *cus;
+    uint32_t *cu_counts;
     int flags_from_recs;
 };
+
+constexpr uint32_t cu_cap_row(int wctb, int log2ctb) { return (uint32_t)wctb << (2 * (log2ctb - 3)); }
+constexpr uint64_t cu_list_off(uint64_t sao_off, int max_log2ctb) { return sao_off << (2 * (max_log2ctb - 3)); }
+constexpr uint32_t cu_word(int x, int y_in_row, int log2, int qpy) {
+    return (uint32_t)(x >> 3) | ((uint32_t)(y_in_row >> 3) << 16) | ((uint32_t)log2 << 20) | ((uint32_t)qpy << 24);
+}
 
 struct ColorArgs {
     uint64_t plane[3];
diff --git a/heif_amd/csrc/kernels/parse_state.hpp b/heif_amd/csrc/kernels/parse_state.hpp
--- a/heif_amd/csrc/kernels/parse_state.hpp
+++ b/heif_amd/csrc/kernels/parse_state.hpp
@@ -4,6 +4,7 @@
 #include "tables.hpp"
 
 #include <algorithm>
+#include <cstddef>
 #include <cstdint>
 #include <vector>
 
@@ -63,6 +64,8 @@
     uint8_t dL[8], dA[8];
     int8_t qL[8], qA[8];
 };
+static_assert(offsetof(LaneLds, ipmL) % 8 == 0 && offsetof(LaneLds, ipmA) % 8 == 0, "64-bit line updates");
+static_assert(offsetof(LaneLds, dL) % 8 == 0 && offsetof(LaneLds, dA) % 8 == 0, "64-bit line updates");
 
 struct LanePic {
     int W, H, log2ctb, wctb, hctb, minCb, minTb, maxTb, maxDepthIntra, chroma;
@@ -78,6 +81,7 @@
     TuRec HG_GAS *tu_base;
     Coef HG_GAS *coef_base;
 };
+HG_HD inline uint32_t HG_GAS *lane_cus(const LanePic &P) { return (uint32_t HG_GAS *)P.gqpy; }
 
 enum Unit : int {
     U_DONE = 0,
@@ -136,6 +140,7 @@
     int rc_scan, rc_last_sub, rc_last_pos, rc_i, rc_prev_c1;
     uint64_t rc_csbf;
     uint32_t ntu, ncoef;
+    uint32_t ncu;
     uint32_t nesc;
     uint32_t tu_row, coef_row;
     uint32_t cx;
@@ -152,9 +157,12 @@
         (t0) = t_;                                                                   \
     } while (0)
 #endif
-#if defined(HG_PARSE_PROF_SB) && !defined(HG_HOST_EMU) && !defined(HG_PARSE_PROF_TB)
+#if defined(HG_PARSE_PROF_TB) && defined(HG_PARSE_PROF_CU)
+#error "prof-tb and prof-cu share the six phase slots: one of them per build"
+#endif
+#if defined(HG_PARSE_PROF_SB) && !defined(HG_HOST_EMU) && !defined(HG_PARSE_PROF_TB) && !defined(HG_PARSE_PROF_CU)
 #define HG_SB_T(L, i, t0) HG_PHASE_T(L, i, t0)
-#elif defined(HG_PARSE_PROF_TB) && !defined(HG_HOST_EMU)
+#elif (defined(HG_PARSE_PROF_TB) || defined(HG_PARSE_PROF_CU)) && !defined(HG_HOST_EMU)
 #define HG_SB_T(L, i, t0) ((void)(t0))
 #else
 #define HG_SB_T(L, i, t0) ((void)0)
@@ -165,6 +173,13 @@
 #else
 #define HG_TB_T0(t0) ((void)0)
 #define HG_TB_T(L, i, t0) ((void)0)
+#endif
+#if defined(HG_PARSE_PROF_CU) && !defined(HG_HOST_EMU)
+#define HG_CU_T0(t0) uint64_t t0 = __builtin_amdgcn_s_memtime()
+#define HG_CU_T(L, i, t0) HG_PHASE_T(L, i, t0)
+#else
+#define HG_CU_T0(t0) ((void)0)
+#define HG_CU_T(L, i, t0) ((void)0)
 #endif
 
 enum Cov : int {
@@ -203,7 +218,9 @@
     COV_LAST_SUFFIX_X_ONLY,
     COV_LAST_SUFFIX_Y_ONLY,
     COV_LAST_SWAP,
-    COV_ALL
+    COV_TB_END,
+    COV_CU_DONE = COV_TB_END,
+    COV_ALL = COV_CU_DONE + 4
 };
 #if defined(HG_HOST_EMU)
 long g_cov[COV_ALL];
diff --git a/heif_amd/csrc/kernels/parse_units.hpp b/heif_amd/csrc/kernels/parse_units.hpp
--- a/heif_amd/csrc/kernels/parse_units.hpp
+++ b/heif_amd/csrc/kernels/parse_units.hpp
@@ -70,6 +70,63 @@
     if (m >= l1) ++m;
     if (m >= l2) ++m;
     return m;
+}
+HG_HD inline int luma_mode(int ca, int cb, int prev, int mpm_idx, int rem) {
+    int l0, l1, l2;
+    if (ca == cb) {
+        if (ca < 2) {
+            l0 = 0;
+            l1 = 1;
+            l2 = 26;
+        } else {
+            l0 = ca;
+            l1 = 2 + ((ca + 29) % 32);
+            l2 = 2 + ((ca - 2 + 1) % 32);
+        }
+    } else {
+        l0 = ca;
+        l1 = cb;
+        if (ca != 0 && cb != 0) l2 = 0;
+        else if (ca != 1 && cb != 1) l2 = 1;
+        else l2 = 26;
+    }
+    if (prev) return mpm_idx == 0 ? l0 : (mpm_idx == 1 ? l1 : l2);
+    int t;
+    if (l0 > l1) { t = l0; l0 = l1; l1 = t; }
+    if (l0 > l2) { t = l0; l0 = l2; l2 = t; }
+    if (l1 > l2) { t = l1; l1 = l2; l2 = t; }
+    int m = rem;
+    if (m >= l0) ++m;
+    if (m >= l1) ++m;
+    if (m >= l2) ++m;
+    return m;
+}
+
+#if !defined(HG_LINE_BYTES)
+#define HG_LINE_BYTES 0
+#endif
+template <class EG>
+constexpr bool kLineWords(int which) { return !EG::kSolo && !(HG_LINE_BYTES & which); }
+HG_HD inline uint64_t line_ld(const void *line) {
+    uint64_t w;
+    __builtin_memcpy(&w, line, 8);
+    return w;
+}
+HG_HD inline void line_st(void *line, uint64_t w) { __builtin_memcpy(line, &w, 8); }
+HG_HD inline void line8_fill(void *line, int b0, int nb, int v) {
+    const uint64_t m = (~0ull >> (64 - 8 * nb)) << (8 * b0);
+    line_st(line, (line_ld(line) & ~m) | ((0x0101010101010101ull * (uint8_t)v) & m));
+}
+HG_HD inline void line16_fill(uint8_t *line, uint64_t w, int b0, int nb, int lo, int hi) {
+    const uint64_t rl = 0x0101010101010101ull * (uint8_t)lo, rh = 0x0101010101010101ull * (uint8_t)hi;
+    if (nb == 16) {
+        line_st(line, rl);
+        line_st(line + 8, rh);
+        return;
+    }
+    const int h = 4 * nb, sh = 8 * (b0 & 7);
+    const uint64_t hm = (1ull << h) - 1, m = ~0ull >> (64 - 8 * nb);
+    line_st(line + (b0 & 8), (w & ~(m << sh)) | (((rl & hm) | ((rh & hm) << h)) << sh));
 }
 
 HG_HD inline uint64_t scan4_word(int scan) { return scan == 0 ? kScan4Pos[0] : (scan == 1 ? kScan4Pos[1] : kScan4Pos[2]); }
@@ -318,6 +375,7 @@
 
 template <class EG>
 HG_HD inline void unit_cqt(Lane &L, LaneLds &ld, LanePic &P, const EG &G) {
+    HG_CU_T0(tcq);
     for (;;) {
         const int n = 1 << L.ql;
         bool split;
@@ -344,9 +402,11 @@
         --L.ql;
         ++L.qd;
     }
+    HG_CU_T(L, 0, tcq);
     L.st = U_CU;
 }
 
+template <class EG>
 HG_HD inline void cu_done(Lane &L, LaneLds &ld, LanePic &P);
 template <class EG>
 HG_HD inline void tu_emit(Lane &L, const LanePic &P);
@@ -356,9 +416,14 @@
     const int n = 1 << L.ql;
     {
         const int nb = n >> 2, by = (L.qy - L.ctby) >> 2, bx = (L.qx - L.ctbx) >> 2;
-        for (int k = 0; k < nb; ++k) {
-            ld.ipmL[by + k] = 1;
-            ld.ipmA[bx + k] = 1;
+        if constexpr (kLineWords<EG>(2)) {
+            line16_fill(ld.ipmL, line_ld(ld.ipmL + (by & 8)), by, nb, 1, 1);
+            line16_fill(ld.ipmA, line_ld(ld.ipmA + (bx & 8)), bx, nb, 1, 1);
+        } else {
+            for (int k = 0; k < nb; ++k) {
+                ld.ipmL[by + k] = 1;
+                ld.ipmA[bx + k] = 1;
+            }
         }
     }
     uint32_t bit = (uint32_t)(8 * (int32_t)P.bits_end - L.budget - L.k + 7) & ~7u;
@@ -406,11 +471,12 @@
     } else {
         engine_init(L, G, next, P.bits_end);
     }
-    cu_done(L, ld, P);
+    cu_done<EG>(L, ld, P);
 }
 
 template <class EG>
 HG_HD inline void unit_cu(Lane &L, LaneLds &ld, LanePic &P, const EG &G) {
+    HG_CU_T0(tcu);
     if (L.fl & F_QG_NEW) {
         derive_qp_pred(L, ld, P);
         L.fl &= ~F_QG_NEW;
@@ -421,14 +487,21 @@
     if (L.ql == P.minCb && !dec(L, G, CTX_PART_MODE)) L.fl |= F_NXN;
     const bool nxn = (L.fl & F_NXN) != 0;
     const bool pcm = !nxn && (pic_flags<EG>(P) & SP_PCM) && L.ql >= P.pcmMin && L.ql <= P.pcmMax && term(L, G);
+    HG_CU_T(L, 1, tcu);
     {
         const int nd = 1 << (L.ql - 3);
         const int dy = (L.qy - L.ctby) >> 3, dx = (L.qx - L.ctbx) >> 3;
-        for (int k = 0; k < nd; ++k) {
-            ld.dL[dy + k] = (uint8_t)L.qd;
-            ld.dA[dx + k] = (uint8_t)L.qd;
-        }
-    }
+        if constexpr (kLineWords<EG>(1)) {
+            line8_fill(ld.dL, dy, nd, L.qd);
+            line8_fill(ld.dA, dx, nd, L.qd);
+        } else {
+            for (int k = 0; k < nd; ++k) {
+                ld.dL[dy + k] = (uint8_t)L.qd;
+                ld.dA[dx + k] = (uint8_t)L.qd;
+            }
+        }
+    }
+    HG_CU_T(L, 2, tcu);
     if constexpr (!EG::kLean) {
         if (pcm) {
             pcm_cu(L, ld, P, G);
@@ -447,6 +520,17 @@
         for (int i = 0; i < np; ++i) prev |= dec(L, G, CTX_PREV_INTRA) << i;
     }
     int modes = 0;
+    const int nbc = 1 << (L.ql - 2), byc = (L.qy - L.ctby) >> 2, bxc = (L.qx - L.ctbx) >> 2;
+    uint64_t wl = 0, wa = 0;
+    int nl1 = 1, na1 = 1;
+    if constexpr (kLineWords<EG>(2)) {
+        wl = line_ld(ld.ipmL + (byc & 8));
+        wa = line_ld(ld.ipmA + (bxc & 8));
+        if (nxn) {
+            nl1 = nbc == 16 ? ld.ipmL[8] : (int)(wl >> (8 * ((byc & 7) + (nbc >> 1)))) & 0xff;
+            na1 = nbc == 16 ? ld.ipmA[8] : (int)(wa >> (8 * ((bxc & 7) + (nbc >> 1)))) & 0xff;
+        }
+    }
     for (int i = 0; i < np; ++i) {
         const int p = (prev >> i) & 1;
         int mpm = 0, rem = 0;
@@ -457,14 +541,30 @@
             mpm = rem = byp_luma_mode(L, G, p);
         }
         if (nxn) HG_COV(p ? COV_NXN_MPM + mpm : COV_NXN_REM);
-        const int xPb = L.qx + (i & 1) * pb, yPb = L.qy + (i >> 1) * pb;
-        const int m = derive_luma_mode(L, ld, xPb, yPb, p, mpm, rem);
-        modes |= m << (8 * i);
-        const int nb = pb >> 2, by = (yPb - L.ctby) >> 2, bx = (xPb - L.ctbx) >> 2;
-        for (int k = 0; k < nb; ++k) {
-            ld.ipmL[by + k] = (uint8_t)m;
-            ld.ipmA[bx + k] = (uint8_t)m;
-        }
+        HG_CU_T(L, 3, tcu);
+        if constexpr (kLineWords<EG>(2)) {
+            const int ca = (i & 1) ? (modes >> (8 * (i - 1))) & 0xff
+                                   : (L.qx <= 0 ? 1 : (i ? nl1 : (int)(wl >> (8 * (byc & 7))) & 0xff));
+            const int cb = (i & 2) ? (modes >> (8 * (i - 2))) & 0xff
+                                   : (L.qy - 1 < L.ctby ? 1 : (i ? na1 : (int)(wa >> (8 * (bxc & 7))) & 0xff));
+            modes |= luma_mode(ca, cb, p, mpm, rem) << (8 * i);
+        } else {
+            const int xPb = L.qx + (i & 1) * pb, yPb = L.qy + (i >> 1) * pb;
+            const int m = derive_luma_mode(L, ld, xPb, yPb, p, mpm, rem);
+            modes |= m << (8 * i);
+            const int nb = pb >> 2, by = (yPb - L.ctby) >> 2, bx = (xPb - L.ctbx) >> 2;
+            for (int k = 0; k < nb; ++k) {
+                ld.ipmL[by + k] = (uint8_t)m;
+                ld.ipmA[bx + k] = (uint8_t)m;
+            }
+        }
+        HG_CU_T(L, 4, tcu);
+    }
+    if constexpr (kLineWords<EG>(2)) {
+        const int m0 = modes & 0xff;
+        line16_fill(ld.ipmL, wl, byc, nbc, nxn ? (modes >> 8) & 0xff : m0, nxn ? (modes >> 24) & 0xff : m0);
+        line16_fill(ld.ipmA, wa, bxc, nbc, nxn ? (modes >> 16) & 0xff : m0, nxn ? (modes >> 24) & 0xff : m0);
+        HG_CU_T(L, 4, tcu);
     }
     L.cu_modes = modes;
     if (HG_PIC_CHROMA(P)) {
@@ -485,6 +585,7 @@
         }
         L.cu_chroma = nc == 1 ? (int)((uint32_t)cms * 0x01010101u) : cms;
     }
+    HG_CU_T(L, 5, tcu);
     L.tx = L.qx, L.ty = L.qy, L.tl = L.ql, L.td = 0, L.tcbf = 0;
     L.st = U_TT;
 }
@@ -496,6 +597,18 @@
 template <class EG>
 constexpr bool kFlagsInParse = EG::kSolo;
 #endif
+#if defined(HG_QPY_IN_PARSE)
+template <class EG>
+constexpr bool kQpyInParse = true;
+#else
+template <class EG>
+constexpr bool kQpyInParse = EG::kSolo;
+#endif
+template <class EG>
+HG_HD inline int8_t HG_GAS *qpy_map(const LanePic &P) {
+    if constexpr (EG::kSolo) return P.gqpy;
+    else return (int8_t HG_GAS *)(P.gflags - (size_t)P.w4 * P.h4);
+}
 
 template <class EG>
 HG_HD inline void unit_tt(Lane &L, LaneLds &ld, LanePic &P, const EG &G) {
@@ -568,7 +681,6 @@
         L.cu_qp_delta_val = v;
         update_qpy(L, P);
     }
-    HG_TB_T(L, 3, ttt);
     if constexpr (kFlagsInParse<EG>) {
         const int nb = 1 << (L.tl - 2), gx0 = L.tx >> 2, gy0 = L.ty >> 2;
         const int wx = gx0 + nb <= P.w4 ? nb : P.w4 - gx0, hy = gy0 + nb <= P.h4 ? nb : P.h4 - gy0;
@@ -580,7 +692,7 @@
             store_bytes(row, wx, (rep * h) | (uint64_t)MF_EDGE_V);
         }
     }
-    HG_TB_T(L, 4, ttt);
+    HG_TB_T(L, 3, ttt);
     const int blk = L.td == 0 ? 0 : (((L.tx >> L.tl) & 1) | (((L.ty >> L.tl) & 1) << 1));
     L.tb_n = (HG_PIC_CHROMA(P) != 0 && (!chroma4 || blk == 3)) ? (HG_PIC_CHROMA(P) == 2 ? 5 : 3) : 1;
     L.tb_t = 0;
@@ -617,6 +729,7 @@
     }
 }
 
+template <class EG>
 HG_HD inline void cu_done(Lane &L, LaneLds &ld, LanePic &P);
 
 template <class EG>
@@ -641,11 +754,13 @@
         ++L.tl;
         --L.td;
     }
-    cu_done(L, ld, P);
-}
-
+    cu_done<EG>(L, ld, P);
+}
+
+template <class EG>
 HG_HD inline void cu_done(Lane &L, LaneLds &ld, LanePic &P) {
     HG_TB_T0(tcu);
+    HG_COV(COV_CU_DONE + L.ql - 3);
     {
         const int n = 1 << L.ql, nd = n >> 3;
         const int dy = (L.qy - L.ctby) >> 3, dx = (L.qx - L.ctbx) >> 3;
@@ -653,11 +768,21 @@
             ld.qL[dy + k] = (int8_t)L.qpy_cur;
             ld.qA[dx + k] = (int8_t)L.qpy_cur;
         }
-        const int nb = n >> 2, gx0 = L.qx >> 2, gy0 = L.qy >> 2;
-        const int wx = gx0 + nb <= P.w4 ? nb : P.w4 - gx0, hy = gy0 + nb <= P.h4 ? nb : P.h4 - gy0;
-        for (int y = 0; y < hy; ++y) {
-            int8_t *row = P.gqpy + (size_t)(gy0 + y) * P.w4 + gx0;
-            store_bytes(reinterpret_cast<uint8_t *>(row), wx, 0x0101010101010101ull * (uint8_t)L.qpy_cur);
+        HG_TB_T(L, 4, tcu);
+        if constexpr (!EG::kSolo) {
+            if (HG_LIKELY(L.ncu < cu_cap_row(P.wctb, P.log2ctb)))
+                lane_cus(P)[(uint32_t)L.row * cu_cap_row(P.wctb, P.log2ctb) + L.ncu++] =
+                    cu_word(L.qx, L.qy - L.ctby, L.ql, L.qpy_cur);
+            else
+                L.status |= ST_CAPACITY;
+        }
+        if constexpr (kQpyInParse<EG>) {
+            const int nb = n >> 2, gx0 = L.qx >> 2, gy0 = L.qy >> 2;
+            const int wx = gx0 + nb <= P.w4 ? nb : P.w4 - gx0, hy = gy0 + nb <= P.h4 ? nb : P.h4 - gy0;
+            for (int y = 0; y < hy; ++y) {
+                int8_t *row = qpy_map<EG>(P) + (size_t)(gy0 + y) * P.w4 + gx0;
+                store_bytes(reinterpret_cast<uint8_t *>(row), wx, 0x0101010101010101ull * (uint8_t)L.qpy_cur);
+            }
         }
         L.qp_prev_last = L.qpy_cur;
     }
@@ -979,7 +1104,7 @@
             cw(off + 1, c0 >> 16);
             cw(off + 2, c0 >> 24);
         }
-#if defined(HG_PARSE_PROF_SB) && !defined(HG_PARSE_PROF_TB) && !defined(HG_HOST_EMU)
+#if defined(HG_PARSE_PROF_SB) && !defined(HG_PARSE_PROF_TB) && !defined(HG_PARSE_PROF_CU) && !defined(HG_HOST_EMU)
         L.psb[4] += (uint64_t)(nstart + 1);
 #endif
         HG_SB_T(L, 1, tsb);
@@ -1181,11 +1306,13 @@
     uint32_t *rc = E.a->row_counts + 2 * (size_t)(P.row_off + L.row);
     rc[0] = L.ntu;
     rc[1] = L.ncoef;
+    if constexpr (!EG::kSolo) E.a->cu_counts[P.row_off + L.row] = L.ncu;
     const int step = (L.fl & F_WPP) ? P.R : 1;
     if (!(L.fl & F_STOP) && L.row + step < P.hctb) {
         L.row += step;
         L.c = 0;
         row_outputs(L, P);
+        if constexpr (!EG::kSolo) L.ncu = 0;
         L.st = U_CTU;
         return;
     }
@@ -1269,7 +1396,8 @@
     P.tu_cap = pd.tu_cap_row;
     P.coef_cap = pd.coef_cap_row;
     P.pic = (uint32_t)pic;
-    P.gqpy = (int8_t HG_GAS *)(a.maps + pd.map_off);
+    if constexpr (Mid) P.gqpy = (int8_t HG_GAS *)(a.cus + cu_list_off(pd.sao_off, a.max_log2ctb));
+    else P.gqpy = (int8_t HG_GAS *)(a.maps + pd.map_off);
     P.gflags = (uint8_t HG_GAS *)(a.maps + pd.map_off + (size_t)P.w4 * P.h4);
     P.gdepth = (uint8_t HG_GAS *)(a.maps + pd.map_off + 2 * (size_t)P.w4 * P.h4);
     P.gsao = (SaoParams HG_GAS *)(a.sao + pd.sao_off);
@@ -1297,6 +1425,7 @@
                             int cap) {
     if (!pic_init<Mid>(P, a, pic, lane0, cap) || row >= P.R) return false;
     lane_start(L, P, ld, row);
+    if constexpr (Mid) L.ncu = 0;
     return true;
 }
 
diff --git a/heif_amd/csrc/kernels/rbsp.hip b/heif_amd/csrc/kernels/rbsp.hip
--- a/heif_amd/csrc/kernels/rbsp.hip
+++ b/heif_amd/csrc/kernels/rbsp.hip
@@ -10,6 +10,8 @@
     const SeqParams &sp = a.seqs[pd.seq];
     const int hctb = (sp.height + (1 << sp.log2_ctb) - 1) >> sp.log2_ctb;
     for (int i = lane; i < 2 * hctb; i += nl) a.row_counts[2 * (size_t)pd.row_off + i] = 0;
+    if (a.cu_counts)
+        for (int i = lane; i < hctb; i += nl) a.cu_counts[pd.row_off + i] = 0;
     if (a.xprog)
         for (int i = lane; i < hctb; i += nl) a.xprog[pd.row_off + i] = 0;
     if (a.intra_stream && a.xntu) {
diff --git a/heif_amd/csrc/kernels/transform.hip b/heif_amd/csrc/kernels/transform.hip
--- a/heif_amd/csrc/kernels/transform.hip
+++ b/heif_amd/csrc/kernels/transform.hip
@@ -232,6 +232,35 @@
             }
         }
     }
+    uint8_t *qmap = a.maps + pd.map_off;
+    const int wctb = (sp.width + (1 << sp.log2_ctb) - 1) >> sp.log2_ctb;
+    const uint32_t cap = cu_cap_row(wctb, sp.log2_ctb);
+    const uint32_t ncu = min(a.cu_counts[pd.row_off + row], cap);
+    const uint32_t *cus = a.cus + cu_list_off(pd.sao_off, a.max_log2ctb) + (uint64_t)row * cap;
+    for (uint32_t t0 = 64u * wave; t0 < ncu; t0 += 64u * kWaves) {
+        for (int vl = lane; vl < 64; vl += kWave) {
+            const uint32_t t = t0 + (uint32_t)vl;
+            if (t >= ncu) continue;
+            const uint32_t w = cus[t];
+            const int log2 = (int)((w >> 20) & 15u);
+            if (log2 < 3 || log2 > 6) continue;
+            const int nb = 1 << (log2 - 2), gx0 = (int)(w & 0xffffu) << 1;
+            const int gy0 = (row << (sp.log2_ctb - 2)) + ((int)((w >> 16) & 15u) << 1);
+            if (gx0 >= w4 || gy0 >= h4) continue;
+            const int wx = gx0 + nb <= w4 ? nb : w4 - gx0, hy = gy0 + nb <= h4 ? nb : h4 - gy0;
+            const uint64_t v = 0x0101010101010101ull * (uint64_t)(w >> 24);
+            for (int y = 0; y < hy; ++y) {
+                uint8_t *r = qmap + (size_t)(gy0 + y) * w4 + gx0;
+                int x = 0;
+                for (; x + 8 <= wx; x += 8) __builtin_memcpy(r + x, &v, 8);
+                if (x + 4 <= wx) {
+                    __builtin_memcpy(r + x, &v, 4);
+                    x += 4;
+                }
+                for (; x < wx; ++x) r[x] = (uint8_t)v;
+            }
+        }
+    }
 }
 
 #if defined(HG_HOST_EMU)
```
